# s-esposito/MonoGS

Measured on AMD Instinct MI355X. Metric: rasteriser fwd+bwd Mpix/s @1080p, higher is better.
Workload: dtype f32; 1 GPU; C5: 2000000 Gaussians, 1920x1080, fwd+bwd, seeded synthetic map (SURVEY.md 8d), one keyframe per GPU; gaussians=2000000, width=1920, height=1080, settle_steps=60, instance_count=device-side (capacity mode, overflow checked), parallelism=keyframe-per-gpu x1

## Files before the change

### include/monogs_raster.h

```cpp
#ifndef MONOGS_RASTER_H
#define MONOGS_RASTER_H

#include <stddef.h>
#include <stdint.h>

#ifdef __cplusplus
extern "C" {
#endif

#define MGS_ABI_VERSION 9
#define MGS_TILE 16

typedef struct mgs_camera {
    int32_t image_height;
    int32_t image_width;
    float tanfovx;
    float tanfovy;
    float scale_modifier;
    int32_t sh_degree;
    int32_t sh_coeffs;
    int32_t scale_dim;
    int32_t flags;
    const float* bg;
    const float* viewmatrix;
    const float* projmatrix;
    const float* projmatrix_raw;
    const float* campos;
} mgs_camera;

#define MGS_FLAG_EXCLUSIVE_DEVICE 1

typedef struct mgs_timing {
    float preprocess_ms;
    float depth_sort_ms;
    float scan_ms;
    float duplicate_ms;
    float sort_ms;
    float ranges_ms;
    float blend_fwd_ms;
    float blend_bwd_ms;
    float geom_bwd_ms;
} mgs_timing;

int mgs_abi_version(void);
const char* mgs_last_error(void);

#define MGS_MAX_GAUSSIANS ((1 << 26) - 1)

size_t mgs_geometry_bytes(int32_t P);
size_t mgs_image_bytes(int32_t width, int32_t height);
size_t mgs_binning_bytes(uint64_t num_rendered, int32_t width, int32_t height);
size_t mgs_backward_bytes(int32_t P);
float* mgs_backward_tau(void* backward_scratch, int32_t P);

int mgs_forward_preprocess(const mgs_camera* cam, int32_t P,
                           const float* means3D,
                           const float* shs,
                           const float* colors_precomp,
                           const float* opacities,
                           const float* scales,
                           const float* rotations,
                           const float* cov3D_precomp,
                           void* geometry, int32_t* radii ,
                           void* prepare_backward ,
                           uint64_t* num_rendered ,
                           const uint32_t* prev_status ,
                           uint32_t* prev_status_out ,
                           mgs_timing* timing , void* stream);

int mgs_forward_render(const mgs_camera* cam, int32_t P, uint64_t num_rendered,
                       void* geometry, void* binning, void* image,
                       float* out_color, float* out_depth, float* out_opacity, int32_t* n_touched,
                       uint32_t* status ,
                       mgs_timing* timing, void* stream);

#define MGS_STATUS_CAPACITY_OVERFLOW 1u
#define MGS_STATUS_DEPTH_SORT_TIMEOUT 2u
#define MGS_STATUS_TILE_SORT_TIMEOUT 4u

int mgs_debug_set_radix_spin_limit(uint32_t limit);
int mgs_debug_set_option(const char* name, int64_t value);

size_t mgs_debug_sort_temp_bytes(uint64_t n, int32_t bits);
int mgs_debug_sort_pairs(uint32_t* keys, uint32_t* vals, uint32_t* keys_alt, uint32_t* vals_alt, uint64_t n, int32_t bits,
                         void* temp, void* stream);

int mgs_forward_render_capacity(const mgs_camera* cam, int32_t P, uint64_t capacity,
                                void* geometry, void* binning, void* image,
                                float* out_color, float* out_depth, float* out_opacity, int32_t* n_touched,
                                uint32_t* overflow, mgs_timing* timing, void* stream);
int mgs_forward_capacity(const mgs_camera* cam, int32_t P, const float* means3D, const float* shs,
                         const float* colors_precomp, const float* opacities, const float* scales, const float* rotations,
                         const float* cov3D_precomp, void* geometry, int32_t* radii, void* prepare_backward,
                         uint64_t capacity, void* binning, void* image, float* out_color, float* out_depth,
                         float* out_opacity, int32_t* n_touched, uint32_t* overflow, mgs_timing* timing, void* stream);

int mgs_backward(const mgs_camera* cam, int32_t P, uint64_t num_rendered,
                 const float* means3D, const float* shs, const float* colors_precomp,
                 const float* opacities, const float* scales, const float* rotations,
                 const float* cov3D_precomp, const int32_t* radii,
                 const void* geometry, const void* binning, const void* image,
                 const float* dL_dcolor, const float* dL_ddepth,
                 float* dL_dmeans2D,
                 float* dL_dcolors,
                 float* dL_dopacity,
                 float* dL_dmeans3D,
                 float* dL_dcov3D,
                 float* dL_dsh,
                 float* dL_dscales,
                 float* dL_drotations,
                 float* dL_dtau,
                 void* backward_scratch, int32_t scratch_prepared, mgs_timing* timing, void* stream);

#define MGS_VALU_CEILING_BLOCKS 2048
int mgs_debug_valu_ceiling(float* out, int32_t iters, void* stream);

int mgs_debug_set_blend_events(void* fwd_start, void* fwd_end, void* bwd_start, void* bwd_end);

#define MGS_BLEND_STATS_WORDS 24
int mgs_debug_blend_stats(const mgs_camera* cam, int32_t P, uint64_t num_rendered, const void* geometry,
                          const void* binning, const void* image, uint64_t* stats_dev, void* stream);

int mgs_mark_visible(int32_t P, const float* means3D, const float* viewmatrix, const float* projmatrix,
                     uint8_t* visible, void* stream);

size_t mgs_knn_scratch_bytes(int32_t P);
int mgs_dist2_knn(int32_t P, const float* points , float* out ,
                  void* scratch, void* stream);

#define MGS_LOSS_TRACKING 1
#define MGS_LOSS_INVERT_DEPTH 2
#define MGS_LOSS_SCRATCH_DAB 10
#define MGS_LOSS_SCRATCH_LOSS 12
size_t mgs_loss_scratch_bytes(void);
int mgs_loss_forward(int32_t width, int32_t height, int32_t mode, int32_t init, float lambda_rgb,
                     const float* render, const float* depth, const float* opacity, const float* gt_rgb,
                     const float* gt_depth, const uint8_t* mask, const uint8_t* grad_mask,
                     const float* exposure_a, const float* exposure_b, float* scratch, float* loss_out,
                     void* stream);
int mgs_loss_backward(int32_t width, int32_t height, int32_t mode, int32_t init, float lambda_rgb,
                      const float* render, const float* depth, const float* opacity, const float* gt_rgb,
                      const float* gt_depth, const uint8_t* mask, const uint8_t* grad_mask,
                      const float* exposure_a, const float* exposure_b, const float* scratch,
                      const float* grad_out, float* d_render, float* d_depth, float* d_exposure, void* stream);
int mgs_loss_grads(int32_t width, int32_t height, int32_t mode, int32_t init, float lambda_rgb,
                   const float* render, const float* depth, const float* opacity, const float* gt_rgb,
                   const float* gt_depth, const uint8_t* mask, const uint8_t* grad_mask,
                   const float* exposure_a, const float* exposure_b, float* scratch, float* d_render, float* d_depth,
                   void* stream);

#define MGS_POSE_STICKY 1
int mgs_pose_step(float* R, float* T, float* rot_delta, float* trans_delta, float* exposure_a, float* exposure_b,
                  const float* grad_rot, const float* grad_trans, const float* grad_a, const float* grad_b,
                  float* adam_m, float* adam_v, int32_t step, float lr_rot, float lr_trans, float lr_exposure,
                  float beta1, float beta2, float eps, float converged_threshold, int32_t* step_counter, float* out,
                  int32_t flags, float* host_flag ,
                  const float* projmatrix_raw, float* viewmatrix, float* projmatrix, float* campos ,
                  void* stream);
int mgs_pose_step_batch(int32_t n, void* const* ptrs, float lr_rot, float lr_trans, float lr_exposure, float beta1,
                        float beta2, float eps, float converged_threshold, int32_t flags, void* stream);

int mgs_backproject(int32_t N, int32_t W, int32_t H, const int64_t* selected, const float* rgb ,
                    const float* depth , const int32_t* segmentation ,
                    const float* exposure_a, const float* exposure_b, float fx, float fy, float cx, float cy,
                    const float* R, const float* T, float* points , float* features ,
                    int32_t* ids , void* stream);

int mgs_camera_setup(const float* R, const float* T, const float* projmatrix_raw, float* viewmatrix ,
                     float* projmatrix , float* campos , void* stream);

int mgs_adam_step(int32_t n_tensors, float* const* params, const float* const* grads, float* const* exp_avg,
                  float* const* exp_avg_sq, const uint64_t* numel, const float* lr, double beta1, double beta2,
                  double eps, int32_t step, int32_t* step_counter,
                  const float* lr_device ,
                  void* stream);
int mgs_densify_stats(int32_t P, const float* viewspace_grad , const int32_t* radii,
                      float* xyz_gradient_accum , float* denom , float* max_radii_2d ,
                      void* stream);
int mgs_window_stats(int32_t P, int32_t n_keyframes, const float* const* grad_means2D, const int32_t* const* radii,
                     const int32_t* const* n_touched, float* grad_norm , float* visible ,
                     float* max_radii , int32_t accumulate, uint64_t* visibility_bits, void* stream);
int mgs_window_apply(int32_t P, const float* grad_norm, const float* visible, const float* max_radii,
                     float* xyz_gradient_accum, float* denom, float* max_radii_2d, void* stream);
int mgs_lr_schedule_step(int32_t* iteration, float* lr_out, double lr_init, double lr_final, int32_t lr_delay_steps,
                         double lr_delay_mult, int32_t max_steps, void* stream);

int mgs_activate_forward(int32_t P, int32_t scale_dim , const float* rot_raw ,
                         const float* scale_raw , const float* opacity_raw ,
                         float* rotations , float* scales3 , float* opacities ,
                         void* stream);
int mgs_activate_backward(int32_t P, int32_t scale_dim, const float* rot_raw, const float* scales3,
                          const float* opacities, const float* grad_rotations, const float* grad_scales3,
                          const float* grad_opacities, float* d_rot_raw, float* d_scale_raw, float* d_opacity_raw,
                          void* stream);

int mgs_sum_buffers(int32_t n_src, const float* const* src, float* dst, uint64_t count, void* stream);

#ifdef __cplusplus
}
#endif
#endif
```

### monogs_amd/_lib.py

```python
from __future__ import annotations

import ctypes as C
import os

_HERE = os.path.dirname(os.path.abspath(__file__))
LIB_PATH = os.environ.get("MGS_LIB_PATH") or os.path.join(_HERE, "lib", "libmonogs_raster.so")
ABI_VERSION = 9

c_float_p = C.c_void_p


class MgsCamera(C.Structure):
    _fields_ = [
        ("image_height", C.c_int32), ("image_width", C.c_int32),
        ("tanfovx", C.c_float), ("tanfovy", C.c_float), ("scale_modifier", C.c_float),
        ("sh_degree", C.c_int32), ("sh_coeffs", C.c_int32), ("scale_dim", C.c_int32), ("flags", C.c_int32),
        ("bg", C.c_void_p), ("viewmatrix", C.c_void_p), ("projmatrix", C.c_void_p),
        ("projmatrix_raw", C.c_void_p), ("campos", C.c_void_p),
    ]


class MgsTiming(C.Structure):
    _fields_ = [(n, C.c_float) for n in (
        "preprocess_ms", "depth_sort_ms", "scan_ms", "duplicate_ms", "sort_ms", "ranges_ms", "blend_fwd_ms",
        "blend_bwd_ms", "geom_bwd_ms")]

    def as_dict(self):
        return {n: float(getattr(self, n)) for n, _ in self._fields_}


SIGNATURES = {
    "mgs_abi_version": (C.c_int, []),
    "mgs_last_error": (C.c_char_p, []),
    "mgs_geometry_bytes": (C.c_size_t, [C.c_int32]),
    "mgs_image_bytes": (C.c_size_t, [C.c_int32, C.c_int32]),
    "mgs_binning_bytes": (C.c_size_t, [C.c_uint64, C.c_int32, C.c_int32]),
    "mgs_backward_bytes": (C.c_size_t, [C.c_int32]),
    "mgs_forward_preprocess": (C.c_int, [C.POINTER(MgsCamera), C.c_int32] + [C.c_void_p] * 7
                               + [C.c_void_p, C.c_void_p, C.c_void_p, C.POINTER(C.c_uint64), C.c_void_p, C.POINTER(C.c_uint32),
                                  C.POINTER(MgsTiming), C.c_void_p]),
    "mgs_forward_capacity": (C.c_int, [C.POINTER(MgsCamera), C.c_int32] + [C.c_void_p] * 7 + [C.c_void_p] * 3 + [C.c_uint64]
                             + [C.c_void_p] * 7 + [C.POINTER(MgsTiming), C.c_void_p]),
    "mgs_forward_render": (C.c_int, [C.POINTER(MgsCamera), C.c_int32, C.c_uint64] + [C.c_void_p] * 8
                           + [C.POINTER(MgsTiming), C.c_void_p]),
    "mgs_debug_set_radix_spin_limit": (C.c_int, [C.c_uint32]),
    "mgs_debug_set_option": (C.c_int, [C.c_char_p, C.c_int64]),
    "mgs_debug_sort_temp_bytes": (C.c_size_t, [C.c_uint64, C.c_int32]),
    "mgs_debug_sort_pairs": (C.c_int, [C.c_void_p] * 4 + [C.c_uint64, C.c_int32, C.c_void_p, C.c_void_p]),
    "mgs_forward_render_capacity": (C.c_int, [C.POINTER(MgsCamera), C.c_int32, C.c_uint64] + [C.c_void_p] * 8
                                    + [C.POINTER(MgsTiming), C.c_void_p]),
    "mgs_backward": (C.c_int, [C.POINTER(MgsCamera), C.c_int32, C.c_uint64] + [C.c_void_p] * 7
                     + [C.c_void_p] * 4 + [C.c_void_p] * 2 + [C.c_void_p] * 9
                     + [C.c_void_p, C.c_int32, C.POINTER(MgsTiming), C.c_void_p]),
    "mgs_backward_tau": (C.c_void_p, [C.c_void_p, C.c_int32]),
    "mgs_debug_blend_stats": (C.c_int, [C.POINTER(MgsCamera), C.c_int32, C.c_uint64] + [C.c_void_p] * 5),
    "mgs_debug_valu_ceiling": (C.c_int, [C.c_void_p, C.c_int32, C.c_void_p]),
    "mgs_debug_set_blend_events": (C.c_int, [C.c_void_p] * 4),
    "mgs_mark_visible": (C.c_int, [C.c_int32, C.c_void_p, C.c_void_p, C.c_void_p, C.c_void_p, C.c_void_p]),
    "mgs_loss_scratch_bytes": (C.c_size_t, []),
    "mgs_loss_forward": (C.c_int, [C.c_int32] * 4 + [C.c_float] + [C.c_void_p] * 9 + [C.c_void_p, C.c_void_p, C.c_void_p]),
    "mgs_loss_backward": (C.c_int, [C.c_int32] * 4 + [C.c_float] + [C.c_void_p] * 9
                          + [C.c_void_p, C.c_void_p, C.c_void_p, C.c_void_p, C.c_void_p, C.c_void_p]),
    "mgs_loss_grads": (C.c_int, [C.c_int32] * 4 + [C.c_float] + [C.c_void_p] * 9 + [C.c_void_p] * 4),
    "mgs_backproject": (C.c_int, [C.c_int32] * 3 + [C.c_void_p] * 6 + [C.c_float] * 4 + [C.c_void_p] * 6),
    "mgs_camera_setup": (C.c_int, [C.c_void_p] * 7),
    "mgs_pose_step": (C.c_int, [C.c_void_p] * 12 + [C.c_int32] + [C.c_float] * 7
                      + [C.c_void_p, C.c_void_p, C.c_int32, C.c_void_p] + [C.c_void_p] * 4 + [C.c_void_p]),
    "mgs_pose_step_batch": (C.c_int, [C.c_int32, C.POINTER(C.c_void_p)] + [C.c_float] * 7 + [C.c_int32, C.c_void_p]),
    "mgs_adam_step": (C.c_int, [C.c_int32] + [C.c_void_p] * 6 + [C.c_double] * 3 + [C.c_int32, C.c_void_p, C.c_void_p, C.c_void_p]),
    "mgs_window_stats": (C.c_int, [C.c_int32, C.c_int32] + [C.c_void_p] * 6 + [C.c_int32, C.c_void_p, C.c_void_p]),
    "mgs_window_apply": (C.c_int, [C.c_int32] + [C.c_void_p] * 7),
    "mgs_lr_schedule_step": (C.c_int, [C.c_void_p, C.c_void_p, C.c_double, C.c_double, C.c_int32, C.c_double, C.c_int32, C.c_void_p]),
    "mgs_densify_stats": (C.c_int, [C.c_int32] + [C.c_void_p] * 6),
    "mgs_sum_buffers": (C.c_int, [C.c_int32, C.POINTER(C.c_void_p), C.c_void_p, C.c_uint64, C.c_void_p]),
    "mgs_activate_forward": (C.c_int, [C.c_int32, C.c_int32] + [C.c_void_p] * 7),
    "mgs_activate_backward": (C.c_int, [C.c_int32, C.c_int32] + [C.c_void_p] * 10),
    "mgs_knn_scratch_bytes": (C.c_size_t, [C.c_int32]),
    "mgs_dist2_knn": (C.c_int, [C.c_int32, C.c_void_p, C.c_void_p, C.c_void_p, C.c_void_p]),
}

_lib = None


class MonoGSNativeError(RuntimeError):
    pass


def load():
    global _lib
    if _lib is not None:
        return _lib
    if not os.path.exists(LIB_PATH):
        raise MonoGSNativeError(
            f"{LIB_PATH} not found: build it with `python -c 'import __graft_entry__ as g; g.build()'` "
            "or `make -C monogs_amd/csrc`.  There is no CPU fallback.")
    lib = C.CDLL(LIB_PATH)
    for name, (res, args) in SIGNATURES.items():
        fn = getattr(lib, name)
        fn.restype = res
        fn.argtypes = args
    if lib.mgs_abi_version() != ABI_VERSION:
        raise MonoGSNativeError(f"ABI mismatch: library {lib.mgs_abi_version()} vs binding {ABI_VERSION}; rebuild")
    for kv in filter(None, os.environ.get("MGS_DEBUG_OPTIONS", "").split(",")):
        k, _, v = kv.partition("=")
        if lib.mgs_debug_set_option(k.strip().encode(), int(v)) != 0:
            raise MonoGSNativeError(f"MGS_DEBUG_OPTIONS: {lib.mgs_last_error().decode()}")
    _lib = lib
    return lib


def check(rc: int, what: str):
    if rc != 0:
        msg = load().mgs_last_error().decode("utf-8", "replace")
        raise Exception(msg) if rc == 1 else MonoGSNativeError(f"{what}: {msg}")
```

### monogs_amd/csrc/api.hip

```cpp
#include "common.h"

#include <stdarg.h>
#include <stdio.h>
#include <string.h>

namespace mgs {

static thread_local char g_err[512] = "";

void set_error(const char* fmt, ...) {
    va_list ap;
    va_start(ap, fmt);
    vsnprintf(g_err, sizeof(g_err), fmt, ap);
    va_end(ap);
}

static inline char* take(char*& p, size_t bytes) {
    char* r = p;
    p += align_up(bytes, 256);
    return r;
}

GeometryState GeometryState::carve(void* base, int P) {
    char* p = (char*)align_up((size_t)base, 256);
    GeometryState g;
    g.rec = (float*)take(p, (size_t)P * REC_FLOATS * sizeof(float));
    g.depth_key = (uint32_t*)take(p, (size_t)P * sizeof(uint32_t));
    g.depth_alt = (uint32_t*)take(p, (size_t)P * sizeof(uint32_t));
    g.iota = (uint32_t*)take(p, (size_t)P * sizeof(uint32_t));
    g.iota_alt = (uint32_t*)take(p, (size_t)P * sizeof(uint32_t));
    g.perm = (uint32_t*)take(p, (size_t)P * sizeof(uint32_t));
    g.point_offsets = (uint32_t*)take(p, (size_t)P * sizeof(uint32_t));
    g.scan_blocks = (uint32_t*)take(p, ((size_t)scan_nblocks(P) + 64) * sizeof(uint32_t));
    g.clamped = (uint8_t*)take(p, (size_t)P * 4);
    g.rect = (uint2*)take(p, (size_t)P * sizeof(uint2));
    g.rect_sorted = (uint2*)take(p, (size_t)P * sizeof(uint2));
    g.scan_status = (uint64_t*)take(p, (SCAN_SMALL_MAX_BLOCKS + 1) * sizeof(uint64_t));
    g.tile_hist = (uint32_t*)take(p, 4 * 256 * sizeof(uint32_t));
    g.sort_temp_bytes = radix_depth_temp_bytes((uint64_t)P);
    g.sort_temp = take(p, g.sort_temp_bytes);
    g.end = p;
    return g;
}
size_t GeometryState::bytes(int P) {
    const GeometryState g = carve(nullptr, P);
    return (size_t)g.end + 256;
}

size_t ImageState::bytes(int W, int H) {
    const size_t HW = (size_t)W * H, nt = (size_t)tiles_x(W) * tiles_y(H);
    return align_up(HW * 4, 256) * 2 + align_up(nt * sizeof(uint2), 256) + 256;
}
ImageState ImageState::carve(void* base, int W, int H) {
    const size_t HW = (size_t)W * H, nt = (size_t)tiles_x(W) * tiles_y(H);
    char* p = (char*)align_up((size_t)base, 256);
    ImageState s;
    s.final_T = (float*)take(p, HW * 4);
    s.n_contrib = (uint32_t*)take(p, HW * 4);
    s.ranges = (uint2*)take(p, nt * sizeof(uint2));
    return s;
}

size_t BinningState::bytes(uint64_t R, int W, int H) {
    const size_t r = (size_t)(R ? R : 1);
    return align_up(r * 4, 256) * 4 + align_up(mgs::sort_temp_bytes(R, tile_bits(W, H)), 256) + 256 + 256;
}
BinningState BinningState::carve(void* base, uint64_t R, int W, int H) {
    const size_t r = (size_t)(R ? R : 1);
    char* p = (char*)align_up((size_t)base, 256);
    BinningState b;
    b.keys_a = (uint32_t*)take(p, r * 4);
    b.keys_b = (uint32_t*)take(p, r * 4);
    b.vals_a = (uint32_t*)take(p, r * 4);
    b.vals_b = (uint32_t*)take(p, r * 4);
    const bool in_b = radix_result_in_b(tile_bits(W, H));
    b.keys_sorted = in_b ? b.keys_b : b.keys_a;
    b.vals_sorted = in_b ? b.vals_b : b.vals_a;
    b.sort_temp_bytes = mgs::sort_temp_bytes(R, tile_bits(W, H));
    b.sort_temp = take(p, b.sort_temp_bytes);
    b.count = (uint32_t*)take(p, 2 * sizeof(uint32_t));
    return b;
}

struct StageTimer {
    hipStream_t s;
    bool on;
    hipEvent_t ev[10];
    int n = 0;
    StageTimer(hipStream_t s_, bool on_) : s(s_), on(on_) {
        if (on) for (auto& e : ev) (void)hipEventCreate(&e);
    }
    ~StageTimer() {
        if (on) for (auto& e : ev) (void)hipEventDestroy(e);
    }
    void mark() {
        if (on && n < 10) (void)hipEventRecord(ev[n++], s);
    }
    float ms(int i) {
        float t = 0.f;
        if (on && i + 1 < n) (void)hipEventElapsedTime(&t, ev[i], ev[i + 1]);
        return t;
    }
    void sync() {
        if (on && n) (void)hipEventSynchronize(ev[n - 1]);
    }
};

static int check_cam(const mgs_camera* cam) {
    if (!cam) { set_error("camera is NULL"); return 1; }
    if (cam->image_width <= 0 || cam->image_height <= 0) { set_error("image size must be positive"); return 1; }
    if (!cam->bg || !cam->viewmatrix || !cam->projmatrix || !cam->projmatrix_raw || !cam->campos) {
        set_error("camera tensors (bg, viewmatrix, projmatrix, projmatrix_raw, campos) must be non-NULL");
        return 1;
    }
    return 0;
}

static hipEvent_t g_dbg_fwd_events[2] = {nullptr, nullptr}, g_dbg_bwd_events[2] = {nullptr, nullptr};

static int check_map_size(int32_t P) {
    if (P > MGS_MAX_GAUSSIANS) {
        set_error("P exceeds MGS_MAX_GAUSSIANS (2^26 - 1): the gradient-line offset of the blend backward is 32-bit");
        return 1;
    }
    return 0;
}

}

using namespace mgs;

extern "C" {

int mgs_abi_version(void) { return MGS_ABI_VERSION; }
const char* mgs_last_error(void) { return g_err; }

size_t mgs_geometry_bytes(int32_t P) { return GeometryState::bytes(P < 0 ? 0 : P); }
size_t mgs_image_bytes(int32_t W, int32_t H) { return ImageState::bytes(W, H); }
size_t mgs_binning_bytes(uint64_t R, int32_t W, int32_t H) { return BinningState::bytes(R, W, H); }
size_t mgs_backward_bytes(int32_t P) {
    return (size_t)(P < 0 ? 0 : P) * GRAD_FLOATS * sizeof(float) + (size_t)(TAU_SLOTS + 1) * 16 * sizeof(float) + 256;
}
float* mgs_backward_tau(void* backward_scratch, int32_t P) { return backward_tau_out(backward_scratch, P < 0 ? 0 : P); }

int mgs_forward_preprocess(const mgs_camera* cam, int32_t P, const float* means3D, const float* shs,
                           const float* colors_precomp, const float* opacities, const float* scales,
                           const float* rotations, const float* cov3D_precomp, void* geometry, int32_t* radii,
                           void* prepare_backward, uint64_t* num_rendered, const uint32_t* prev_status,
                           uint32_t* prev_status_out, mgs_timing* timing, void* stream) {
    if (check_cam(cam)) return 1;
    if (P < 0) { set_error("P must be >= 0"); return 1; }
    if (check_map_size(P)) return 1;
    if (num_rendered) *num_rendered = 0;
    if (prev_status_out) *prev_status_out = 0;
    if (P == 0) {
        if (prev_status && prev_status_out) {
            MGS_HIP(hipMemcpyAsync(prev_status_out, prev_status, sizeof(uint32_t), hipMemcpyDeviceToHost, (hipStream_t)stream));
            MGS_HIP(hipStreamSynchronize((hipStream_t)stream));
        }
        return 0;
    }
    if (!means3D || !opacities || !geometry || !radii) { set_error("means3D, opacities, geometry, radii must be non-NULL"); return 1; }
    if ((shs == nullptr) == (colors_precomp == nullptr)) {
        set_error("Please provide excatly one of either SHs or precomputed colors!");
        return 1;
    }
    const bool have_sr = scales != nullptr || rotations != nullptr;
    if ((have_sr && (!scales || !rotations || cov3D_precomp)) || (!have_sr && !cov3D_precomp)) {
        set_error("Please provide exactly one of either scale/rotation pair or precomputed 3D covariance!");
        return 1;
    }
    if (shs && (cam->sh_degree < 0 || cam->sh_degree > 3 || cam->sh_coeffs < (cam->sh_degree + 1) * (cam->sh_degree + 1))) {
        set_error("sh_degree must be 0..3 and shs must hold at least (degree+1)^2 coefficients");
        return 1;
    }
    hipStream_t s = (hipStream_t)stream;
    GeometryState g = GeometryState::carve(geometry, P);
    StageTimer tm(s, timing != nullptr);
    tm.mark();
    if (int rc = launch_preprocess_forward(*cam, P, means3D, shs, colors_precomp, opacities, scales, rotations,
                                           cov3D_precomp, g, radii,
                                           prepare_backward ? backward_grad_acc(prepare_backward) : nullptr, s)) return rc;
    tm.mark();
    const bool exclusive = (cam->flags & MGS_FLAG_EXCLUSIVE_DEVICE) != 0;
    if (depth_chain_is_small(P)) {
        if (int rc = launch_depth_chain_small(g, P, s)) return rc;
        tm.mark();
    } else {
        if (int rc = launch_depth_sort(g, P, depth_sort_payload(P, cam->image_width, cam->image_height), s, exclusive)) return rc;
        tm.mark();
        if (int rc = launch_scan(g, P, s, exclusive)) return rc;
    }
    tm.mark();
    if (num_rendered) {
        uint32_t total = 0, sort_errors[RADIX_ERROR_WORDS] = {0, 0, 0, 0};
        MGS_HIP(hipMemcpyAsync(&total, g.scan_blocks + scan_nblocks(P), sizeof(uint32_t), hipMemcpyDeviceToHost, s));
        MGS_HIP(hipMemcpyAsync(sort_errors, radix_depth_error_flag(g.sort_temp, (uint64_t)P), sizeof(sort_errors),
                               hipMemcpyDeviceToHost, s));
        if (prev_status && prev_status_out)
            MGS_HIP(hipMemcpyAsync(prev_status_out, prev_status, sizeof(uint32_t), hipMemcpyDeviceToHost, s));
        MGS_HIP(hipStreamSynchronize(s));
        if (sort_errors[0] | sort_errors[1] | sort_errors[2] | sort_errors[3]) { set_error("depth sort: a look-back spin timed out (results invalid)"); return 3; }
        *num_rendered = total;
    }
    if (timing) {
        if (!num_rendered) MGS_HIP(hipStreamSynchronize(s));
        timing->preprocess_ms = tm.ms(0);
        timing->depth_sort_ms = tm.ms(1);
        timing->scan_ms = tm.ms(2);
    }
    return 0;
}

static int forward_render_impl(const mgs_camera* cam, int32_t P, uint64_t R, bool capacity, void* geometry,
                               void* binning, void* image, float* out_color, float* out_depth, float* out_opacity,
                               int32_t* n_touched, uint32_t* overflow, mgs_timing* timing, void* stream) {
    if (check_cam(cam)) return 1;
    if (P < 0) { set_error("P must be >= 0"); return 1; }
    if (check_map_size(P)) return 1;
    if (!image || !out_color || !out_depth || !out_opacity) { set_error("image scratch and outputs must be non-NULL"); return 1; }
    if (P > 0 && (!geometry || !n_touched)) { set_error("geometry and n_touched must be non-NULL"); return 1; }
    if (R > 0 && !binning) { set_error("binning scratch is NULL"); return 1; }
    if (R >= (1ull << 32)) { set_error("num_rendered exceeds 2^32-1"); return 1; }
    if (P == 0) R = 0;
    hipStream_t s = (hipStream_t)stream;
    const int W = cam->image_width, H = cam->image_height;
    GeometryState g = GeometryState::carve(geometry, P);
    ImageState img = ImageState::carve(image, W, H);
    BinningState b = BinningState::carve(binning, R, W, H);
    const uint32_t* n_dev = nullptr;
    StageTimer tm(s, timing != nullptr);
    const bool cap = capacity && binning;
    if (cap) n_dev = b.count;
    tm.mark();
    if (int rc = launch_duplicate(*cam, P, g, b, capacity ? R : (R > 0 ? 0xFFFFFFFFull : 0ull), n_touched, img, R,
                                  tile_bits(W, H), cap ? b.count : nullptr, overflow, s)) return rc;
    tm.mark();
    if (int rc = launch_sort(g, b, R, tile_bits(W, H), s, n_dev, (cam->flags & MGS_FLAG_EXCLUSIVE_DEVICE) != 0, img.ranges)) return rc;
    tm.mark();
    if (g_dbg_fwd_events[0]) MGS_HIP(hipEventRecord(g_dbg_fwd_events[0], s));
    if (int rc = launch_blend_forward(*cam, g, b, img, out_color, out_depth, out_opacity, n_touched,
                                      R > 0 ? radix_error_flag(b.sort_temp, R, tile_bits(W, H)) : nullptr, overflow, s)) return rc;
    if (g_dbg_fwd_events[1]) MGS_HIP(hipEventRecord(g_dbg_fwd_events[1], s));
    tm.mark();
    if (timing) {
        tm.sync();
        timing->duplicate_ms = tm.ms(0);
        timing->sort_ms = tm.ms(1);
        timing->ranges_ms = 0.f;
        timing->blend_fwd_ms = tm.ms(2);
    }
    return 0;
}

int mgs_forward_render(const mgs_camera* cam, int32_t P, uint64_t R, void* geometry, void* binning, void* image,
                       float* out_color, float* out_depth, float* out_opacity, int32_t* n_touched,
                       uint32_t* status, mgs_timing* timing, void* stream) {
    return forward_render_impl(cam, P, R, false, geometry, binning, image, out_color, out_depth, out_opacity, n_touched,
                               status, timing, stream);
}

int mgs_forward_render_capacity(const mgs_camera* cam, int32_t P, uint64_t capacity, void* geometry, void* binning,
                                void* image, float* out_color, float* out_depth, float* out_opacity,
                                int32_t* n_touched, uint32_t* overflow, mgs_timing* timing, void* stream) {
    if (capacity == 0) { set_error("capacity must be > 0"); return 1; }
    return forward_render_impl(cam, P, capacity, true, geometry, binning, image, out_color, out_depth, out_opacity,
                               n_touched, overflow, timing, stream);
}

int mgs_forward_capacity(const mgs_camera* cam, int32_t P, const float* means3D, const float* shs,
                         const float* colors_precomp, const float* opacities, const float* scales, const float* rotations,
                         const float* cov3D_precomp, void* geometry, int32_t* radii, void* prepare_backward,
                         uint64_t capacity, void* binning, void* image, float* out_color, float* out_depth,
                         float* out_opacity, int32_t* n_touched, uint32_t* overflow, mgs_timing* timing, void* stream) {
    if (int rc = mgs_forward_preprocess(cam, P, means3D, shs, colors_precomp, opacities, scales, rotations, cov3D_precomp,
                                        geometry, radii, prepare_backward, nullptr, nullptr, nullptr, timing, stream)) return rc;
    return mgs_forward_render_capacity(cam, P, capacity, geometry, binning, image, out_color, out_depth, out_opacity,
                                       n_touched, overflow, timing, stream);
}

int mgs_backward(const mgs_camera* cam, int32_t P, uint64_t R, const float* means3D, const float* shs,
                 const float* colors_precomp, const float* opacities, const float* scales, const float* rotations,
                 const float* cov3D_precomp, const int32_t* radii, const void* geometry, const void* binning,
                 const void* image, const float* dL_dcolor, const float* dL_ddepth, float* dL_dmeans2D,
                 float* dL_dcolors, float* dL_dopacity, float* dL_dmeans3D, float* dL_dcov3D, float* dL_dsh,
                 float* dL_dscales, float* dL_drotations, float* dL_dtau, void* backward_scratch,
                 int32_t scratch_prepared, mgs_timing* timing, void* stream) {
    if (check_cam(cam)) return 1;
    if (P < 0) { set_error("P must be >= 0"); return 1; }
    if (check_map_size(P)) return 1;
    hipStream_t s = (hipStream_t)stream;
    if (P == 0) {
        if (dL_dtau) MGS_HIP(zero_fill(dL_dtau, 6 * sizeof(float), s));
        return 0;
    }
    if (!means3D || !opacities || !radii || !geometry || !image || !dL_dcolor || !dL_ddepth || !backward_scratch) {
        set_error("means3D, opacities, radii, geometry, image, dL_dcolor, dL_ddepth, backward_scratch must be non-NULL");
        return 1;
    }
    if (R > 0 && !binning) { set_error("binning scratch is NULL"); return 1; }
    const int W = cam->image_width, H = cam->image_height;
    GeometryState g = GeometryState::carve(const_cast<void*>(geometry), P);
    ImageState img = ImageState::carve(const_cast<void*>(image), W, H);
    BinningState b = BinningState::carve(const_cast<void*>(binning), R, W, H);
    float* grad_acc = backward_grad_acc(backward_scratch);
    StageTimer tm(s, timing != nullptr);
    float* tau_part = (dL_dtau && (P + 255) / 256 > TAU_DIRECT_MAX_BLOCKS) ? backward_tau_part(backward_scratch, P) : nullptr;
    if (scratch_prepared) {
        if (dL_dtau && dL_dtau != backward_tau_out(backward_scratch, P)) {
            set_error("scratch_prepared: dL_dtau must be mgs_backward_tau(backward_scratch, P)");
            return 1;
        }
    } else {
        MGS_HIP(zero_fill2(grad_acc, (size_t)P * GRAD_FLOATS * sizeof(float) + (tau_part ? (size_t)TAU_SLOTS * 16 * sizeof(float) : 0),
                           dL_dtau, 6 * sizeof(float), s));
    }
    tm.mark();
    if (R > 0) {
        const bool pose_only = !dL_dcolors && !dL_dopacity && !dL_dsh && !shs;
        if (g_dbg_bwd_events[0]) MGS_HIP(hipEventRecord(g_dbg_bwd_events[0], s));
        if (int rc = launch_blend_backward(*cam, g, b, img, dL_dcolor, dL_ddepth, grad_acc, pose_only, s)) return rc;
        if (g_dbg_bwd_events[1]) MGS_HIP(hipEventRecord(g_dbg_bwd_events[1], s));
    }
    tm.mark();
    GeomBackwardArgs a;
    a.means3D = means3D; a.shs = shs; a.colors_precomp = colors_precomp; a.opacities = opacities;
    a.scales = scales; a.rotations = rotations; a.cov3D_precomp = cov3D_precomp; a.radii = radii;
    a.grad_acc = grad_acc;
    a.dL_dmeans2D = dL_dmeans2D; a.dL_dcolors = dL_dcolors; a.dL_dopacity = dL_dopacity;
    a.dL_dmeans3D = dL_dmeans3D; a.dL_dcov3D = dL_dcov3D; a.dL_dsh = dL_dsh; a.dL_dscales = dL_dscales;
    a.dL_drotations = dL_drotations; a.dL_dtau = dL_dtau; a.tau_part = tau_part;
    if (int rc = launch_geom_backward(*cam, P, g, a, s)) return rc;
    tm.mark();
    if (timing) {
        tm.sync();
        timing->blend_bwd_ms = tm.ms(0);
        timing->geom_bwd_ms = tm.ms(1);
    }
    return 0;
}

int mgs_debug_blend_stats(const mgs_camera* cam, int32_t P, uint64_t R, const void* geometry, const void* binning,
                           const void* image, uint64_t* stats_dev, void* stream) {
    if (check_cam(cam)) return 1;
    if (!geometry || !image || !stats_dev || (R > 0 && !binning)) { set_error("bad arguments"); return 1; }
    hipStream_t s = (hipStream_t)stream;
    MGS_HIP(zero_fill(stats_dev, MGS_BLEND_STATS_WORDS * sizeof(uint64_t), s));
    if (P == 0 || R == 0) return 0;
    const int W = cam->image_width, H = cam->image_height;
    GeometryState g = GeometryState::carve(const_cast<void*>(geometry), P);
    ImageState img = ImageState::carve(const_cast<void*>(image), W, H);
    BinningState b = BinningState::carve(const_cast<void*>(binning), R, W, H);
    return launch_blend_backward_stats(*cam, g, b, img, (unsigned long long*)stats_dev, s);
}

int mgs_debug_valu_ceiling(float* out, int32_t iters, void* stream) {
    if (!out || iters < 1) { set_error("mgs_debug_valu_ceiling: bad arguments"); return 1; }
    return launch_valu_ceiling(out, iters, (hipStream_t)stream);
}

int mgs_debug_set_radix_spin_limit(uint32_t limit) { return set_radix_spin_limit(limit); }

int mgs_debug_set_blend_events(void* fwd_start, void* fwd_end, void* bwd_start, void* bwd_end) {
    if ((fwd_start == nullptr) != (fwd_end == nullptr) || (bwd_start == nullptr) != (bwd_end == nullptr)) {
        set_error("mgs_debug_set_blend_events: a pair is both events or neither");
        return 1;
    }
    g_dbg_fwd_events[0] = (hipEvent_t)fwd_start; g_dbg_fwd_events[1] = (hipEvent_t)fwd_end;
    g_dbg_bwd_events[0] = (hipEvent_t)bwd_start; g_dbg_bwd_events[1] = (hipEvent_t)bwd_end;
    return 0;
}

static int g_opt_debug_sort_exclusive = 0;
size_t mgs_debug_sort_temp_bytes(uint64_t n, int32_t bits) { return radix_temp_bytes(n, bits); }
int mgs_debug_sort_pairs(uint32_t* keys, uint32_t* vals, uint32_t* keys_alt, uint32_t* vals_alt, uint64_t n, int32_t bits,
                         void* temp, void* stream) {
    if (bits < 1 || bits > 32 || (n && (!keys || !vals || !keys_alt || !vals_alt || !temp))) {
        set_error("mgs_debug_sort_pairs: bad arguments");
        return 1;
    }
    if (n == 0) return 0;
    hipStream_t s = (hipStream_t)stream;
    if (int rc = radix_sort_pairs(keys, vals, keys_alt, vals_alt, n, bits, temp, s, nullptr, false, nullptr, nullptr, nullptr, false,
                                  g_opt_debug_sort_exclusive != 0))
        return rc;
    if (radix_result_in_b(bits)) {
        MGS_HIP(hipMemcpyAsync(keys, keys_alt, n * 4, hipMemcpyDeviceToDevice, s));
        MGS_HIP(hipMemcpyAsync(vals, vals_alt, n * 4, hipMemcpyDeviceToDevice, s));
    }
    uint32_t err[RADIX_ERROR_WORDS];
    MGS_HIP(hipMemcpyAsync(err, radix_error_flag(temp, n, bits), sizeof(err), hipMemcpyDeviceToHost, s));
    MGS_HIP(hipStreamSynchronize(s));
    if (err[0] | err[1] | err[2] | err[3]) { set_error("mgs_debug_sort_pairs: a look-back spin timed out"); return 2; }
    return 0;
}

int mgs_debug_set_option(const char* name, int64_t value) {
    if (name && !strcmp(name, "radix_scanned")) { g_opt_radix_scanned = (int)value; return 0; }
    if (name && !strcmp(name, "radix_ballot_rank")) { g_opt_radix_ballot_rank = (int)value; return 0; }
    if (name && !strcmp(name, "radix_tile_items")) { g_opt_radix_tile_items = (int)value; return 0; }
    if (name && !strcmp(name, "radix_xcd_band")) { g_opt_radix_xcd_band = (int)value; return 0; }
    if (name && !strcmp(name, "debug_sort_exclusive")) { g_opt_debug_sort_exclusive = (int)value; return 0; }
    if (name && !strcmp(name, "dup_slot_major")) { g_opt_dup_slot_major = (int)value; return 0; }
    if (name && !strcmp(name, "blend_bwd_transposed")) { g_opt_blend_bwd_transposed = (int)value; return 0; }
    if (name && !strcmp(name, "scan_small")) { g_opt_scan_small = (int)value; return 0; }
    if (name && !strcmp(name, "depth_small")) { g_opt_depth_small = (int)value; return 0; }
    if (name && !strcmp(name, "blend_lds_pad_fwd")) { g_opt_blend_lds_pad_fwd = (int)value; return 0; }
    if (name && !strcmp(name, "blend_lds_pad_bwd")) { g_opt_blend_lds_pad_bwd = (int)value; return 0; }
    if (name && !strcmp(name, "knn_grid_min")) { g_opt_knn_grid_min = value > 0x7FFFFFFF ? 0x7FFFFFFF : (int)value; return 0; }
    set_error("mgs_debug_set_option: unknown option");
    return 1;
}

int mgs_mark_visible(int32_t P, const float* means3D, const float* viewmatrix, const float* projmatrix,
                     uint8_t* visible, void* stream) {
    (void)projmatrix;
    if (P < 0 || (P > 0 && (!means3D || !viewmatrix || !visible))) { set_error("bad arguments"); return 1; }
    return launch_mark_visible(P, means3D, viewmatrix, visible, (hipStream_t)stream);
}

size_t mgs_knn_scratch_bytes(int32_t P) { return knn_scratch_bytes(P); }

int mgs_dist2_knn(int32_t P, const float* points, float* out, void* scratch, void* stream) {
    if (P < 0 || (P > 0 && (!points || !out))) { set_error("bad arguments"); return 1; }
    return launch_knn(P, points, out, scratch, (hipStream_t)stream);
}

}
```

### monogs_amd/csrc/binning.hip

```cpp
#include "common.h"


namespace mgs {

constexpr int SCAN_THREADS = 256;
__device__ __forceinline__ int scan_nblocks_dev(int P) { return (P + SCAN_ITEMS - 1) / SCAN_ITEMS; }
constexpr int SCAN_PER_THREAD = SCAN_ITEMS / SCAN_THREADS;

__device__ __forceinline__ uint32_t wave_incl_scan(uint32_t v, int) { return wave_incl_scan_dpp(v); }

__device__ __forceinline__ uint32_t block_excl_scan(uint32_t v, uint32_t& total, uint32_t* smem ) {
    const int lane = threadIdx.x & 63, wv = threadIdx.x >> 6;
    const uint32_t incl = wave_incl_scan(v, lane);
    if (lane == 63) smem[wv] = incl;
    __syncthreads();
    uint32_t base = 0;
    for (int w = 0; w < wv; ++w) base += smem[w];
    total = smem[0] + smem[1] + smem[2] + smem[3];
    __syncthreads();
    return base + incl - v;
}

__device__ __forceinline__ uint32_t scan_block_rows(const uint2* __restrict__ rects, int n, int cbase, int lane, int wv,
                                                    uint32_t (&incl)[SCAN_PER_THREAD], uint32_t* smem ) {
    uint32_t v[SCAN_PER_THREAD];
#pragma unroll
    for (int i = 0; i < SCAN_PER_THREAD; ++i) {
        const int idx = cbase + i * WAVE + lane;
        const uint32_t wh = idx < n ? rects[idx].y : 0u;
        v[i] = (wh & 0xFFFFu) * (wh >> 16);
    }
    uint32_t run = 0;
#pragma unroll
    for (int i = 0; i < SCAN_PER_THREAD; ++i) {
        const uint32_t sc = wave_incl_scan_dpp(v[i]);
        incl[i] = run + sc;
        run += (uint32_t)__builtin_amdgcn_readlane((int)sc, 63);
    }
    if (lane == 0) smem[wv] = run;
    __syncthreads();
    uint32_t wbase = 0;
    for (int w = 0; w < wv; ++w) wbase += smem[w];
    const uint32_t total = (smem[0] + smem[1]) + (smem[2] + smem[3]);
#pragma unroll
    for (int i = 0; i < SCAN_PER_THREAD; ++i) incl[i] += wbase;
    return total;
}

__global__ void __launch_bounds__(SCAN_THREADS) scan_local_kernel(const uint2* __restrict__ rects, uint32_t* out,
                                                                  uint32_t* block_sums, int n) {
    __shared__ uint32_t smem[8];
    const int lane = threadIdx.x & 63, wv = threadIdx.x >> 6;
    const int cbase = blockIdx.x * SCAN_ITEMS + wv * (SCAN_PER_THREAD * WAVE);
    uint32_t incl[SCAN_PER_THREAD];
    const uint32_t total = scan_block_rows(rects, n, cbase, lane, wv, incl, smem);
#pragma unroll
    for (int i = 0; i < SCAN_PER_THREAD; ++i) {
        const int idx = cbase + i * WAVE + lane;
        if (idx < n) out[idx] = incl[i];
    }
    if (threadIdx.x == 0) block_sums[blockIdx.x] = total;
}

__global__ void __launch_bounds__(SCAN_THREADS) scan_blocks_kernel(uint32_t* block_sums, int nblocks) {
    __shared__ uint32_t smem[8];
    uint32_t carry = 0;
    for (int start = 0; start < nblocks; start += SCAN_THREADS) {
        const int i = start + threadIdx.x;
        const uint32_t v = i < nblocks ? block_sums[i] : 0u;
        uint32_t total;
        const uint32_t ex = block_excl_scan(v, total, smem);
        if (i < nblocks) block_sums[i] = carry + ex;
        carry += total;
    }
    if (threadIdx.x == 0) block_sums[nblocks] = carry;
}

constexpr uint32_t SCAN_SPIN_LIMIT = 1u << 22;
__global__ void __launch_bounds__(SCAN_THREADS) scan_small_kernel(const uint2* __restrict__ rects, uint32_t* out,
                                                                  uint32_t* block_sums, uint64_t* status, int n, int nb,
                                                                  uint32_t* err, int ticketed) {
    __shared__ uint32_t smem[8];
    __shared__ uint32_t s_prefix, s_bid;
    const int lane = threadIdx.x & 63, wv = threadIdx.x >> 6;
    int bid = (int)blockIdx.x;
    if (ticketed) {
        if (threadIdx.x == 0) s_bid = atomicAdd((uint32_t*)(status + SCAN_SMALL_MAX_BLOCKS), 1u);
        __syncthreads();
        bid = (int)s_bid;
    }
    const int cbase = bid * SCAN_ITEMS + wv * (SCAN_PER_THREAD * WAVE);
    uint32_t incl[SCAN_PER_THREAD];
    const uint32_t total = scan_block_rows(rects, n, cbase, lane, wv, incl, smem);
    if (threadIdx.x == 0)
        __hip_atomic_store(status + bid, (1ull << 63) | (uint64_t)total, __ATOMIC_RELAXED, __HIP_MEMORY_SCOPE_AGENT);
    if (threadIdx.x < WAVE) {
        uint32_t before = 0;
        if ((int)threadIdx.x < bid) {
            uint64_t w = 0;
            uint32_t spins = 0;
            while (true) {
                w = __hip_atomic_load(status + threadIdx.x, __ATOMIC_RELAXED, __HIP_MEMORY_SCOPE_AGENT);
                if (w >> 63) break;
                if (++spins > SCAN_SPIN_LIMIT) { atomicExch(err, 1u); break; }
                __builtin_amdgcn_s_sleep(1);
            }
            before = (uint32_t)w;
        }
#pragma unroll
        for (int o = 32; o > 0; o >>= 1) before += __shfl_xor(before, o, 64);
        if (threadIdx.x == 0) s_prefix = before;
    }
    __syncthreads();
#pragma unroll
    for (int i = 0; i < SCAN_PER_THREAD; ++i) {
        const int idx = cbase + i * WAVE + lane;
        if (idx < n) out[idx] = incl[i] + s_prefix;
    }
    if (threadIdx.x == 0 && bid == nb - 1) block_sums[nb] = s_prefix + total;
}
int g_opt_scan_small = -1;
bool scan_is_small(int P) { return g_opt_scan_small != 0 && scan_nblocks(P) <= SCAN_SMALL_MAX_BLOCKS; }


int launch_scan(const GeometryState& g, int P, hipStream_t s, bool exclusive) {
    if (P == 0) return 0;
    const int nb = scan_nblocks(P);
    if (scan_is_small(P)) {
        hipLaunchKernelGGL(scan_small_kernel, dim3(nb), dim3(SCAN_THREADS), 0, s, g.rect_sorted, g.point_offsets, g.scan_blocks,
                           g.scan_status, P, nb, const_cast<uint32_t*>(radix_depth_error_flag(g.sort_temp, (uint64_t)P)),
                           exclusive ? 0 : 1);
        MGS_HIP(hipGetLastError());
        return 0;
    }
    hipLaunchKernelGGL(scan_local_kernel, dim3(nb), dim3(SCAN_THREADS), 0, s, g.rect_sorted, g.point_offsets,
                       g.scan_blocks, P);
    hipLaunchKernelGGL(scan_blocks_kernel, dim3(1), dim3(SCAN_THREADS), 0, s, g.scan_blocks, nb);
    MGS_HIP(hipGetLastError());
    return 0;
}

constexpr int DS_THREADS = 1024, DS_WAVES = DS_THREADS / WAVE, DS_ROWS = 24;
constexpr int DS_SMALL_MAX = DS_THREADS * DS_ROWS;
__global__ void __launch_bounds__(DS_THREADS) depth_chain_small_kernel(const uint32_t* __restrict__ depth_key,
                                                                       const uint2* __restrict__ rect,
                                                                       uint32_t* __restrict__ perm, uint2* __restrict__ rect_sorted,
                                                                       uint32_t* __restrict__ offsets,
                                                                       uint32_t* __restrict__ grand_total, int n
#ifdef DS_TRACE
                                                                       , unsigned long long* trace
#define DS_STAMP(i) do { __syncthreads(); if (threadIdx.x == 0) { unsigned long long t_; asm volatile("s_memrealtime %0\n\ts_waitcnt lgkmcnt(0)" : "=s"(t_) :: "memory"); trace[i] = t_; } } while (0)
#else
#define DS_STAMP(i) do { } while (0)
#endif
                                                                       ) {
    __shared__ uint32_t s_key[DS_SMALL_MAX];
    __shared__ uint16_t s_idx[DS_SMALL_MAX];
    __shared__ uint32_t s_tab[DS_WAVES][128];
    __shared__ uint32_t s_part[DS_WAVES];
    const int lane = threadIdx.x & 63, wv = __builtin_amdgcn_readfirstlane((int)(threadIdx.x >> 6));
    const int rows = (n + DS_THREADS - 1) / DS_THREADS;
    const int chunk = rows * WAVE;
    const int e0 = wv * chunk + lane;
#pragma unroll
    for (int i = 0; i < DS_ROWS; ++i) {
        const int e = e0 + i * WAVE;
        if (i < rows && e < n) {
            s_key[e] = depth_key[e];
            s_idx[e] = (uint16_t)e;
        }
    }
    uint16_t* const tab16 = reinterpret_cast<uint16_t*>(&s_tab[0][0]);
    DS_STAMP(0);
    for (int pass = 0; pass < 4; ++pass) {
        const int shift = 8 * pass;
        for (int t = threadIdx.x; t < DS_WAVES * 128; t += DS_THREADS) (&s_tab[0][0])[t] = 0u;
        __syncthreads();
        uint32_t k[DS_ROWS], vr[DS_ROWS];
#pragma unroll
        for (int i = 0; i < DS_ROWS; ++i) {
            const int e = e0 + i * WAVE;
            k[i] = 0u; vr[i] = 0u;
            if (i < rows && e < n) {
                k[i] = s_key[e];
                const uint32_t d = (k[i] >> shift) & 255u, sh = 16u * (d & 1u);
                const uint32_t old = atomicAdd(&s_tab[wv][d >> 1], 1u << sh);
                vr[i] = ((uint32_t)s_idx[e] << 16) | ((old >> sh) & 0xFFFFu);
            }
        }
        __syncthreads();
        DS_STAMP(1 + 4 * pass);
        uint32_t tot = 0;
        if (threadIdx.x < 256) {
#pragma unroll
            for (int w = 0; w < DS_WAVES; ++w) {
                const uint32_t c = tab16[w * 256 + threadIdx.x];
                tab16[w * 256 + threadIdx.x] = (uint16_t)tot;
                tot += c;
            }
        }
        if (threadIdx.x < 256) {
            const uint32_t incl = wave_incl_scan_dpp(tot);
            if (lane == 63) s_part[wv] = incl;
            tot = incl - tot;
        }
        __syncthreads();
        if (threadIdx.x < 256) {
            uint32_t base = tot;
            for (int w = 0; w < wv; ++w) base += s_part[w];
#pragma unroll
            for (int w = 0; w < DS_WAVES; ++w) tab16[w * 256 + threadIdx.x] = (uint16_t)(tab16[w * 256 + threadIdx.x] + base);
        }
        __syncthreads();
        DS_STAMP(2 + 4 * pass);
#pragma unroll
        for (int i = 0; i < DS_ROWS; ++i) {
            const int e = e0 + i * WAVE;
            if (i < rows && e < n) {
                const uint32_t d = (k[i] >> shift) & 255u;
                const uint32_t dst = (uint32_t)tab16[wv * 256 + d] + (vr[i] & 0xFFFFu);
                s_key[dst] = k[i];
                s_idx[dst] = (uint16_t)(vr[i] >> 16);
            }
        }
        __syncthreads();
        DS_STAMP(3 + 4 * pass);
    }
    uint2 rc[DS_ROWS];
#pragma unroll
    for (int i = 0; i < DS_ROWS; ++i) {
        const int e = e0 + i * WAVE;
        rc[i] = make_uint2(0u, 0u);
        if (i < rows && e < n) {
            const uint32_t g = s_idx[e];
            perm[e] = g;
            if (s_key[e] != 0xFFFFFFFFu) rc[i] = rect[g];
        }
    }
    DS_STAMP(17);
    uint32_t incl[DS_ROWS], run = 0;
#pragma unroll
    for (int i = 0; i < DS_ROWS; ++i) {
        const uint32_t tt = (rc[i].y & 0xFFFFu) * (rc[i].y >> 16);
        const uint32_t sc = wave_incl_scan_dpp(tt);
        incl[i] = run + sc;
        run += (uint32_t)__builtin_amdgcn_readlane((int)sc, 63);
    }
    if (lane == 0) s_part[wv] = run;
    __syncthreads();
    uint32_t wbase = 0, total = 0;
    for (int w = 0; w < DS_WAVES; ++w) {
        const uint32_t p = s_part[w];
        wbase += w < wv ? p : 0u;
        total += p;
    }
#pragma unroll
    for (int i = 0; i < DS_ROWS; ++i) {
        const int e = e0 + i * WAVE;
        if (i < rows && e < n) {
            rect_sorted[e] = rc[i];
            offsets[e] = incl[i] + wbase;
        }
    }
    if (threadIdx.x == 0) *grand_total = total;
    DS_STAMP(18);
}
int g_opt_depth_small = 0;
bool depth_chain_is_small(int P) { return g_opt_depth_small > 0 && P > 0 && P <= DS_SMALL_MAX; }
int launch_depth_chain_small(const GeometryState& g, int P, hipStream_t s) {
    hipLaunchKernelGGL(depth_chain_small_kernel, dim3(1), dim3(DS_THREADS), 0, s, g.depth_key, g.rect, g.perm, g.rect_sorted,
                       g.point_offsets, g.scan_blocks + scan_nblocks(P), P
#ifdef DS_TRACE
                       , (unsigned long long*)nullptr
#endif
                       );
    MGS_HIP(hipGetLastError());
    return 0;
}

__global__ void __launch_bounds__(256) duplicate_kernel(int P, const uint2* __restrict__ rects,
                                                        const uint32_t* __restrict__ perm,
                                                        const uint32_t* __restrict__ offsets ,
                                                        const uint32_t* __restrict__ block_sums ,
                                                        uint32_t* keys,
                                                        uint32_t* vals, int gx, int gy, uint32_t r_cap,
                                                        int32_t* __restrict__ n_touched, uint2* __restrict__ ranges,
                                                        int ntiles, uint32_t* __restrict__ zero_ptr, size_t zero_words,
                                                        uint32_t* __restrict__ count, uint32_t* __restrict__ overflow,
                                                        const uint32_t* __restrict__ depth_err, int offsets_global,
                                                        uint32_t* __restrict__ hist , int hist_passes,
                                                        int n_threads , int slot_major) {
    const int i = blockIdx.x * 256 + threadIdx.x;
    const int lane = threadIdx.x & 63;
    grid_zero(zero_ptr, zero_words, (size_t)n_threads, 256);
    const bool depth_bad = depth_err && radix_failed(depth_err) != 0u;
    if (i == 0 && count) {
        const uint32_t R = (P > 0 && !depth_bad) ? block_sums[scan_nblocks_dev(P)] : 0u;
        count[0] = min(R, r_cap);
        count[1] = R > r_cap ? 1u : 0u;
    }
    if (i == 0 && overflow)
        overflow[0] = (count ? count[1] : 0u) | (depth_bad ? (uint32_t)MGS_STATUS_DEPTH_SORT_TIMEOUT : 0u);
    if (i < ntiles) ranges[i] = make_uint2(0xFFFFFFFFu, 0u);
    if (i < P) n_touched[i] = 0;
    uint32_t idx = 0, nt = 0, off = 0;
    int x0 = 0, y0 = 0, x1 = 0;
    if (i < P) {
        idx = perm[i];
        const uint2 r = rects[i];
        const int w = (int)(r.y & 0xFFFFu), h = (int)(r.y >> 16);
        nt = (uint32_t)(w * h);
        x0 = (int)(r.x & 0xFFFFu); y0 = (int)(r.x >> 16); x1 = x0 + w;
    }
    if (depth_bad) nt = 0;
    if (nt) off = i == 0 ? 0u : offsets[i - 1] + (offsets_global ? 0u : block_sums[(i - 1) / SCAN_ITEMS]);
    __shared__ uint32_t s_own[4][WAVE];
    __shared__ uint32_t s_idx[4][WAVE], s_off[4][WAVE];
    __shared__ int s_x0[4][WAVE], s_y0[4][WAVE], s_w[4][WAVE];
    __shared__ uint32_t s_hist[2][256];
    if (hist) {
        s_hist[0][threadIdx.x] = 0u; s_hist[1][threadIdx.x] = 0u;
        __syncthreads();
    }
    const int wv = threadIdx.x >> 6;
    if (slot_major) {
        const uint32_t R_all = (P > 0 && !depth_bad) ? block_sums[scan_nblocks_dev(P)] : 0u;
        const uint32_t R_emit = min(R_all, r_cap);
        const uint32_t n_waves = (uint32_t)n_threads / WAVE;
        const uint32_t CH = (((R_emit + n_waves - 1u) / n_waves) + 63u) & ~63u;
        const uint32_t wave_id = (uint32_t)blockIdx.x * 4u + (uint32_t)wv;
        const uint64_t s0w = (uint64_t)wave_id * CH;
        const uint32_t s0 = s0w < (uint64_t)R_emit ? (uint32_t)s0w : R_emit, s1 = (uint64_t)s0 + CH < (uint64_t)R_emit ? s0 + CH : R_emit;
        auto incl = [&](uint32_t k) { return offsets[k] + (offsets_global ? 0u : block_sums[k / SCAN_ITEMS]); };
        uint32_t g = 0;
        if (s0 < s1) {
            uint32_t lo = 0, hi = (uint32_t)P;
            while (hi - lo > 1u) {
                const uint32_t span = hi - lo, step = (span + 63u) / 64u;
                const uint32_t probe = lo + min(((uint32_t)lane + 1u) * step, span) - 1u;
                const unsigned long long above = __builtin_amdgcn_ballot_w64(incl(probe) > s0);
                const int k = __builtin_ctzll(above);
                const uint32_t pk = lo + min(((uint32_t)k + 1u) * step, span) - 1u;
                const uint32_t pk1 = k == 0 ? lo : lo + min((uint32_t)k * step, span);
                lo = pk1; hi = pk + 1u;
            }
            g = lo;
        }
        uint32_t sl = s0;
        while (sl < s1 && g < (uint32_t)P) {
            const uint32_t gi = g + (uint32_t)lane;
            const bool valid = gi < (uint32_t)P;
            uint32_t inc = 0, ntg = 0, idg = 0;
            int gx0 = 0, gy0 = 0, gw = 1;
            if (valid) {
                inc = incl(gi);
                const uint2 r = rects[gi];
                gw = (int)(r.y & 0xFFFFu);
                ntg = (uint32_t)(gw * (int)(r.y >> 16));
                gx0 = (int)(r.x & 0xFFFFu); gy0 = (int)(r.x >> 16);
                idg = perm[gi];
            }
            const uint32_t exc = inc - ntg;
            uint32_t Eg = valid ? inc : 0u;
#pragma unroll
            for (int o2 = 32; o2 > 0; o2 >>= 1) Eg = max(Eg, (uint32_t)__shfl_xor((int)Eg, o2, 64));
            __builtin_amdgcn_wave_barrier();
            s_idx[wv][lane] = idg; s_off[wv][lane] = exc; s_x0[wv][lane] = gx0; s_y0[wv][lane] = gy0; s_w[wv][lane] = max(gw, 1);
            const uint32_t e = min(s1, Eg);
            const uint32_t cb0 = sl & ~63u;
            const unsigned long long before = __builtin_amdgcn_ballot_w64(ntg != 0u && exc < cb0);
            uint32_t carry = before ? 64u - (uint32_t)__builtin_clzll(before) : 0u;
            for (uint32_t cb = cb0; cb < e; cb += WAVE) {
                __builtin_amdgcn_wave_barrier();
                s_own[wv][lane] = 0u;
                __builtin_amdgcn_wave_barrier();
                if (ntg != 0u && exc >= cb && exc < cb + WAVE) s_own[wv][exc - cb] = (uint32_t)lane + 1u;
                __builtin_amdgcn_wave_barrier();
                uint32_t m = s_own[wv][lane];
#define MGS_DPP_MAX(ctrl, row_mask) m = max(m, (uint32_t)__builtin_amdgcn_update_dpp(0, (int)m, ctrl, row_mask, 0xf, false))
                MGS_DPP_MAX(0x111, 0xf); MGS_DPP_MAX(0x112, 0xf); MGS_DPP_MAX(0x114, 0xf); MGS_DPP_MAX(0x118, 0xf);
                MGS_DPP_MAX(0x142, 0xa); MGS_DPP_MAX(0x143, 0xc);
#undef MGS_DPP_MAX
                const uint32_t owner = max(m, carry);
                carry = (uint32_t)__builtin_amdgcn_readlane((int)owner, 63);
                const uint32_t o = cb + lane;
                if (owner != 0u && o >= sl && o < e) {
                    const uint32_t L = owner - 1u;
                    const uint32_t t = o - s_off[wv][L];
                    const uint32_t w = (uint32_t)s_w[wv][L];
                    const uint32_t yy = t / w, xx = t - yy * w;
                    const uint32_t key = (uint32_t)((s_y0[wv][L] + (int)yy) * gx + s_x0[wv][L] + (int)xx);
                    keys[o] = key;
                    vals[o] = s_idx[wv][L];
                    if (hist) {
                        atomicAdd(&s_hist[0][key & 0xFFu], 1u);
                        if (hist_passes > 1) {
                            const uint32_t d1 = (key >> 8) & 0xFFu;
                            const uint32_t lead = (uint32_t)__builtin_amdgcn_readfirstlane((int)d1);
                            const unsigned long long same = __builtin_amdgcn_ballot_w64(d1 == lead);
                            if (d1 != lead) atomicAdd(&s_hist[1][d1], 1u);
                            else if (lane == (int)__builtin_ctzll(same)) atomicAdd(&s_hist[1][lead], (uint32_t)__popcll(same));
                        }
                    }
                }
            }
            sl = max(sl, e);
            if (Eg <= sl) g += WAVE;
        }
        if (hist) {
            __syncthreads();
            const uint32_t c0 = s_hist[0][threadIdx.x], c1 = s_hist[1][threadIdx.x];
            if (c0) atomicAdd(hist + threadIdx.x, c0);
            if (c1) atomicAdd(hist + 256 + threadIdx.x, c1);
        }
        return;
    }
    s_idx[wv][lane] = idx; s_off[wv][lane] = off; s_x0[wv][lane] = x0; s_y0[wv][lane] = y0; s_w[wv][lane] = max(x1 - x0, 1);
    const unsigned long long live = __builtin_amdgcn_ballot_w64(nt != 0);
    if (live == 0ull && !hist) return;
    const int first = live ? __builtin_ctzll(live) : 0, lastl = live ? 63 - __builtin_clzll(live) : 0;
    const uint32_t S = live ? (uint32_t)__builtin_amdgcn_readlane((int)off, first) : 0u;
    const uint32_t E = live ? (uint32_t)__builtin_amdgcn_readlane((int)(off + nt), lastl) : 0u;
    uint32_t carry = 0;
    for (uint32_t cb = S & ~63u; cb < E; cb += WAVE) {
        __builtin_amdgcn_wave_barrier();
        s_own[wv][lane] = 0u;
        __builtin_amdgcn_wave_barrier();
        if (nt != 0 && off >= cb && off < cb + WAVE) s_own[wv][off - cb] = (uint32_t)lane + 1u;
        __builtin_amdgcn_wave_barrier();
        uint32_t m = s_own[wv][lane];
#define MGS_DPP_MAX(ctrl, row_mask) m = max(m, (uint32_t)__builtin_amdgcn_update_dpp(0, (int)m, ctrl, row_mask, 0xf, false))
        MGS_DPP_MAX(0x111, 0xf); MGS_DPP_MAX(0x112, 0xf); MGS_DPP_MAX(0x114, 0xf); MGS_DPP_MAX(0x118, 0xf);
        MGS_DPP_MAX(0x142, 0xa); MGS_DPP_MAX(0x143, 0xc);
#undef MGS_DPP_MAX
        const uint32_t owner = max(m, carry);
        carry = (uint32_t)__builtin_amdgcn_readlane((int)owner, 63);
        const uint32_t o = cb + lane;
        if (owner != 0u && o < E && o < r_cap) {
            const uint32_t L = owner - 1u;
            const uint32_t t = o - s_off[wv][L];
            const uint32_t w = (uint32_t)s_w[wv][L];
            const uint32_t yy = t / w, xx = t - yy * w;
            const uint32_t key = (uint32_t)((s_y0[wv][L] + (int)yy) * gx + s_x0[wv][L] + (int)xx);
            keys[o] = key;
            vals[o] = s_idx[wv][L];
            if (hist) {
                atomicAdd(&s_hist[0][key & 0xFFu], 1u);
                if (hist_passes > 1) {
                    const uint32_t d1 = (key >> 8) & 0xFFu;
                    const uint32_t lead = (uint32_t)__builtin_amdgcn_readfirstlane((int)d1);
                    const unsigned long long same = __builtin_amdgcn_ballot_w64(d1 == lead);
                    if (d1 != lead) atomicAdd(&s_hist[1][d1], 1u);
                    else if (lane == (int)__builtin_ctzll(same)) atomicAdd(&s_hist[1][lead], (uint32_t)__popcll(same));
                }
            }
        }
    }
    if (hist) {
        __syncthreads();
        const uint32_t c0 = s_hist[0][threadIdx.x], c1 = s_hist[1][threadIdx.x];
        if (c0) atomicAdd(hist + threadIdx.x, c0);
        if (c1) atomicAdd(hist + 256 + threadIdx.x, c1);
    }
}

constexpr uint64_t DUP_SLOT_MAJOR_MIN = 768ull * 1024;
int g_opt_dup_slot_major = -1;

int launch_duplicate(const mgs_camera& cam, int P, const GeometryState& g, const BinningState& b, uint64_t r_cap,
                     int32_t* n_touched, const ImageState& img, uint64_t sort_n, int sort_bits, uint32_t* count,
                     uint32_t* overflow, hipStream_t s) {
    const uint32_t* depth_err = P > 0 ? radix_depth_error_flag(g.sort_temp, (uint64_t)P) : nullptr;
    const int ntiles = tiles_x(cam.image_width) * tiles_y(cam.image_height);
    int n = P > ntiles ? P : ntiles;
    if (n == 0) return 0;
    const bool slot_major = P > 0 && g_opt_dup_slot_major != 0 &&
                            (g_opt_dup_slot_major > 0 || (sort_n >= DUP_SLOT_MAJOR_MIN && sort_n >= 6ull * (uint64_t)P));
    if (slot_major) {
        const uint64_t want = sort_n / 8;
        if (want > (uint64_t)n) n = (int)(want > 0x3FFFFFFFull ? 0x3FFFFFFFull : want);
    }
    const int n_threads = (n + 255) / 256 * 256;
    uint32_t* zero_ptr = nullptr;
    size_t zero_words = 0;
    if (sort_n > 0) radix_zero_region(b.sort_temp, sort_n, sort_bits, &zero_ptr, &zero_words);
    const bool count_digits = P > 0 && sort_bits <= 16 && radix_wants_hist(sort_n);
    hipLaunchKernelGGL(duplicate_kernel, dim3(n_threads / 256), dim3(256), 0, s, P, g.rect_sorted, g.perm, g.point_offsets,
                       g.scan_blocks, b.keys_a, b.vals_a, tiles_x(cam.image_width), tiles_y(cam.image_height),
                       (uint32_t)(r_cap > 0xFFFFFFFFull ? 0xFFFFFFFFull : r_cap), n_touched, img.ranges, ntiles, zero_ptr,
                       zero_words, count, overflow, depth_err, (P > 0 && (scan_is_small(P) || depth_chain_is_small(P))) ? 1 : 0,
                       count_digits ? g.tile_hist : nullptr, (sort_bits + 7) / 8, n_threads, slot_major ? 1 : 0);
    MGS_HIP(hipGetLastError());
    return 0;
}

size_t sort_temp_bytes(uint64_t n, int bits) { return radix_temp_bytes(n, bits); }

int launch_depth_sort(const GeometryState& g, int P, bool payload, hipStream_t s, bool exclusive) {
    return radix_sort_depth(g.depth_key, g.depth_alt, g.iota, g.iota_alt, g.rect, payload, g.perm, g.rect_sorted, (uint64_t)P,
                            g.sort_temp, s, true, exclusive);
}

int launch_sort(const GeometryState& g, const BinningState& b, uint64_t R, int bits, hipStream_t s, const uint32_t* n_dev,
                bool exclusive, uint2* ranges) {
    if (R == 0) return 0;
    const bool counted = bits <= 16 && radix_wants_hist(R) && g.tile_hist != nullptr;
    return radix_sort_pairs(b.keys_a, b.vals_a, b.keys_b, b.vals_b, R, bits, b.sort_temp, s, n_dev, true, nullptr, nullptr,
                            counted ? g.tile_hist : nullptr, false, exclusive, ranges);
}


}
```

### monogs_amd/csrc/common.h

```cpp
#pragma once

#include <hip/hip_runtime.h>
#include <stdint.h>
#include <stddef.h>

#include "../../include/monogs_raster.h"

namespace mgs {

constexpr int TILE = MGS_TILE;
constexpr int WAVE = 64;
constexpr int SUB = 8;
constexpr int REC_FLOATS = 16;
constexpr int GRAD_FLOATS = 16;

enum : int {
    R_X = 0, R_Y = 1, R_EX = 2, R_EY = 3,
    R_CA = 4, R_CB = 5, R_CC = 6, R_OPAC = 7,
    R_R = 8, R_G = 9, R_B = 10, R_DEPTH = 11,
    R_NA = 12, R_NB = 13, R_NC = 14, R_RADIUS = 15
};
enum : int {
    G_SX = 0, G_SY = 1, G_SXX = 2, G_SXY = 3, G_SYY = 4, G_SH = 5,
    G_DR = 6, G_DG = 7, G_DB = 8, G_DDEPTH = 9
};

inline size_t align_up(size_t v, size_t a) { return (v + a - 1) / a * a; }

#if defined(__HIP_DEVICE_COMPILE__)
typedef const float __attribute__((address_space(4))) * const_float_p;
#define MGS_CONST(p) ((mgs::const_float_p)(p))
#else
typedef const float* const_float_p;
#define MGS_CONST(p) (p)
#endif

__device__ __forceinline__ uint32_t wave_incl_scan_dpp(uint32_t v) {
#define MGS_DPP_ADD(ctrl, row_mask) v += (uint32_t)__builtin_amdgcn_update_dpp(0, (int)v, ctrl, row_mask, 0xf, false)
    MGS_DPP_ADD(0x111, 0xf);
    MGS_DPP_ADD(0x112, 0xf);
    MGS_DPP_ADD(0x114, 0xf);
    MGS_DPP_ADD(0x118, 0xf);
    MGS_DPP_ADD(0x142, 0xa);
    MGS_DPP_ADD(0x143, 0xc);
#undef MGS_DPP_ADD
    return v;
}

__global__ static void zero_fill_kernel(uint32_t* __restrict__ p, size_t n_words, int vec) {
    const size_t i0 = (size_t)blockIdx.x * blockDim.x + threadIdx.x, stride = (size_t)gridDim.x * blockDim.x;
    if (vec) {
        uint4* q = reinterpret_cast<uint4*>(p);
        const size_t nv = n_words / 4;
        for (size_t i = i0; i < nv; i += stride) q[i] = make_uint4(0u, 0u, 0u, 0u);
        for (size_t i = nv * 4 + i0; i < n_words; i += stride) p[i] = 0u;
    } else {
        for (size_t i = i0; i < n_words; i += stride) p[i] = 0u;
    }
}
__device__ __forceinline__ void grid_zero(uint32_t* __restrict__ p, size_t n_words, size_t threads, int block) {
    const size_t i0 = (size_t)blockIdx.x * block + threadIdx.x, stride = threads;
    uint4* q = reinterpret_cast<uint4*>(p);
    const size_t nv = n_words / 4;
    for (size_t i = i0; i < nv; i += stride) q[i] = make_uint4(0u, 0u, 0u, 0u);
    for (size_t i = nv * 4 + i0; i < n_words; i += stride) p[i] = 0u;
}
__global__ static void zero_fill2_kernel(uint32_t* __restrict__ p, size_t n_words, uint32_t* __restrict__ p2, int n2) {
    grid_zero(p, n_words, (size_t)gridDim.x * 256, 256);
    if (blockIdx.x == 0 && (int)threadIdx.x < n2) p2[threadIdx.x] = 0u;
}
static inline hipError_t zero_fill2(void* ptr, size_t bytes, void* ptr2, size_t bytes2, hipStream_t s) {
    const size_t n_words = bytes / 4;
    size_t blocks = (n_words / 4 + 255) / 256;
    blocks = blocks < 1 ? 1 : (blocks > 4096 ? 4096 : blocks);
    hipLaunchKernelGGL(zero_fill2_kernel, dim3((unsigned)blocks), dim3(256), 0, s, (uint32_t*)ptr, n_words,
                       (uint32_t*)ptr2, ptr2 ? (int)(bytes2 / 4) : 0);
    return hipGetLastError();
}
static inline hipError_t zero_fill(void* ptr, size_t bytes, hipStream_t s) {
    if (bytes == 0) return hipSuccess;
    const size_t n_words = bytes / 4;
    const int vec = ((size_t)ptr % 16 == 0) ? 1 : 0;
    const size_t items = vec ? (n_words + 3) / 4 : n_words;
    size_t blocks = (items + 255) / 256;
    if (blocks > 4096) blocks = 4096;
    hipLaunchKernelGGL(zero_fill_kernel, dim3((unsigned)blocks), dim3(256), 0, s, (uint32_t*)ptr, n_words, vec);
    return hipGetLastError();
}

struct GeometryState {
    float* rec;
    uint32_t* depth_key;
    uint32_t* depth_alt;
    uint32_t* iota;
    uint32_t* iota_alt;
    uint32_t* perm;
    uint32_t* point_offsets;
    uint32_t* scan_blocks;
    uint8_t* clamped;
    uint2* rect;
    uint2* rect_sorted;
    uint64_t* scan_status;
    uint32_t* tile_hist;
    void* sort_temp;
    size_t sort_temp_bytes;
    char* end;
    static size_t bytes(int P);
    static GeometryState carve(void* base, int P);
};
constexpr int SCAN_SMALL_MAX_BLOCKS = 64;

struct ImageState {
    float* final_T;
    uint32_t* n_contrib;
    uint2* ranges;
    static size_t bytes(int W, int H);
    static ImageState carve(void* base, int W, int H);
};

struct BinningState {
    uint32_t* keys_a;
    uint32_t* vals_a;
    uint32_t* keys_b;
    uint32_t* vals_b;
    uint32_t* keys_sorted;
    uint32_t* vals_sorted;
    void* sort_temp;
    size_t sort_temp_bytes;
    uint32_t* count;
    static size_t bytes(uint64_t R, int W, int H);
    static BinningState carve(void* base, uint64_t R, int W, int H);
};

constexpr int SCAN_ITEMS = 2048;
inline int scan_nblocks(int P) { return (P + SCAN_ITEMS - 1) / SCAN_ITEMS; }

inline int tiles_x(int W) { return (W + TILE - 1) / TILE; }
inline int tiles_y(int H) { return (H + TILE - 1) / TILE; }
inline int tile_bits(int W, int H) {
    uint32_t n = (uint32_t)(tiles_x(W) * tiles_y(H));
    int b = 0;
    while ((1u << b) < n && b < 31) ++b;
    return b == 0 ? 1 : b;
}

void set_error(const char* fmt, ...);
#define MGS_HIP(expr)                                                                     \
    do {                                                                                  \
        hipError_t _e = (expr);                                                           \
        if (_e != hipSuccess) {                                                           \
            mgs::set_error("%s failed: %s (%s:%d)", #expr, hipGetErrorString(_e), __FILE__, __LINE__); \
            return 2;                                                                     \
        }                                                                                 \
    } while (0)

struct StageTimer;

int launch_preprocess_forward(const mgs_camera& cam, int P, const float* means3D, const float* shs,
                              const float* colors_precomp, const float* opacities, const float* scales,
                              const float* rotations, const float* cov3D_precomp,
                              const GeometryState& g, int32_t* radii, float* prepare_grad_acc, hipStream_t s);
constexpr int TAU_SLOTS = 256;
inline float* backward_grad_acc(void* scratch) { return (float*)align_up((size_t)scratch, 256); }
inline float* backward_tau_part(void* scratch, int P) { return backward_grad_acc(scratch) + (size_t)P * GRAD_FLOATS; }
inline float* backward_tau_out(void* scratch, int P) { return backward_tau_part(scratch, P) + (size_t)TAU_SLOTS * 16; }
int launch_scan(const GeometryState& g, int P, hipStream_t s, bool exclusive = false);
bool depth_chain_is_small(int P);
int launch_depth_chain_small(const GeometryState& g, int P, hipStream_t s);
int launch_duplicate(const mgs_camera& cam, int P, const GeometryState& g, const BinningState& b, uint64_t r_cap,
                     int32_t* n_touched, const ImageState& img, uint64_t sort_n, int sort_bits, uint32_t* count,
                     uint32_t* overflow, hipStream_t s);
size_t sort_temp_bytes(uint64_t n, int bits);
size_t radix_temp_bytes(uint64_t n, int bits);
size_t radix_depth_temp_bytes(uint64_t n);
bool radix_result_in_b(int bits);
constexpr int RADIX_ERROR_WORDS = 4;
const uint32_t* radix_error_flag(void* temp, uint64_t n, int bits);
const uint32_t* radix_depth_error_flag(void* temp, uint64_t n);
__device__ __forceinline__ uint32_t radix_failed(const uint32_t* __restrict__ e) { return (e[0] | e[1]) | (e[2] | e[3]); }
void radix_zero_region(void* temp, uint64_t n, int bits, uint32_t** ptr, size_t* words);
void radix_depth_zero_region(void* temp, uint64_t n, uint32_t** ptr, size_t* words);
int radix_sort_pairs(uint32_t* ka, uint32_t* va, uint32_t* kb, uint32_t* vb, uint64_t n, int bits, void* temp,
                     hipStream_t s, const uint32_t* n_dev = nullptr, bool temp_zeroed = false,
                     const uint2* aux_in = nullptr, uint2* aux_out = nullptr,
                     const uint32_t* ext_hist = nullptr,
                     bool aux_empty_for_ones = false,
                     bool exclusive = false,
                     uint2* ranges = nullptr);
bool radix_wants_hist(uint64_t n);
bool radix_depth_payload(uint64_t n);
int radix_sort_depth(uint32_t* keys, uint32_t* key_b, uint32_t* val_a, uint32_t* val_b, void* rect, bool payload,
                     uint32_t* perm, uint2* rect_sorted, uint64_t n, void* temp, hipStream_t s, bool temp_zeroed,
                     bool exclusive = false);
inline bool depth_sort_payload(int P, int W, int H) { return radix_depth_payload((uint64_t)P) && tiles_x(W) <= 255 && tiles_y(H) <= 255; }
int launch_depth_sort(const GeometryState& g, int P, bool payload, hipStream_t s, bool exclusive = false);
int launch_sort(const GeometryState& g, const BinningState& b, uint64_t R, int bits, hipStream_t s,
                const uint32_t* n_dev = nullptr, bool exclusive = false, uint2* ranges = nullptr);
int set_radix_spin_limit(uint32_t limit);
extern int g_opt_radix_ballot_rank, g_opt_radix_scanned, g_opt_radix_xcd_band, g_opt_radix_tile_items, g_opt_knn_grid_min, g_opt_scan_small, g_opt_dup_slot_major, g_opt_blend_bwd_transposed, g_opt_blend_lds_pad_fwd, g_opt_blend_lds_pad_bwd, g_opt_depth_small;
int launch_blend_forward(const mgs_camera& cam, const GeometryState& g, const BinningState& b,
                         const ImageState& img, float* out_color, float* out_depth, float* out_opacity,
                         int32_t* n_touched, const uint32_t* sort_err, uint32_t* status, hipStream_t s);
int launch_blend_backward(const mgs_camera& cam, const GeometryState& g, const BinningState& b,
                          const ImageState& img, const float* dL_dcolor, const float* dL_ddepth,
                          float* grad_acc, bool pose_only, hipStream_t s);
int launch_blend_backward_stats(const mgs_camera& cam, const GeometryState& g, const BinningState& b,
                                const ImageState& img, unsigned long long* stats, hipStream_t s);
int launch_valu_ceiling(float* out, int iters, hipStream_t s);
struct GeomBackwardArgs {
    const float *means3D, *shs, *colors_precomp, *opacities, *scales, *rotations, *cov3D_precomp;
    const int32_t* radii;
    const float* grad_acc;
    float *dL_dmeans2D, *dL_dcolors, *dL_dopacity, *dL_dmeans3D, *dL_dcov3D, *dL_dsh, *dL_dscales,
        *dL_drotations, *dL_dtau;
    float* tau_part;
};
constexpr int TAU_DIRECT_MAX_BLOCKS = 256;
int launch_geom_backward(const mgs_camera& cam, int P, const GeometryState& g, const GeomBackwardArgs& a,
                         hipStream_t s);
int launch_mark_visible(int P, const float* means3D, const float* viewmatrix, uint8_t* visible, hipStream_t s);
size_t knn_scratch_bytes(int P);
int launch_knn(int P, const float* points, float* out, void* scratch, hipStream_t s);

}
```

### monogs_amd/csrc/preprocess.hip

```cpp
#include "common.h"

#pragma clang fp contract(off)

namespace mgs {

__device__ __forceinline__ float dot3p(float m0, float m1, float m2, float m3, float x, float y, float z) {
    return ((m0 * x + m1 * y) + m2 * z) + m3;
}

__device__ constexpr float SH_C0 = 0.28209479177387814f;
__device__ constexpr float SH_C1 = 0.4886025119029199f;
__device__ constexpr float SH_C2[5] = {1.0925484305920792f, -1.0925484305920792f, 0.31539156525252005f,
                                       -1.0925484305920792f, 0.5462742152960396f};
__device__ constexpr float SH_C3[7] = {-0.5900435899266435f, 2.890611442640554f, -0.4570457994644658f,
                                       0.3731763325901154f, -0.4570457994644658f, 1.445305721320277f,
                                       -0.5900435899266435f};

struct Cam {
    float V[16], PM[16], PR[16];
    float campos[3];
    float tanfovx, tanfovy, focal_x, focal_y, mod;
    int W, H, gx, gy, deg, M;
};

__device__ __forceinline__ void load_cam(Cam& c, const float* V_, const float* PM_, const float* PR_,
                                         const float* campos_) {
    const const_float_p V = MGS_CONST(V_), PM = MGS_CONST(PM_), PR = MGS_CONST(PR_), campos = MGS_CONST(campos_);
#pragma unroll
    for (int i = 0; i < 16; ++i) { c.V[i] = V[i]; c.PM[i] = PM[i]; }
    if (PR_) {
#pragma unroll
        for (int i = 0; i < 16; ++i) c.PR[i] = PR[i];
    } else {
#pragma unroll
        for (int i = 0; i < 16; ++i) c.PR[i] = 0.f;
    }
    c.campos[0] = campos[0]; c.campos[1] = campos[1]; c.campos[2] = campos[2];
}

__device__ __forceinline__ void pin_cam(const Cam& c, bool with_pr) {
    asm volatile("" ::"s"(c.V[0]), "s"(c.V[1]), "s"(c.V[2]), "s"(c.V[3]), "s"(c.V[4]), "s"(c.V[5]), "s"(c.V[6]), "s"(c.V[7]),
                 "s"(c.V[8]), "s"(c.V[9]), "s"(c.V[10]), "s"(c.V[11]), "s"(c.V[12]), "s"(c.V[13]), "s"(c.V[14]), "s"(c.V[15]));
    asm volatile("" ::"s"(c.PM[0]), "s"(c.PM[1]), "s"(c.PM[2]), "s"(c.PM[3]), "s"(c.PM[4]), "s"(c.PM[5]), "s"(c.PM[6]),
                 "s"(c.PM[7]), "s"(c.PM[8]), "s"(c.PM[9]), "s"(c.PM[10]), "s"(c.PM[11]), "s"(c.PM[12]), "s"(c.PM[13]),
                 "s"(c.PM[14]), "s"(c.PM[15]), "s"(c.campos[0]), "s"(c.campos[1]), "s"(c.campos[2]));
    if (with_pr)
        asm volatile("" ::"s"(c.PR[0]), "s"(c.PR[1]), "s"(c.PR[2]), "s"(c.PR[3]), "s"(c.PR[4]), "s"(c.PR[5]), "s"(c.PR[6]),
                     "s"(c.PR[7]), "s"(c.PR[8]), "s"(c.PR[9]), "s"(c.PR[10]), "s"(c.PR[11]), "s"(c.PR[12]), "s"(c.PR[13]),
                     "s"(c.PR[14]), "s"(c.PR[15]));
}

__device__ __forceinline__ void cov3d_from_scale_rot(const float s[3], const float q[4], float mod, float cov[6],
                                                     float Mm[9]) {
    const float r = q[0], x = q[1], y = q[2], z = q[3];
    float Rm[9] = {1.f - 2.f * (y * y + z * z), 2.f * (x * y - r * z), 2.f * (x * z + r * y),
                   2.f * (x * y + r * z), 1.f - 2.f * (x * x + z * z), 2.f * (y * z - r * x),
                   2.f * (x * z - r * y), 2.f * (y * z + r * x), 1.f - 2.f * (x * x + y * y)};
    const float sx = s[0] * mod, sy = s[1] * mod, sz = s[2] * mod;
#pragma unroll
    for (int i = 0; i < 3; ++i) {
        Mm[3 * i + 0] = Rm[3 * i + 0] * sx;
        Mm[3 * i + 1] = Rm[3 * i + 1] * sy;
        Mm[3 * i + 2] = Rm[3 * i + 2] * sz;
    }
    auto e = [&](int i, int j) {
        return (Mm[3 * i] * Mm[3 * j] + Mm[3 * i + 1] * Mm[3 * j + 1]) + Mm[3 * i + 2] * Mm[3 * j + 2];
    };
    cov[0] = e(0, 0); cov[1] = e(0, 1); cov[2] = e(0, 2);
    cov[3] = e(1, 1); cov[4] = e(1, 2); cov[5] = e(2, 2);
}

struct Proj {
    float tx, ty, tz;
    bool clamp_x, clamp_y;
    float J00, J02, J11, J12;
    float T0[3], T1[3];
    float cxx, cxy, cyy;
};

__device__ __forceinline__ void project_cov(const Cam& c, const float pv[3], const float cov[6], Proj& p) {
    const float limx = 1.3f * c.tanfovx, limy = 1.3f * c.tanfovy;
    const float tz = pv[2];
    const float txtz = pv[0] / tz, tytz = pv[1] / tz;
    p.clamp_x = (txtz < -limx) || (txtz > limx);
    p.clamp_y = (tytz < -limy) || (tytz > limy);
    p.tx = fminf(limx, fmaxf(-limx, txtz)) * tz;
    p.ty = fminf(limy, fmaxf(-limy, tytz)) * tz;
    p.tz = tz;
    const float tz2 = tz * tz;
    p.J00 = c.focal_x / tz;
    p.J02 = -(c.focal_x * p.tx) / tz2;
    p.J11 = c.focal_y / tz;
    p.J12 = -(c.focal_y * p.ty) / tz2;
#pragma unroll
    for (int j = 0; j < 3; ++j) {
        p.T0[j] = p.J00 * c.V[4 * j + 0] + p.J02 * c.V[4 * j + 2];
        p.T1[j] = p.J11 * c.V[4 * j + 1] + p.J12 * c.V[4 * j + 2];
    }
    const float S[3][3] = {{cov[0], cov[1], cov[2]}, {cov[1], cov[3], cov[4]}, {cov[2], cov[4], cov[5]}};
    float U0[3], U1[3];
#pragma unroll
    for (int j = 0; j < 3; ++j) {
        U0[j] = (p.T0[0] * S[0][j] + p.T0[1] * S[1][j]) + p.T0[2] * S[2][j];
        U1[j] = (p.T1[0] * S[0][j] + p.T1[1] * S[1][j]) + p.T1[2] * S[2][j];
    }
    p.cxx = ((U0[0] * p.T0[0] + U0[1] * p.T0[1]) + U0[2] * p.T0[2]) + 0.3f;
    p.cxy = (U0[0] * p.T1[0] + U0[1] * p.T1[1]) + U0[2] * p.T1[2];
    p.cyy = ((U1[0] * p.T1[0] + U1[1] * p.T1[1]) + U1[2] * p.T1[2]) + 0.3f;
}

__device__ __forceinline__ void tile_rect(float px, float py, float radius, int gx, int gy, int& x0, int& y0,
                                          int& x1, int& y1) {
    x0 = min(gx, max(0, (int)((px - radius) / (float)TILE)));
    y0 = min(gy, max(0, (int)((py - radius) / (float)TILE)));
    x1 = min(gx, max(0, (int)(((px + radius) + (float)(TILE - 1)) / (float)TILE)));
    y1 = min(gy, max(0, (int)(((py + radius) + (float)(TILE - 1)) / (float)TILE)));
}

__device__ __forceinline__ void eval_sh(int deg, const float* sh, const float d[3], float out[3]) {
    const float x = d[0], y = d[1], z = d[2];
#pragma unroll
    for (int ch = 0; ch < 3; ++ch) {
        float res = SH_C0 * sh[ch];
        if (deg > 0) {
            res = res - SH_C1 * y * sh[3 + ch] + SH_C1 * z * sh[6 + ch] - SH_C1 * x * sh[9 + ch];
            if (deg > 1) {
                const float xx = x * x, yy = y * y, zz = z * z, xy = x * y, yz = y * z, xz = x * z;
                res = res + SH_C2[0] * xy * sh[12 + ch] + SH_C2[1] * yz * sh[15 + ch] +
                      SH_C2[2] * (2.f * zz - xx - yy) * sh[18 + ch] + SH_C2[3] * xz * sh[21 + ch] +
                      SH_C2[4] * (xx - yy) * sh[24 + ch];
                if (deg > 2) {
                    res = res + SH_C3[0] * y * (3.f * xx - yy) * sh[27 + ch] + SH_C3[1] * xy * z * sh[30 + ch] +
                          SH_C3[2] * y * (4.f * zz - xx - yy) * sh[33 + ch] +
                          SH_C3[3] * z * (2.f * zz - 3.f * xx - 3.f * yy) * sh[36 + ch] +
                          SH_C3[4] * x * (4.f * zz - xx - yy) * sh[39 + ch] + SH_C3[5] * z * (xx - yy) * sh[42 + ch] +
                          SH_C3[6] * x * (xx - 3.f * yy) * sh[45 + ch];
                }
            }
        }
        out[ch] = res + 0.5f;
    }
}

struct PreArgs {
    const float *means3D, *shs, *colors, *opacities, *scales, *rotations, *cov3D;
    const float *V, *PM, *campos;
    float* rec;
    uint32_t* depth_key;
    int rect_packed;
    uint8_t* clamped;
    uint2* rect;
    int32_t* radii;
    float tanfovx, tanfovy, focal_x, focal_y, mod;
    int P, W, H, gx, gy, deg, M;
    int iso;
    int rot_aligned16;
    uint32_t* zero_ptr;
    size_t zero_words;
    float* grad_acc;
};

__device__ __forceinline__ void load4(const float* __restrict__ p, bool aligned16, float o[4]) {
    if (aligned16) {
        const float4 v = *reinterpret_cast<const float4*>(p);
        o[0] = v.x; o[1] = v.y; o[2] = v.z; o[3] = v.w;
    } else {
        o[0] = p[0]; o[1] = p[1]; o[2] = p[2]; o[3] = p[3];
    }
}

struct PreOut {
    float4 r0, r1, r2, r3;
    int radius;
    uint2 rect;
    uint32_t key;
};

template <bool COV, bool PRECOMP>
__device__ __forceinline__ bool preprocess_one(const PreArgs& a, const Cam& c, int idx, float x, float y, float z,
                                               const float cov_in[6], const float s[3], const float q[4],
                                               const float col_in[3], float opac, PreOut& o) {
    float pv[3];
#pragma unroll
    for (int k = 0; k < 3; ++k) pv[k] = dot3p(c.V[k], c.V[4 + k], c.V[8 + k], c.V[12 + k], x, y, z);
    if (!(pv[2] > 0.2f)) return false;
    float ph[4];
#pragma unroll
    for (int k = 0; k < 4; ++k) ph[k] = dot3p(c.PM[k], c.PM[4 + k], c.PM[8 + k], c.PM[12 + k], x, y, z);
    const float p_w = 1.0f / (ph[3] + 0.0000001f);
    const float projx = ph[0] * p_w, projy = ph[1] * p_w;

    float cov[6];
    if (COV) {
#pragma unroll
        for (int k = 0; k < 6; ++k) cov[k] = cov_in[k];
    } else {
        float Mm[9];
        cov3d_from_scale_rot(s, q, a.mod, cov, Mm);
    }
    Proj p;
    project_cov(c, pv, cov, p);
    const float det = p.cxx * p.cyy - p.cxy * p.cxy;
    if (det == 0.0f) return false;
    const float det_inv = 1.f / det;
    const float ca = p.cyy * det_inv, cb = -p.cxy * det_inv, cc = p.cxx * det_inv;
    const float mid = 0.5f * (p.cxx + p.cyy);
    const float disc = sqrtf(fmaxf(0.1f, mid * mid - det));
    const float lam = fmaxf(mid + disc, mid - disc);
    const float radius = ceilf(3.f * sqrtf(lam));
    const float px = ((projx + 1.0f) * (float)a.W - 1.0f) * 0.5f;
    const float py = ((projy + 1.0f) * (float)a.H - 1.0f) * 0.5f;
    if (!(isfinite(px) && isfinite(py) && isfinite(radius))) return false;
    int x0, y0, x1, y1;
    tile_rect(px, py, radius, a.gx, a.gy, x0, y0, x1, y1);
    const int ntile = (x1 - x0) * (y1 - y0);
    if (ntile == 0) return false;

    float rgb[3];
    if (PRECOMP) {
        rgb[0] = col_in[0]; rgb[1] = col_in[1]; rgb[2] = col_in[2];
    } else {
        float d[3] = {x - c.campos[0], y - c.campos[1], z - c.campos[2]};
        const float len = sqrtf((d[0] * d[0] + d[1] * d[1]) + d[2] * d[2]);
        d[0] = d[0] / len; d[1] = d[1] / len; d[2] = d[2] / len;
        eval_sh(a.deg, a.shs + (size_t)idx * a.M * 3, d, rgb);
#pragma unroll
        for (int ch = 0; ch < 3; ++ch) {
            a.clamped[4 * idx + ch] = rgb[ch] < 0.f;
            rgb[ch] = fmaxf(rgb[ch], 0.f);
        }
    }

    float ex = -1.f, ey = -1.f;
    float na = 0.f, nb = 0.f, nc = 0.f;
    const float tau = logf(255.0f * opac);
    if (tau > 0.f) {
        ex = sqrtf(2.f * tau * p.cxx) * 1.001f + 0.05f;
        ey = sqrtf(2.f * tau * p.cyy) * 1.001f + 0.05f;
        const float it = 1.f / (2.f * tau);
        na = ca * it; nb = cb * it; nc = cc * it;
    } else if (!(tau <= 0.f)) {
        ex = ey = 3.0e38f;
    }

    o.r0 = make_float4(px, py, ex, ey);
    constexpr float LOG2E = 1.4426950408889634f;
    o.r1 = make_float4(-0.5f * LOG2E * ca, -LOG2E * cb, -0.5f * LOG2E * cc, opac);
    o.r2 = make_float4(rgb[0], rgb[1], rgb[2], pv[2]);
    o.r3 = make_float4(na, nb, nc, radius);
    o.radius = (int)radius;
    o.rect = make_uint2((uint32_t)x0 | ((uint32_t)y0 << 16), (uint32_t)(x1 - x0) | ((uint32_t)(y1 - y0) << 16));
    o.key = __float_as_uint(pv[2]);
    return true;
}

template <bool COV, bool PRECOMP>
__global__ void __launch_bounds__(256) preprocess_forward_kernel(PreArgs a) {
    const int idx = blockIdx.x * 256 + threadIdx.x;
    grid_zero(a.zero_ptr, a.zero_words, (size_t)((a.P + 255) / 256) * 256, 256);
    if (a.grad_acc && blockIdx.x == 0) {
        float4* t4 = reinterpret_cast<float4*>(a.grad_acc + (size_t)a.P * GRAD_FLOATS);
        for (int i = threadIdx.x; i < (TAU_SLOTS + 1) * 4; i += 256) t4[i] = make_float4(0.f, 0.f, 0.f, 0.f);
    }
    if (idx >= a.P) return;
    Cam c;
    load_cam(c, a.V, a.PM, nullptr, a.campos);
    c.tanfovx = a.tanfovx; c.tanfovy = a.tanfovy; c.focal_x = a.focal_x; c.focal_y = a.focal_y;
    const float x = a.means3D[3 * idx], y = a.means3D[3 * idx + 1], z = a.means3D[3 * idx + 2];
    const float opac = a.opacities[idx];
    float cov_in[6] = {0.f, 0.f, 0.f, 0.f, 0.f, 0.f}, s[3] = {0.f, 0.f, 0.f}, q[4] = {1.f, 0.f, 0.f, 0.f};
    float col_in[3] = {0.f, 0.f, 0.f};
    if (COV) {
#pragma unroll
        for (int k = 0; k < 6; ++k) cov_in[k] = a.cov3D[6 * idx + k];
    } else {
        const float* sp = a.scales + (a.iso ? (size_t)idx : 3 * (size_t)idx);
        const int o1 = a.iso ? 0 : 1, o2 = a.iso ? 0 : 2;
        s[0] = sp[0]; s[1] = sp[o1]; s[2] = sp[o2];
        load4(a.rotations + 4 * (size_t)idx, a.rot_aligned16 != 0, q);
    }
    if (PRECOMP) { col_in[0] = a.colors[3 * idx]; col_in[1] = a.colors[3 * idx + 1]; col_in[2] = a.colors[3 * idx + 2]; }
    asm volatile("" ::"v"(x), "v"(y), "v"(z), "v"(opac), "v"(s[0]), "v"(s[1]), "v"(s[2]), "v"(q[0]), "v"(q[1]), "v"(q[2]),
                 "v"(q[3]), "v"(col_in[0]), "v"(col_in[1]), "v"(col_in[2]));
    if (COV) asm volatile("" ::"v"(cov_in[0]), "v"(cov_in[1]), "v"(cov_in[2]), "v"(cov_in[3]), "v"(cov_in[4]), "v"(cov_in[5]));
    pin_cam(c, false);

    PreOut o;
    const bool vis = preprocess_one<COV, PRECOMP>(a, c, idx, x, y, z, cov_in, s, q, col_in, opac, o);
    a.radii[idx] = vis ? o.radius : 0;
    if (a.rect_packed) {
        const uint32_t r4 = (o.rect.x & 0xFFu) | ((o.rect.x >> 16) << 8) | ((o.rect.y & 0xFFu) << 16) | ((o.rect.y >> 16) << 24);
        reinterpret_cast<uint32_t*>(a.rect)[idx] = vis ? r4 : 0u;
    } else {
        a.rect[idx] = vis ? o.rect : make_uint2(0u, 0u);
    }
    a.depth_key[idx] = vis ? o.key : 0xFFFFFFFFu;
    {
        __shared__ float4 s_rec[4][WAVE * 5];
        const int lane = threadIdx.x & 63, wv = threadIdx.x >> 6, wave_first = idx - lane;
        if (wave_first + WAVE <= a.P) {
            const unsigned long long vm = __builtin_amdgcn_ballot_w64(vis);
            float4* mine = s_rec[wv] + lane * 5;
            mine[0] = o.r0; mine[1] = o.r1; mine[2] = o.r2; mine[3] = o.r3;
            float4* base = reinterpret_cast<float4*>(a.rec + (size_t)wave_first * REC_FLOATS);
#pragma unroll
            for (int k = 0; k < 4; ++k) {
                const int src = (lane >> 2) + 16 * k;
                const float4 v = s_rec[wv][src * 5 + (lane & 3)];
                if ((vm >> src) & 1ull) base[k * WAVE + lane] = v;
            }
        } else if (vis) {
            float4* rec = reinterpret_cast<float4*>(a.rec + (size_t)idx * REC_FLOATS);
            rec[0] = o.r0; rec[1] = o.r1; rec[2] = o.r2; rec[3] = o.r3;
        }
    }
    if (a.grad_acc) {
        const float4 z4 = make_float4(0.f, 0.f, 0.f, 0.f);
        const int lane = threadIdx.x & 63, wave_first = idx - lane;
        if (wave_first + WAVE <= a.P) {
            const unsigned long long vm = __builtin_amdgcn_ballot_w64(vis);
            float4* base = reinterpret_cast<float4*>(a.grad_acc + (size_t)wave_first * GRAD_FLOATS);
#pragma unroll
            for (int k = 0; k < 4; ++k)
                if ((vm >> ((lane >> 2) + 16 * k)) & 1ull) base[k * WAVE + lane] = z4;
        } else if (vis) {
            float4* ga = reinterpret_cast<float4*>(a.grad_acc + (size_t)idx * GRAD_FLOATS);
            ga[0] = z4; ga[1] = z4; ga[2] = z4; ga[3] = z4;
        }
    }
}

int launch_preprocess_forward(const mgs_camera& cam, int P, const float* means3D, const float* shs,
                              const float* colors_precomp, const float* opacities, const float* scales,
                              const float* rotations, const float* cov3D_precomp, const GeometryState& g,
                              int32_t* radii, float* prepare_grad_acc, hipStream_t s) {
    PreArgs a;
    a.means3D = means3D; a.shs = shs; a.colors = colors_precomp; a.opacities = opacities;
    a.scales = scales; a.rotations = rotations; a.cov3D = cov3D_precomp;
    a.V = cam.viewmatrix; a.PM = cam.projmatrix; a.campos = cam.campos;
    a.rec = g.rec; a.depth_key = g.depth_key;
    a.grad_acc = prepare_grad_acc;
    a.rot_aligned16 = rotations && ((size_t)rotations % 16 == 0);
    a.clamped = g.clamped; a.rect = g.rect; a.radii = radii;
    a.tanfovx = cam.tanfovx; a.tanfovy = cam.tanfovy;
    a.focal_x = (float)cam.image_width / (2.0f * cam.tanfovx);
    a.focal_y = (float)cam.image_height / (2.0f * cam.tanfovy);
    a.mod = cam.scale_modifier;
    a.iso = cam.scale_dim == 1;
    a.P = P; a.W = cam.image_width; a.H = cam.image_height;
    a.gx = tiles_x(a.W); a.gy = tiles_y(a.H); a.deg = cam.sh_degree; a.M = cam.sh_coeffs;
    if (P == 0) return 0;
    a.rect_packed = depth_sort_payload(P, cam.image_width, cam.image_height) ? 1 : 0;
    radix_depth_zero_region(g.sort_temp, (uint64_t)P, &a.zero_ptr, &a.zero_words);
    a.zero_words += (size_t)((char*)a.zero_ptr - (char*)g.scan_status) / 4;
    a.zero_ptr = (uint32_t*)g.scan_status;
    const dim3 grid((P + 255) / 256), block(256);
    if (cov3D_precomp && colors_precomp) hipLaunchKernelGGL((preprocess_forward_kernel<true, true>), grid, block, 0, s, a);
    else if (cov3D_precomp) hipLaunchKernelGGL((preprocess_forward_kernel<true, false>), grid, block, 0, s, a);
    else if (colors_precomp) hipLaunchKernelGGL((preprocess_forward_kernel<false, true>), grid, block, 0, s, a);
    else hipLaunchKernelGGL((preprocess_forward_kernel<false, false>), grid, block, 0, s, a);
    MGS_HIP(hipGetLastError());
    return 0;
}

struct BwdArgs {
    GeomBackwardArgs g;
    const float *V, *PM, *PR, *campos;
    const float* rec;
    const uint8_t* clamped;
    float tanfovx, tanfovy, focal_x, focal_y, mod;
    int P, W, H, deg, M;
    int iso;
    int rot_aligned16, drot_aligned16;
};

__device__ __forceinline__ float wave_sum(float v) {
#pragma unroll
    for (int o = 32; o > 0; o >>= 1) v += __shfl_xor(v, o, 64);
    return v;
}

template <bool SH, bool COV>
__global__ void __launch_bounds__(256) geom_backward_kernel(BwdArgs a) {
    const int idx = blockIdx.x * 256 + threadIdx.x;
    float tau[6] = {0.f, 0.f, 0.f, 0.f, 0.f, 0.f};
    const bool in = idx < a.P;
    const size_t ci = in ? (size_t)idx : 0;
    Cam c;
    load_cam(c, a.V, a.PM, a.PR, a.campos);
    c.tanfovx = a.tanfovx; c.tanfovy = a.tanfovy; c.focal_x = a.focal_x; c.focal_y = a.focal_y;
    const int rad = a.g.radii[ci];
    const float x = a.g.means3D[3 * ci], y = a.g.means3D[3 * ci + 1], z = a.g.means3D[3 * ci + 2];
    const float opq = a.g.opacities[ci];
    __shared__ float4 s_ga[4][WAVE * 5];
    const int lane_ = threadIdx.x & 63, wv_ = threadIdx.x >> 6, wave_first = idx - lane_;
    const bool full_wave = wave_first + WAVE <= a.P;
    const float4* gsrc = full_wave ? reinterpret_cast<const float4*>(a.g.grad_acc + (size_t)wave_first * GRAD_FLOATS) + lane_
                                   : reinterpret_cast<const float4*>(a.g.grad_acc + ci * GRAD_FLOATS);
    const int gstep = full_wave ? WAVE : 1;
    const float4 t0 = gsrc[0], t1 = gsrc[gstep], t2 = gsrc[2 * gstep], t3 = gsrc[3 * gstep];
    float cov[6] = {0.f, 0.f, 0.f, 0.f, 0.f, 0.f}, Mm[9];
    float s[3] = {0.f, 0.f, 0.f}, q[4] = {1.f, 0.f, 0.f, 0.f};
    if (COV) {
#pragma unroll
        for (int k = 0; k < 6; ++k) cov[k] = a.g.cov3D_precomp[6 * ci + k];
        asm volatile("" ::"v"(cov[0]), "v"(cov[1]), "v"(cov[2]), "v"(cov[3]), "v"(cov[4]), "v"(cov[5]));
    } else {
        const float* sp = a.g.scales + (a.iso ? ci : 3 * ci);
        const int o1 = a.iso ? 0 : 1, o2 = a.iso ? 0 : 2;
        s[0] = sp[0]; s[1] = sp[o1]; s[2] = sp[o2];
        load4(a.g.rotations + 4 * ci, a.rot_aligned16 != 0, q);
        asm volatile("" ::"v"(s[0]), "v"(s[1]), "v"(s[2]), "v"(q[0]), "v"(q[1]), "v"(q[2]), "v"(q[3]));
    }
    asm volatile("" ::"v"(rad), "v"(x), "v"(y), "v"(z), "v"(opq));
    float4 ga0 = t0, ga1 = t1, ga2 = t2;
    if (full_wave) {
        float4* row = s_ga[wv_] + (lane_ >> 2) * 5 + (lane_ & 3);
        row[0] = t0; row[16 * 5] = t1; row[32 * 5] = t2; row[48 * 5] = t3;
        ga0 = s_ga[wv_][lane_ * 5 + 0]; ga1 = s_ga[wv_][lane_ * 5 + 1]; ga2 = s_ga[wv_][lane_ * 5 + 2];
    }
    pin_cam(c, true);
    const float ga[GRAD_FLOATS] = {ga0.x, ga0.y, ga0.z, ga0.w, ga1.x, ga1.y, ga1.z, ga1.w, ga2.x, ga2.y, 0.f, 0.f, 0.f, 0.f, 0.f, 0.f};
    const bool live = in && rad > 0;
    float o_m2[2] = {0.f, 0.f}, o_m3[3] = {0.f, 0.f, 0.f}, o_col[3] = {0.f, 0.f, 0.f}, o_sc[3] = {0.f, 0.f, 0.f};
    float o_rot[4] = {0.f, 0.f, 0.f, 0.f}, o_cov[6] = {0.f, 0.f, 0.f, 0.f, 0.f, 0.f}, o_opac = 0.f, o_siso = 0.f;
    if (in && !live && a.g.dL_dsh) for (int k = 0; k < a.M * 3; ++k) a.g.dL_dsh[(size_t)idx * a.M * 3 + k] = 0.f;
    if (live) {
        float pv[3];
#pragma unroll
        for (int k = 0; k < 3; ++k) pv[k] = dot3p(c.V[k], c.V[4 + k], c.V[8 + k], c.V[12 + k], x, y, z);
        if (!COV) cov3d_from_scale_rot(s, q, a.mod, cov, Mm);
        Proj p;
        project_cov(c, pv, cov, p);

        const float det_q = p.cxx * p.cyy - p.cxy * p.cxy;
        const float det_inv_q = 1.f / det_q;
        const float qa = p.cyy * det_inv_q, qb = -p.cxy * det_inv_q, qc = p.cxx * det_inv_q;
        const float gA = -0.5f * opq * ga[G_SXX], gBh = 0.5f * (-opq * ga[G_SXY]), gC = -0.5f * opq * ga[G_SYY];
        const float n00 = gA * qa + gBh * qb, n01 = gA * qb + gBh * qc;
        const float n10 = gBh * qa + gC * qb, n11 = gBh * qb + gC * qc;
        const float m00 = -(qa * n00 + qb * n10);
        const float m01 = -(qa * n01 + qb * n11);
        const float m11 = -(qb * n01 + qc * n11);

        float A0[3], A1[3];
#pragma unroll
        for (int j = 0; j < 3; ++j) {
            A0[j] = m00 * p.T0[j] + m01 * p.T1[j];
            A1[j] = m01 * p.T0[j] + m11 * p.T1[j];
        }
        float Gs[3][3];
#pragma unroll
        for (int i = 0; i < 3; ++i)
#pragma unroll
            for (int j = 0; j < 3; ++j) Gs[i][j] = p.T0[i] * A0[j] + p.T1[i] * A1[j];
        const float S[3][3] = {{cov[0], cov[1], cov[2]}, {cov[1], cov[3], cov[4]}, {cov[2], cov[4], cov[5]}};
        float dT0[3], dT1[3];
#pragma unroll
        for (int j = 0; j < 3; ++j) {
            dT0[j] = 2.f * ((A0[0] * S[0][j] + A0[1] * S[1][j]) + A0[2] * S[2][j]);
            dT1[j] = 2.f * ((A1[0] * S[0][j] + A1[1] * S[1][j]) + A1[2] * S[2][j]);
        }
        const float dJ00 = (dT0[0] * c.V[0] + dT0[1] * c.V[4]) + dT0[2] * c.V[8];
        const float dJ02 = (dT0[0] * c.V[2] + dT0[1] * c.V[6]) + dT0[2] * c.V[10];
        const float dJ11 = (dT1[0] * c.V[1] + dT1[1] * c.V[5]) + dT1[2] * c.V[9];
        const float dJ12 = (dT1[0] * c.V[2] + dT1[1] * c.V[6]) + dT1[2] * c.V[10];
        float dRv[3][3];
#pragma unroll
        for (int j = 0; j < 3; ++j) {
            dRv[0][j] = p.J00 * dT0[j];
            dRv[1][j] = p.J11 * dT1[j];
            dRv[2][j] = p.J02 * dT0[j] + p.J12 * dT1[j];
        }
        const float tz = p.tz, itz = 1.f / tz, itz2 = itz * itz, itz3 = itz2 * itz;
        float gpc[3];
        gpc[0] = p.clamp_x ? 0.f : -c.focal_x * itz2 * dJ02;
        gpc[1] = p.clamp_y ? 0.f : -c.focal_y * itz2 * dJ12;
        gpc[2] = -c.focal_x * itz2 * dJ00 - c.focal_y * itz2 * dJ11 + 2.f * c.focal_x * p.tx * itz3 * dJ02 +
                 2.f * c.focal_y * p.ty * itz3 * dJ12;

        const float gpx = -opq * (qa * ga[G_SX] + qb * ga[G_SY]);
        const float gpy = -opq * (qc * ga[G_SY] + qb * ga[G_SX]);
        const float gnx = gpx * 0.5f * (float)a.W, gny = gpy * 0.5f * (float)a.H;
        o_m2[0] = gnx; o_m2[1] = gny;
        float ph[4];
#pragma unroll
        for (int k = 0; k < 4; ++k) ph[k] = dot3p(c.PM[k], c.PM[4 + k], c.PM[8 + k], c.PM[12 + k], x, y, z);
        const float p_w = 1.0f / (ph[3] + 0.0000001f);
        const float dph[4] = {gnx * p_w, gny * p_w, 0.f, -(gnx * ph[0] + gny * ph[1]) * p_w * p_w};
#pragma unroll
        for (int j = 0; j < 3; ++j)
            gpc[j] += ((dph[0] * c.PR[4 * j] + dph[1] * c.PR[4 * j + 1]) + dph[2] * c.PR[4 * j + 2]) +
                      dph[3] * c.PR[4 * j + 3];
        gpc[2] += ga[G_DDEPTH];

        float gmean_w[3] = {0.f, 0.f, 0.f};
        if (!SH) {
            if (a.g.dL_dcolors) { o_col[0] = ga[G_DR]; o_col[1] = ga[G_DG]; o_col[2] = ga[G_DB]; }
        } else {
            float gc[3] = {ga[G_DR], ga[G_DG], ga[G_DB]};
#pragma unroll
            for (int ch = 0; ch < 3; ++ch) if (a.clamped[4 * idx + ch]) gc[ch] = 0.f;
            float dv[3] = {x - c.campos[0], y - c.campos[1], z - c.campos[2]};
            const float len2 = (dv[0] * dv[0] + dv[1] * dv[1]) + dv[2] * dv[2];
            const float len = sqrtf(len2), ilen = 1.f / len;
            const float dx = dv[0] * ilen, dy = dv[1] * ilen, dz = dv[2] * ilen;
            const float* sh = a.g.shs + (size_t)idx * a.M * 3;
            float* dsh = a.g.dL_dsh ? a.g.dL_dsh + (size_t)idx * a.M * 3 : nullptr;
            float gdir[3] = {0.f, 0.f, 0.f};
            const int deg = a.deg;
            if (dsh) for (int k = (deg + 1) * (deg + 1) * 3; k < a.M * 3; ++k) dsh[k] = 0.f;
#pragma unroll
            for (int ch = 0; ch < 3; ++ch) {
                const float g = gc[ch];
                if (dsh) dsh[ch] = SH_C0 * g;
                if (deg > 0) {
                    if (dsh) { dsh[3 + ch] = -SH_C1 * dy * g; dsh[6 + ch] = SH_C1 * dz * g; dsh[9 + ch] = -SH_C1 * dx * g; }
                    float gx_ = -SH_C1 * sh[9 + ch], gy_ = -SH_C1 * sh[3 + ch], gz_ = SH_C1 * sh[6 + ch];
                    if (deg > 1) {
                        const float xx = dx * dx, yy = dy * dy, zz = dz * dz, xy = dx * dy, yz = dy * dz, xz = dx * dz;
                        if (dsh) {
                            dsh[12 + ch] = SH_C2[0] * xy * g; dsh[15 + ch] = SH_C2[1] * yz * g;
                            dsh[18 + ch] = SH_C2[2] * (2.f * zz - xx - yy) * g;
                            dsh[21 + ch] = SH_C2[3] * xz * g; dsh[24 + ch] = SH_C2[4] * (xx - yy) * g;
                        }
                        gx_ += SH_C2[0] * dy * sh[12 + ch] + SH_C2[2] * 2.f * -dx * sh[18 + ch] + SH_C2[3] * dz * sh[21 + ch] + SH_C2[4] * 2.f * dx * sh[24 + ch];
                        gy_ += SH_C2[0] * dx * sh[12 + ch] + SH_C2[1] * dz * sh[15 + ch] + SH_C2[2] * 2.f * -dy * sh[18 + ch] + SH_C2[4] * 2.f * -dy * sh[24 + ch];
                        gz_ += SH_C2[1] * dy * sh[15 + ch] + SH_C2[2] * 2.f * 2.f * dz * sh[18 + ch] + SH_C2[3] * dx * sh[21 + ch];
                        if (deg > 2) {
                            if (dsh) {
                                dsh[27 + ch] = SH_C3[0] * dy * (3.f * xx - yy) * g; dsh[30 + ch] = SH_C3[1] * xy * dz * g;
                                dsh[33 + ch] = SH_C3[2] * dy * (4.f * zz - xx - yy) * g;
                                dsh[36 + ch] = SH_C3[3] * dz * (2.f * zz - 3.f * xx - 3.f * yy) * g;
                                dsh[39 + ch] = SH_C3[4] * dx * (4.f * zz - xx - yy) * g;
                                dsh[42 + ch] = SH_C3[5] * dz * (xx - yy) * g; dsh[45 + ch] = SH_C3[6] * dx * (xx - 3.f * yy) * g;
                            }
                            gx_ += SH_C3[0] * sh[27 + ch] * 3.f * 2.f * xy + SH_C3[1] * sh[30 + ch] * yz +
                                   SH_C3[2] * sh[33 + ch] * -2.f * xy + SH_C3[3] * sh[36 + ch] * -3.f * 2.f * xz +
                                   SH_C3[4] * sh[39 + ch] * (-3.f * xx + 4.f * zz - yy) + SH_C3[5] * sh[42 + ch] * 2.f * xz +
                                   SH_C3[6] * sh[45 + ch] * 3.f * (xx - yy);
                            gy_ += SH_C3[0] * sh[27 + ch] * 3.f * (xx - yy) + SH_C3[1] * sh[30 + ch] * xz +
                                   SH_C3[2] * sh[33 + ch] * (-3.f * yy + 4.f * zz - xx) + SH_C3[3] * sh[36 + ch] * -3.f * 2.f * yz +
                                   SH_C3[4] * sh[39 + ch] * -2.f * xy + SH_C3[5] * sh[42 + ch] * -2.f * yz +
                                   SH_C3[6] * sh[45 + ch] * -3.f * 2.f * xy;
                            gz_ += SH_C3[1] * sh[30 + ch] * xy + SH_C3[2] * sh[33 + ch] * 4.f * 2.f * yz +
                                   SH_C3[3] * sh[36 + ch] * 3.f * (2.f * zz - xx - yy) + SH_C3[4] * sh[39 + ch] * 4.f * 2.f * xz +
                                   SH_C3[5] * sh[42 + ch] * (xx - yy);
                        }
                    }
                    gdir[0] += gx_ * g; gdir[1] += gy_ * g; gdir[2] += gz_ * g;
                }
            }
            const float dg = (dx * gdir[0] + dy * gdir[1]) + dz * gdir[2];
            gmean_w[0] = (gdir[0] - dx * dg) * ilen;
            gmean_w[1] = (gdir[1] - dy * dg) * ilen;
            gmean_w[2] = (gdir[2] - dz * dg) * ilen;
#pragma unroll
            for (int i = 0; i < 3; ++i)
                tau[i] += (c.V[i] * gmean_w[0] + c.V[4 + i] * gmean_w[1]) + c.V[8 + i] * gmean_w[2];
        }
        o_opac = ga[G_SH];

        if (a.g.dL_dmeans3D) {
#pragma unroll
            for (int j = 0; j < 3; ++j)
                o_m3[j] = ((c.V[4 * j] * gpc[0] + c.V[4 * j + 1] * gpc[1]) + c.V[4 * j + 2] * gpc[2]) + gmean_w[j];
        }
        tau[0] += gpc[0]; tau[1] += gpc[1]; tau[2] += gpc[2];
        tau[3] += pv[1] * gpc[2] - pv[2] * gpc[1];
        tau[4] += pv[2] * gpc[0] - pv[0] * gpc[2];
        tau[5] += pv[0] * gpc[1] - pv[1] * gpc[0];
#pragma unroll
        for (int j = 0; j < 3; ++j) {
            const float r0 = c.V[4 * j], r1_ = c.V[4 * j + 1], r2 = c.V[4 * j + 2];
            tau[3] += r1_ * dRv[2][j] - r2 * dRv[1][j];
            tau[4] += r2 * dRv[0][j] - r0 * dRv[2][j];
            tau[5] += r0 * dRv[1][j] - r1_ * dRv[0][j];
        }

        if (COV) {
            o_cov[0] = Gs[0][0]; o_cov[1] = 2.f * Gs[0][1]; o_cov[2] = 2.f * Gs[0][2];
            o_cov[3] = Gs[1][1]; o_cov[4] = 2.f * Gs[1][2]; o_cov[5] = Gs[2][2];
        } else {
            float dM[9];
#pragma unroll
            for (int i = 0; i < 3; ++i)
#pragma unroll
                for (int j = 0; j < 3; ++j)
                    dM[3 * i + j] = 2.f * ((Gs[i][0] * Mm[j] + Gs[i][1] * Mm[3 + j]) + Gs[i][2] * Mm[6 + j]);
            const float r = q[0], qx = q[1], qy = q[2], qz = q[3];
            const float Rm[9] = {1.f - 2.f * (qy * qy + qz * qz), 2.f * (qx * qy - r * qz), 2.f * (qx * qz + r * qy),
                                 2.f * (qx * qy + r * qz), 1.f - 2.f * (qx * qx + qz * qz), 2.f * (qy * qz - r * qx),
                                 2.f * (qx * qz - r * qy), 2.f * (qy * qz + r * qx), 1.f - 2.f * (qx * qx + qy * qy)};
            const float sm[3] = {s[0] * a.mod, s[1] * a.mod, s[2] * a.mod};
            if (a.g.dL_dscales) {
                float ds[3];
#pragma unroll
                for (int j = 0; j < 3; ++j)
                    ds[j] = a.mod * ((dM[j] * Rm[j] + dM[3 + j] * Rm[3 + j]) + dM[6 + j] * Rm[6 + j]);
                if (a.iso) o_siso = (ds[0] + ds[1]) + ds[2];
                else { o_sc[0] = ds[0]; o_sc[1] = ds[1]; o_sc[2] = ds[2]; }
            }
            if (a.g.dL_drotations) {
                float dR[9];
#pragma unroll
                for (int i = 0; i < 3; ++i)
#pragma unroll
                    for (int j = 0; j < 3; ++j) dR[3 * i + j] = dM[3 * i + j] * sm[j];
                const float dr = 2.f * (qz * (dR[3] - dR[1]) + qy * (dR[2] - dR[6]) + qx * (dR[7] - dR[5]));
                const float dqx = 2.f * (qy * (dR[1] + dR[3]) + qz * (dR[2] + dR[6]) + r * (dR[7] - dR[5])) -
                                  4.f * qx * (dR[4] + dR[8]);
                const float dqy = 2.f * (qx * (dR[1] + dR[3]) + r * (dR[2] - dR[6]) + qz * (dR[5] + dR[7])) -
                                  4.f * qy * (dR[0] + dR[8]);
                const float dqz = 2.f * (r * (dR[3] - dR[1]) + qx * (dR[2] + dR[6]) + qy * (dR[5] + dR[7])) -
                                  4.f * qz * (dR[0] + dR[4]);
                o_rot[0] = dr; o_rot[1] = dqx; o_rot[2] = dqy; o_rot[3] = dqz;
            }
        }
    }
    if (in) {
        if (a.g.dL_dopacity) a.g.dL_dopacity[idx] = o_opac;
        if (a.g.dL_dscales && a.iso) a.g.dL_dscales[idx] = o_siso;
        if (a.g.dL_drotations) {
            float* o = a.g.dL_drotations + 4 * (size_t)idx;
            if (a.drot_aligned16) *reinterpret_cast<float4*>(o) = make_float4(o_rot[0], o_rot[1], o_rot[2], o_rot[3]);
            else { o[0] = o_rot[0]; o[1] = o_rot[1]; o[2] = o_rot[2]; o[3] = o_rot[3]; }
        }
        if (COV && a.g.dL_dcov3D) {
            float* o = a.g.dL_dcov3D + 6 * (size_t)idx;
#pragma unroll
            for (int k = 0; k < 6; ++k) o[k] = o_cov[k];
        }
    }
    if (in) {
        struct F3 { float x, y, z; };
        auto store3 = [&](float* __restrict__ out, float v0, float v1, float v2) {
            if (out) *reinterpret_cast<F3*>(out + 3 * (size_t)idx) = F3{v0, v1, v2};
        };
        store3(a.g.dL_dmeans2D, o_m2[0], o_m2[1], 0.f);
        store3(a.g.dL_dmeans3D, o_m3[0], o_m3[1], o_m3[2]);
        store3(a.g.dL_dcolors, o_col[0], o_col[1], o_col[2]);
        if (!a.iso) store3(a.g.dL_dscales, o_sc[0], o_sc[1], o_sc[2]);
    }
    if (a.g.dL_dtau) {
        __shared__ float part[4][6];
        const int lane = threadIdx.x & 63, wv = threadIdx.x >> 6;
#pragma unroll
        for (int k = 0; k < 6; ++k) {
            const float v = wave_sum(tau[k]);
            if (lane == 0) part[wv][k] = v;
        }
        __syncthreads();
        if (threadIdx.x < 6) {
            const float v = (part[0][threadIdx.x] + part[1][threadIdx.x]) + (part[2][threadIdx.x] + part[3][threadIdx.x]);
            if (v != 0.f) {
                if (a.g.tau_part) atomicAdd(a.g.tau_part + (size_t)(blockIdx.x % TAU_SLOTS) * 16 + threadIdx.x, v);
                else atomicAdd(a.g.dL_dtau + threadIdx.x, v);
            }
        }
    }
}

__global__ void __launch_bounds__(256) tau_finalize_kernel(const float* __restrict__ tau_part, float* __restrict__ dL_dtau) {
    __shared__ float part[4][6];
    const int t = threadIdx.x, lane = t & 63, wv = t >> 6;
    float v[6];
#pragma unroll
    for (int k = 0; k < 6; ++k) v[k] = t < TAU_SLOTS ? tau_part[(size_t)t * 16 + k] : 0.f;
#pragma unroll
    for (int k = 0; k < 6; ++k) {
        const float r = wave_sum(v[k]);
        if (lane == 0) part[wv][k] = r;
    }
    __syncthreads();
    if (t < 6) dL_dtau[t] = (part[0][t] + part[1][t]) + (part[2][t] + part[3][t]);
}

int launch_geom_backward(const mgs_camera& cam, int P, const GeometryState& g, const GeomBackwardArgs& ga,
                         hipStream_t s) {
    BwdArgs a;
    a.g = ga;
    a.V = cam.viewmatrix; a.PM = cam.projmatrix; a.PR = cam.projmatrix_raw; a.campos = cam.campos;
    a.rec = g.rec; a.clamped = g.clamped;
    a.tanfovx = cam.tanfovx; a.tanfovy = cam.tanfovy;
    a.focal_x = (float)cam.image_width / (2.0f * cam.tanfovx);
    a.focal_y = (float)cam.image_height / (2.0f * cam.tanfovy);
    a.mod = cam.scale_modifier;
    a.iso = cam.scale_dim == 1;
    a.P = P; a.W = cam.image_width; a.H = cam.image_height; a.deg = cam.sh_degree; a.M = cam.sh_coeffs;
    if (P == 0) return 0;
    a.rot_aligned16 = ga.rotations && ((size_t)ga.rotations % 16 == 0);
    a.drot_aligned16 = ga.dL_drotations && ((size_t)ga.dL_drotations % 16 == 0);
    const dim3 grid((P + 255) / 256), block(256);
    const bool cov = ga.cov3D_precomp != nullptr;
    if (ga.colors_precomp && cov) hipLaunchKernelGGL((geom_backward_kernel<false, true>), grid, block, 0, s, a);
    else if (ga.colors_precomp) hipLaunchKernelGGL((geom_backward_kernel<false, false>), grid, block, 0, s, a);
    else if (cov) hipLaunchKernelGGL((geom_backward_kernel<true, true>), grid, block, 0, s, a);
    else hipLaunchKernelGGL((geom_backward_kernel<true, false>), grid, block, 0, s, a);
    if (ga.tau_part && ga.dL_dtau) hipLaunchKernelGGL(tau_finalize_kernel, dim3(1), dim3(256), 0, s, ga.tau_part, ga.dL_dtau);
    MGS_HIP(hipGetLastError());
    return 0;
}

__global__ void mark_visible_kernel(int P, const float* means3D, const float* V, uint8_t* visible) {
    const int idx = blockIdx.x * 256 + threadIdx.x;
    if (idx >= P) return;
    const float x = means3D[3 * idx], y = means3D[3 * idx + 1], z = means3D[3 * idx + 2];
    const float vz = dot3p(V[2], V[6], V[10], V[14], x, y, z);
    visible[idx] = vz > 0.2f;
}

int launch_mark_visible(int P, const float* means3D, const float* viewmatrix, uint8_t* visible, hipStream_t s) {
    if (P == 0) return 0;
    hipLaunchKernelGGL(mark_visible_kernel, dim3((P + 255) / 256), dim3(256), 0, s, P, means3D, viewmatrix, visible);
    MGS_HIP(hipGetLastError());
    return 0;
}

}
```

### monogs_amd/csrc/radix_sort.hip

```cpp
#include "common.h"

namespace mgs {

#ifdef RS_TRACE
__device__ uint64_t* g_rs_trace = nullptr;
#define RS_STAMP(k) do { if (g_rs_trace && threadIdx.x == 0) g_rs_trace[(size_t)blockIdx.x * 8 + (k)] = wall_clock64(); } while (0)
#define RS_DRAIN() asm volatile("s_waitcnt vmcnt(0) lgkmcnt(0)" ::: "memory")
__device__ uint64_t* g_rs_htrace = nullptr;
#define RS_HSTAMP(k) do { if (g_rs_htrace && threadIdx.x == 0) g_rs_htrace[(size_t)blockIdx.x * 4 + (k)] = wall_clock64(); } while (0)
#else
#define RS_HSTAMP(k)
#define RS_STAMP(k)
#define RS_DRAIN()
#endif

constexpr int RS_THREADS = 256;
constexpr int RS_WAVES = RS_THREADS / WAVE;
constexpr int RS_ITEMS = 16;
constexpr int RS_ITEMS_WIDE = 12;
constexpr int RS_ITEMS_MID = 8;
constexpr int RS_ITEMS_SMALL = 4;
constexpr uint64_t RS_ONE_SWEEP_MAX = 512ull * 1024;
static inline int rs_items(uint64_t n) {
    return n <= 192ull * 1024 ? RS_ITEMS_SMALL : (n <= RS_ONE_SWEEP_MAX ? RS_ITEMS_MID : RS_ITEMS);
}
constexpr int RS_MAX_RADIX = 512;
constexpr int RS_MAX_PASSES = 4;
constexpr uint64_t RS_FLAG_LOCAL = 1ull << 62;
constexpr uint64_t RS_FLAG_GLOBAL = 2ull << 62;
constexpr uint64_t RS_COUNT_MASK = (1ull << 62) - 1;
constexpr uint32_t RS_SPIN_LIMIT = 1u << 22;
__device__ uint32_t g_rs_spin_limit = RS_SPIN_LIMIT;
constexpr uint32_t RS_GROUP = 16;

constexpr uint32_t RS_DEPTH_SUB = 0x3E4CCCCDu;
constexpr uint32_t RS_DEPTH_NARROW = (1u << 27) - 1u;
__device__ __forceinline__ uint32_t rs_xf(uint32_t k, uint32_t sub) { return k == 0xFFFFFFFFu ? k : k - sub; }

int g_opt_radix_scanned = -1;
int g_opt_radix_ballot_rank = 0;
int g_opt_radix_xcd_band = 1;
constexpr uint64_t RS_SCANNED_MIN = 64ull * 1024;
static inline bool rs_scanned(uint64_t n) {
    if (g_opt_radix_scanned >= 0) return g_opt_radix_scanned == 1 && n > RS_SCANNED_MIN;
    return n > RS_ONE_SWEEP_MAX;
}
int g_opt_radix_tile_items = 0;
static inline int rs_tile_items(uint64_t n, bool scanned) {
    if (!scanned) return rs_items(n);
    if (g_opt_radix_tile_items == RS_ITEMS_MID || g_opt_radix_tile_items == RS_ITEMS_WIDE || g_opt_radix_tile_items == RS_ITEMS)
        return g_opt_radix_tile_items;
    return n > 1024ull * RS_THREADS * RS_ITEMS ? RS_ITEMS_WIDE : RS_ITEMS;
}
static inline uint32_t rs_tiles(uint64_t n, bool scanned) {
    const uint64_t tile = (uint64_t)RS_THREADS * rs_tile_items(n, scanned);
    return (uint32_t)((n + tile - 1) / tile);
}
static inline uint32_t rs_tiles(uint64_t n) { return rs_tiles(n, rs_scanned(n)); }

struct RsPlan {
    int npasses;
    int shift[RS_MAX_PASSES];
    int db[RS_MAX_PASSES];
    int radix;
    uint32_t sub;
    bool depth;
};
static inline RsPlan rs_plan_plain(int bits) {
    RsPlan pl;
    pl.npasses = (bits + 7) / 8;
    for (int p = 0; p < RS_MAX_PASSES; ++p) { pl.shift[p] = 8 * p; pl.db[p] = 8; }
    pl.radix = 256; pl.sub = 0u; pl.depth = false;
    return pl;
}
static inline RsPlan rs_plan_depth() {
    RsPlan pl;
    pl.npasses = 4;
    for (int p = 0; p < 3; ++p) { pl.shift[p] = 9 * p; pl.db[p] = 9; }
    pl.shift[3] = 27; pl.db[3] = 8;
    pl.radix = 512; pl.sub = RS_DEPTH_SUB; pl.depth = true;
    return pl;
}

static inline RsPlan rs_plan_for_depth(uint64_t n) { return rs_scanned(n) ? rs_plan_depth() : rs_plan_plain(32); }

constexpr int RS_FAN_LOG = 2;
constexpr int RS_TOP_BATCH = 8;
constexpr int RS_MAX_LEVELS = 6;
struct RsTree {
    int levels;
    uint32_t rows[RS_MAX_LEVELS];
    uint32_t off[RS_MAX_LEVELS];
    uint32_t sum_rows;
};
static inline RsTree rs_tree(uint32_t tiles) {
    RsTree tr;
    tr.levels = 1; tr.rows[0] = tiles; tr.off[0] = 0; tr.sum_rows = 0;
    while (tr.rows[tr.levels - 1] > (uint32_t)RS_TOP_BATCH && tr.levels < RS_MAX_LEVELS) {
        tr.rows[tr.levels] = (tr.rows[tr.levels - 1] + (1u << RS_FAN_LOG) - 1u) >> RS_FAN_LOG;
        tr.off[tr.levels] = tr.sum_rows;
        tr.sum_rows += tr.rows[tr.levels];
        ++tr.levels;
    }
    return tr;
}

static inline size_t rs_status_rows(uint32_t tiles) { return (size_t)tiles + (tiles + RS_GROUP - 1) / RS_GROUP; }
struct RsTemp {
    uint32_t* hist;
    uint32_t* tickets;
    uint32_t* error;
    uint32_t* wide;
    uint64_t* status;
    uint32_t* sums;
    uint32_t* counts;
    size_t zero_bytes;
    size_t bytes;
};
static RsTemp rs_carve(void* temp, uint64_t n, const RsPlan& pl, bool scanned) {
    char* p = (char*)align_up((size_t)temp, 256);
    RsTemp t;
    t.hist = (uint32_t*)p;
    t.tickets = t.hist + RS_MAX_PASSES * pl.radix;
    t.error = t.tickets + RS_MAX_PASSES;
    t.wide = t.error + RS_MAX_PASSES;
    char* q = (char*)align_up((size_t)(t.wide + 1), 256);
    t.status = (uint64_t*)q;
    t.sums = (uint32_t*)q;
    const uint32_t tiles = rs_tiles(n, scanned);
    if (scanned) {
        const size_t sums_bytes = (size_t)pl.npasses * rs_tree(tiles).sum_rows * pl.radix * sizeof(uint32_t);
        t.counts = (uint32_t*)(q + sums_bytes);
        t.zero_bytes = (size_t)(q - p) + sums_bytes;
        t.bytes = t.zero_bytes + (size_t)tiles * pl.radix * sizeof(uint32_t);
    } else {
        t.counts = nullptr;
        t.zero_bytes = (size_t)(q - p) + (size_t)pl.npasses * rs_status_rows(tiles) * pl.radix * sizeof(uint64_t);
        t.bytes = t.zero_bytes;
    }
    return t;
}
static size_t rs_temp_bytes(uint64_t n, const RsPlan& pl) {
    if (n == 0) return 256;
    const size_t a = rs_carve(nullptr, n, pl, false).bytes;
    const size_t b = n > RS_SCANNED_MIN ? rs_carve(nullptr, n, pl, true).bytes : 0;
    return (a > b ? a : b) + 512;
}
size_t radix_temp_bytes(uint64_t n, int bits) { return rs_temp_bytes(n, rs_plan_plain(bits)); }
size_t radix_depth_temp_bytes(uint64_t n) {
    const size_t a = rs_temp_bytes(n, rs_plan_depth()), b = rs_temp_bytes(n, rs_plan_plain(32));
    return a > b ? a : b;
}


struct RsHistArgs {
    int npasses, radix;
    int shift[RS_MAX_PASSES], mask[RS_MAX_PASSES];
    uint32_t sub;
    uint32_t* wide;
};
__global__ void __launch_bounds__(RS_THREADS) rs_hist_kernel(const uint32_t* __restrict__ keys, uint32_t n,
                                                             const uint32_t* __restrict__ n_dev, RsHistArgs h,
                                                             uint32_t* __restrict__ hist) {
    __shared__ uint32_t lh[RS_WAVES][RS_MAX_PASSES * RS_MAX_RADIX];
    if (n_dev) n = min(n, n_dev[0]);
    const int words = h.npasses * h.radix;
    for (int w = 0; w < RS_WAVES; ++w)
        for (int i = threadIdx.x; i < words; i += RS_THREADS) lh[w][i] = 0;
    __syncthreads();
    const int wv = threadIdx.x >> 6;
    bool far = false;
    for (uint32_t i = blockIdx.x * RS_THREADS + threadIdx.x; i < n; i += gridDim.x * RS_THREADS) {
        const uint32_t k = keys[i], x = rs_xf(k, h.sub);
        far |= k != 0xFFFFFFFFu && x >= RS_DEPTH_NARROW;
        for (int p = 0; p < h.npasses; ++p) atomicAdd(&lh[wv][p * h.radix + ((x >> h.shift[p]) & h.mask[p])], 1u);
    }
    if (h.wide && far) atomicOr(h.wide, 1u);
    __syncthreads();
    for (int i = threadIdx.x; i < words; i += RS_THREADS) {
        uint32_t c = 0;
#pragma unroll
        for (int w = 0; w < RS_WAVES; ++w) c += lh[w][i];
        if (c) atomicAdd(hist + i, c);
    }
}

struct RsTreeArgs {
    int levels;
    uint32_t off[RS_MAX_LEVELS];
    uint32_t top_rows;
};
struct RsTileHistArgs {
    const uint32_t* keys;
    uint32_t n;
    const uint32_t* n_dev;
    int shift;
    uint32_t sub;
    uint32_t tiles;
    RsTreeArgs tr;
    uint32_t* counts;
    uint32_t* sums;
    uint32_t* wide;
    int detect;
    int only_if_wide;
};
template <int ITEMS, int TPW, int DB>
__global__ void __launch_bounds__(RS_THREADS * TPW) rs_tile_hist_kernel(RsTileHistArgs a) {
    static_assert(TPW == 1 || TPW == (1 << RS_FAN_LOG), "a workgroup counts one tile or one level-1 node");
    constexpr int RADIX = 1 << DB, DPT = RADIX / RS_THREADS, COPIES = 16 / DPT;
    constexpr uint32_t TILE_PAIRS = RS_THREADS * ITEMS;
    __shared__ uint32_t wh[TPW][COPIES][RADIX];
    const int t = threadIdx.x & (RS_THREADS - 1), q = threadIdx.x >> 8, wv = t >> 6, lane = t & 63;
    if (a.only_if_wide && a.wide[0] == 0u) return;
    RS_HSTAMP(0);
    const uint32_t n_live = a.n_dev ? min(a.n, a.n_dev[0]) : a.n;
    if (a.tr.levels > 1 && (uint64_t)blockIdx.x * TPW * TILE_PAIRS >= n_live) return;
    const uint32_t tile = blockIdx.x * TPW + q, tile_start = tile * TILE_PAIRS;
    const uint32_t tile_n = tile_start < n_live ? min(TILE_PAIRS, n_live - tile_start) : 0u;
    uint32_t k[ITEMS];
#pragma unroll
    for (int i = 0; i < ITEMS; ++i) {
        const uint32_t e = (uint32_t)i * RS_THREADS + t;
        k[i] = e < tile_n ? a.keys[tile_start + e] : 0xFFFFFFFFu;
    }
#pragma unroll
    for (int i = 0; i < COPIES; ++i)
#pragma unroll
        for (int j = 0; j < DPT; ++j) wh[q][i][t * DPT + j] = 0;
    __syncthreads();
    RS_DRAIN();
    RS_HSTAMP(1);
    uint32_t* mine = wh[q][wv * (COPIES / RS_WAVES) + (lane & (COPIES / RS_WAVES - 1))];
    bool far = false;
#pragma unroll
    for (int i = 0; i < ITEMS; ++i) {
        const uint32_t x = rs_xf(k[i], a.sub);
        far |= k[i] != 0xFFFFFFFFu && x >= RS_DEPTH_NARROW;
        if ((uint32_t)i * RS_THREADS + t < tile_n) atomicAdd(&mine[(x >> a.shift) & (RADIX - 1)], 1u);
    }
    if (a.detect && far) atomicOr(a.wide, 1u);
    __syncthreads();
    RS_HSTAMP(2);
    uint32_t c[DPT];
#pragma unroll
    for (int j = 0; j < DPT; ++j) {
        c[j] = 0;
#pragma unroll
        for (int i = 0; i < COPIES; ++i) c[j] += wh[q][i][t * DPT + j];
        if (tile < a.tiles) a.counts[(size_t)tile * RADIX + t * DPT + j] = c[j];
    }
    if (TPW == 1) {
#pragma unroll
        for (int j = 0; j < DPT; ++j)
            if (c[j])
                for (int l = 1; l < a.tr.levels; ++l)
                    atomicAdd(a.sums + ((size_t)a.tr.off[l] + (tile >> (RS_FAN_LOG * l))) * RADIX + t * DPT + j, c[j]);
    } else if (a.tr.levels > 1) {
        __syncthreads();
#pragma unroll
        for (int j = 0; j < DPT; ++j) wh[q][0][t * DPT + j] = c[j];
        __syncthreads();
        if (q == 0) {
#pragma unroll
            for (int j = 0; j < DPT; ++j) {
                uint32_t s1 = 0;
#pragma unroll
                for (int m = 0; m < TPW; ++m) s1 += wh[m][0][t * DPT + j];
                a.sums[((size_t)a.tr.off[1] + blockIdx.x) * RADIX + t * DPT + j] = s1;
                if (s1)
                    for (int l = 2; l < a.tr.levels; ++l)
                        atomicAdd(a.sums + ((size_t)a.tr.off[l] + (blockIdx.x >> (RS_FAN_LOG * (l - 1)))) * RADIX + t * DPT + j, s1);
            }
        }
    }
    RS_DRAIN();
    RS_HSTAMP(3);
}
template <int ITEMS, int DB>
static void rs_launch_tile_hist(const RsTileHistArgs& a, hipStream_t s) {
    if (a.tiles >= 1024u)
        hipLaunchKernelGGL((rs_tile_hist_kernel<ITEMS, 4, DB>), dim3((a.tiles + 3) / 4), dim3(RS_THREADS * 4), 0, s, a);
    else
        hipLaunchKernelGGL((rs_tile_hist_kernel<ITEMS, 1, DB>), dim3(a.tiles), dim3(RS_THREADS), 0, s, a);
}

struct RsPassArgs {
    const uint32_t* kin;
    const uint32_t* vin;
    const uint32_t* pin;
    uint32_t* kout;
    uint32_t* vout;
    uint32_t* pout;
    uint32_t* vfinal;
    uint32_t* kfinal;
    const uint2* aux_in;
    uint2* aux_out;
    int aux_skip_ones;
    uint32_t n;
    const uint32_t* n_dev;
    int shift;
    uint32_t sub;
    const uint32_t* hist;
    uint64_t* status;
    uint32_t tiles;
    uint32_t* ticket;
    uint32_t* error;
    int pass;
    int xcd_band;
    int last;
    int cond;
    const uint32_t* wide;
    uint2* ranges;
    const uint32_t* counts;
    const uint32_t* sums;
    RsTreeArgs tree;
};

template <int ITEMS>
__device__ __forceinline__ void rs_exchange(uint32_t* __restrict__ sbuf, const uint32_t (&slot)[ITEMS], uint32_t (&x)[ITEMS], int t) {
#pragma unroll
    for (int i = 0; i < ITEMS; ++i)
        if (slot[i] != 0xFFFFFFFFu) sbuf[slot[i]] = x[i];
    __syncthreads();
#pragma unroll
    for (int i = 0; i < ITEMS; ++i) x[i] = sbuf[min((uint32_t)i * RS_THREADS + (uint32_t)t, (uint32_t)(RS_THREADS * ITEMS - 1))];
}

template <int DPT>
__device__ __forceinline__ void rs_digit_bases(const uint32_t (&hcount)[DPT], uint32_t (&gdigit_base)[DPT], uint32_t* wsum, int lane, int wv) {
    uint32_t hsum = 0;
#pragma unroll
    for (int j = 0; j < DPT; ++j) hsum += hcount[j];
    const uint32_t hincl = wave_incl_scan_dpp(hsum);
    __syncthreads();
    if (lane == 63) wsum[wv] = hincl;
    __syncthreads();
    uint32_t hadd = 0;
    for (int w = 0; w < wv; ++w) hadd += wsum[w];
    uint32_t run = hadd + hincl - hsum;
#pragma unroll
    for (int j = 0; j < DPT; ++j) { gdigit_base[j] = run; run += hcount[j]; }
}

__device__ __forceinline__ bool rs_gather(const uint64_t* row, size_t stride, uint32_t cnt, uint32_t& pre, uint32_t& spins,
                                          uint32_t* err) {
    constexpr uint32_t G = RS_GROUP;
    for (uint32_t r0 = 0; r0 < cnt; r0 += G) {
        uint64_t w[G];
        bool ready;
        do {
#pragma unroll
            for (uint32_t q = 0; q < G; ++q) {
                const uint32_t r = r0 + q;
                w[q] = r < cnt ? __hip_atomic_load(row + (size_t)r * stride, __ATOMIC_RELAXED, __HIP_MEMORY_SCOPE_AGENT)
                                              : RS_FLAG_GLOBAL;
            }
            ready = true;
#pragma unroll
            for (uint32_t q = 0; q < G; ++q) ready &= (w[q] >> 62) != 0ull;
            if (!ready) {
                if (++spins > g_rs_spin_limit) { atomicExch(err, 1u); return false; }
                __builtin_amdgcn_s_sleep(1);
            }
        } while (!ready);
#pragma unroll
        for (uint32_t q = 0; q < G; ++q) pre += (uint32_t)(w[q] & RS_COUNT_MASK);
    }
    return true;
}

template <int ITEMS, int DB, bool SCANNED, bool PAYLOAD, bool BALLOT, bool VIDX>
__global__ void __launch_bounds__(RS_THREADS, (SCANNED && ITEMS == RS_ITEMS_WIDE && DB == 8 && !PAYLOAD) ? 7 : 1) rs_pass_kernel(RsPassArgs a) {
    constexpr int TILE_PAIRS = RS_THREADS * ITEMS;
    constexpr int RADIX = 1 << DB, DPT = RADIX / RS_THREADS;
    constexpr int SBUF = (SCANNED && 2 * RS_WAVES * RADIX > TILE_PAIRS) ? 2 * RS_WAVES * RADIX : TILE_PAIRS;
    __shared__ uint32_t wave_hist[RS_WAVES][RADIX];
    __shared__ uint32_t digit_base[RADIX];
    __shared__ uint32_t gbase[RADIX];
    __shared__ uint32_t sbuf[SBUF];
    __shared__ uint32_t wsum[RS_WAVES];
    __shared__ uint32_t s_tile;

    const int t = threadIdx.x, lane = t & 63, wv = t >> 6;
    const bool wide = a.wide ? a.wide[0] != 0u : false;
    if (a.cond == 2 && !wide) return;
    RS_STAMP(0);
    const bool final_pass = a.cond == 0 ? a.last != 0 : (a.cond == 1 ? !wide : true);
    if (!SCANNED) {
        uint32_t failed = 0;
        for (int q = 0; q < a.pass; ++q) failed |= a.error[q];
        if (failed) return;
    }
    const uint32_t n_live = a.n_dev ? min(a.n, a.n_dev[0]) : a.n;
    if (t == 0) {
        uint32_t id = blockIdx.x;
        if (a.xcd_band) {
            const uint32_t live = (n_live + (uint32_t)TILE_PAIRS - 1) / (uint32_t)TILE_PAIRS;
            const uint32_t q = live >> 3, r = live & 7u, x = id & 7u, j = id >> 3;
            id = j < q + (x < r ? 1u : 0u) ? x * q + min(x, r) + j : 0xFFFFFFFFu;
        }
        s_tile = (!SCANNED && a.ticket) ? atomicAdd(a.ticket, 1u) : id;
    }
#pragma unroll
    for (int w = 0; w < RS_WAVES; ++w)
#pragma unroll
        for (int j = 0; j < DPT; ++j) wave_hist[w][t * DPT + j] = 0;
    __syncthreads();
    const uint32_t tile = s_tile;
    if (tile == 0xFFFFFFFFu) return;
    const uint32_t tile_start = tile * (uint32_t)TILE_PAIRS;
    if (tile_start >= n_live) return;
    const uint32_t tile_n = min((uint32_t)TILE_PAIRS, n_live - tile_start);

    uint32_t hcount[DPT], before[DPT];
#pragma unroll
    for (int j = 0; j < DPT; ++j) hcount[j] = before[j] = 0;
    constexpr int R4 = RADIX / 4;
    uint4 lv[RS_MAX_LEVELS - 1][DPT], tv[RS_TOP_BATCH / RS_WAVES][DPT];
    uint32_t lw[RS_MAX_LEVELS - 1], tw[RS_TOP_BATCH / RS_WAVES], tb[RS_TOP_BATCH / RS_WAVES];
    const int levels = a.tree.levels;
    const uint32_t top_node = tile >> (RS_FAN_LOG * (levels - 1));
    const uint4* __restrict__ c4 = reinterpret_cast<const uint4*>(a.counts);
    const uint4* __restrict__ top4 = levels == 1 ? c4 : reinterpret_cast<const uint4*>(a.sums) + (size_t)a.tree.off[levels - 1] * R4;
    if (SCANNED) {
#pragma unroll
        for (int l = 0; l < RS_MAX_LEVELS - 1; ++l) {
            const bool have = l < levels - 1;
            const uint32_t node = tile >> (RS_FAN_LOG * l), first = node & ~3u, nb = node & 3u;
            const uint4* base = (l == 0 || !have) ? c4 : reinterpret_cast<const uint4*>(a.sums) + (size_t)a.tree.off[l] * R4;
            lw[l] = (have && (uint32_t)wv < nb) ? 1u : 0u;
#pragma unroll
            for (int j = 0; j < DPT; ++j) lv[l][j] = base[(size_t)(lw[l] ? first + (uint32_t)wv : 0u) * R4 + j * WAVE + lane];
        }
#pragma unroll
        for (int q = 0; q < RS_TOP_BATCH / RS_WAVES; ++q) {
            const uint32_t r = (uint32_t)wv + 4u * q;
            tw[q] = r < a.tree.top_rows ? 1u : 0u;
            tb[q] = r < top_node ? 1u : 0u;
#pragma unroll
            for (int j = 0; j < DPT; ++j) tv[q][j] = top4[(size_t)(tw[q] ? r : 0u) * R4 + j * WAVE + lane];
        }
    } else {
#pragma unroll
        for (int j = 0; j < DPT; ++j) hcount[j] = a.hist[t * DPT + j];
    }

    uint32_t key[ITEMS], val[ITEMS], rank[ITEMS], pay[PAYLOAD ? ITEMS : 1];
#pragma unroll
    for (int i = 0; i < ITEMS; ++i) {
        const uint32_t e = (uint32_t)wv * (ITEMS * WAVE) + (uint32_t)i * WAVE + lane;
        const bool valid = e < tile_n;
        key[i] = valid ? a.kin[tile_start + e] : 0xFFFFFFFFu;
        if constexpr (VIDX) val[i] = tile_start + e;
        else val[i] = valid ? a.vin[tile_start + e] : 0u;
        if constexpr (PAYLOAD) pay[i] = valid ? a.pin[tile_start + e] : 0u;
    }
    if (SCANNED) {
        uint4* part = reinterpret_cast<uint4*>(sbuf);
#pragma unroll
        for (int j = 0; j < DPT; ++j) {
            uint4 ab = make_uint4(0u, 0u, 0u, 0u), at = make_uint4(0u, 0u, 0u, 0u);
#pragma unroll
            for (int l = 0; l < RS_MAX_LEVELS - 1; ++l) {
                ab.x += lw[l] ? lv[l][j].x : 0u; ab.y += lw[l] ? lv[l][j].y : 0u; ab.z += lw[l] ? lv[l][j].z : 0u; ab.w += lw[l] ? lv[l][j].w : 0u;
            }
#pragma unroll
            for (int q = 0; q < RS_TOP_BATCH / RS_WAVES; ++q) {
                at.x += tw[q] ? tv[q][j].x : 0u; at.y += tw[q] ? tv[q][j].y : 0u; at.z += tw[q] ? tv[q][j].z : 0u; at.w += tw[q] ? tv[q][j].w : 0u;
                ab.x += tb[q] ? tv[q][j].x : 0u; ab.y += tb[q] ? tv[q][j].y : 0u; ab.z += tb[q] ? tv[q][j].z : 0u; ab.w += tb[q] ? tv[q][j].w : 0u;
            }
            for (uint32_t r0 = RS_TOP_BATCH; r0 < a.tree.top_rows; r0 += RS_TOP_BATCH)
#pragma unroll
                for (int q = 0; q < RS_TOP_BATCH / RS_WAVES; ++q) {
                    const uint32_t r = r0 + (uint32_t)wv + 4u * q;
                    if (r < a.tree.top_rows) {
                        const uint4 v = top4[(size_t)r * R4 + j * WAVE + lane];
                        at.x += v.x; at.y += v.y; at.z += v.z; at.w += v.w;
                        if (r < top_node) { ab.x += v.x; ab.y += v.y; ab.z += v.z; ab.w += v.w; }
                    }
                }
            part[(wv * 2 + 0) * R4 + j * WAVE + lane] = ab;
            part[(wv * 2 + 1) * R4 + j * WAVE + lane] = at;
        }
    }
    RS_DRAIN();
    RS_STAMP(1);
    if (!BALLOT) {
#pragma unroll
        for (int i = 0; i < ITEMS; ++i) {
            const uint32_t e = (uint32_t)wv * (ITEMS * WAVE) + (uint32_t)i * WAVE + lane;
            const uint32_t d = (rs_xf(key[i], a.sub) >> a.shift) & (RADIX - 1);
            rank[i] = 0;
            if (e < tile_n) rank[i] = __hip_atomic_fetch_add(&wave_hist[wv][d], 1u, __ATOMIC_RELAXED, __HIP_MEMORY_SCOPE_WORKGROUP);
        }
    } else {
        const unsigned long long lt_mask = (1ull << lane) - 1ull;
#pragma unroll
        for (int i = 0; i < ITEMS; ++i) {
            const uint32_t e = (uint32_t)wv * (ITEMS * WAVE) + (uint32_t)i * WAVE + lane;
            const bool valid = e < tile_n;
            const uint32_t d = (rs_xf(key[i], a.sub) >> a.shift) & (RADIX - 1);
            unsigned long long peers = __builtin_amdgcn_ballot_w64(valid);
#pragma unroll
            for (int b = 0; b < DB; ++b) {
                const bool bit = (d >> b) & 1u;
                const unsigned long long bm = __builtin_amdgcn_ballot_w64(valid && bit);
                peers &= bit ? bm : ~bm;
            }
            rank[i] = 0;
            if (valid) {
                const uint32_t prev = wave_hist[wv][d];
                rank[i] = prev + (uint32_t)__popcll(peers & lt_mask);
                if ((peers & lt_mask) == 0ull) wave_hist[wv][d] = prev + (uint32_t)__popcll(peers);
            }
        }
    }
    __syncthreads();
    if (SCANNED) {
#pragma unroll
        for (int j = 0; j < DPT; ++j)
#pragma unroll
            for (int w = 0; w < RS_WAVES; ++w) {
                before[j] += sbuf[(w * 2 + 0) * RADIX + t * DPT + j];
                hcount[j] += sbuf[(w * 2 + 1) * RADIX + t * DPT + j];
            }
    }
    RS_STAMP(2);

    uint32_t total[DPT], tsum = 0;
#pragma unroll
    for (int j = 0; j < DPT; ++j) {
        uint32_t run = 0;
#pragma unroll
        for (int w = 0; w < RS_WAVES; ++w) {
            const uint32_t c = wave_hist[w][t * DPT + j];
            wave_hist[w][t * DPT + j] = run;
            run += c;
        }
        total[j] = run;
        tsum += run;
    }
    const uint32_t incl = wave_incl_scan_dpp(tsum);
    if (lane == 63) wsum[wv] = incl;
    __syncthreads();
    uint32_t wadd = 0;
    for (int w = 0; w < wv; ++w) wadd += wsum[w];
    uint32_t dbase[DPT];
    {
        uint32_t run = wadd + incl - tsum;
#pragma unroll
        for (int j = 0; j < DPT; ++j) { dbase[j] = run; digit_base[t * DPT + j] = run; run += total[j]; }
    }
    uint32_t gdigit_base[DPT];
    if constexpr (SCANNED) {
        rs_digit_bases<DPT>(hcount, gdigit_base, wsum, lane, wv);
#pragma unroll
        for (int j = 0; j < DPT; ++j) gbase[t * DPT + j] = gdigit_base[j] + before[j] - dbase[j];
        __syncthreads();
    } else {
        static_assert(DPT == 1, "the one-sweep path ranks 256 digits");
        constexpr uint32_t G = RS_GROUP;
        const uint32_t live_tiles = (n_live + (uint32_t)TILE_PAIRS - 1) / (uint32_t)TILE_PAIRS;
        const uint32_t grp = tile / G, jin = tile % G;
        const uint32_t members = min(G, live_tiles - grp * G);
        uint64_t* gstat = a.status + (size_t)a.tiles * RADIX;
        rs_digit_bases<DPT>(hcount, gdigit_base, wsum, lane, wv);
        __hip_atomic_store(a.status + (size_t)tile * RADIX + t, RS_FLAG_LOCAL | (uint64_t)total[0], __ATOMIC_RELAXED,
                           __HIP_MEMORY_SCOPE_AGENT);
        uint32_t spins = 0, pre = 0, gpre = 0;
        bool ok = rs_gather(a.status + (size_t)grp * G * RADIX + t, RADIX, jin, pre, spins, a.error + a.pass);
        if (jin == members - 1)
            __hip_atomic_store(gstat + (size_t)grp * RADIX + t, RS_FLAG_GLOBAL | (uint64_t)(pre + total[0]), __ATOMIC_RELAXED,
                               __HIP_MEMORY_SCOPE_AGENT);
        if (ok) ok = rs_gather(gstat + t, RADIX, grp, gpre, spins, a.error + a.pass);
        gbase[t] = gdigit_base[0] + gpre + pre - dbase[0];
        __syncthreads();
    }

    RS_STAMP(3);
#pragma unroll
    for (int i = 0; i < ITEMS; ++i) {
        const uint32_t e = (uint32_t)wv * (ITEMS * WAVE) + (uint32_t)i * WAVE + lane;
        const uint32_t d = (rs_xf(key[i], a.sub) >> a.shift) & (RADIX - 1);
        rank[i] = e < tile_n ? digit_base[d] + wave_hist[wv][d] + rank[i] : 0xFFFFFFFFu;
    }
    rs_exchange<ITEMS>(sbuf, rank, key, t);
    __syncthreads();
    rs_exchange<ITEMS>(sbuf, rank, val, t);
    if constexpr (PAYLOAD) {
        __syncthreads();
        rs_exchange<ITEMS>(sbuf, rank, pay, t);
    }
    RS_STAMP(4);
    uint32_t g[ITEMS];
    bool live[ITEMS];
#pragma unroll
    for (int i = 0; i < ITEMS; ++i) {
        const uint32_t p = (uint32_t)i * RS_THREADS + t;
        live[i] = p < tile_n;
        g[i] = gbase[(rs_xf(key[i], a.sub) >> a.shift) & (RADIX - 1)] + p;
    }
    if (!final_pass) {
#pragma unroll
        for (int i = 0; i < ITEMS; ++i)
            if (live[i]) {
                a.kout[g[i]] = key[i];
                a.vout[g[i]] = val[i];
                if constexpr (PAYLOAD) a.pout[g[i]] = pay[i];
            }
        RS_STAMP(5); RS_DRAIN(); RS_STAMP(6); RS_STAMP(7);
        return;
    }
#pragma unroll
    for (int i = 0; i < ITEMS; ++i)
        if (live[i]) {
            if (a.kfinal) a.kfinal[g[i]] = key[i];
            a.vfinal[g[i]] = val[i];
        }
    if (a.ranges) {
        __shared__ uint32_t s_edge[RS_WAVES * ITEMS];
        if (lane == 63) {
#pragma unroll
            for (int i = 0; i < ITEMS; ++i) s_edge[wv * ITEMS + i] = key[i];
        }
        __syncthreads();
#pragma unroll
        for (int i = 0; i < ITEMS; ++i) {
            const uint32_t p = (uint32_t)i * RS_THREADS + t;
            uint32_t l = (uint32_t)__shfl_up((int)key[i], 1, 64);
            if (lane == 0) l = wv > 0 ? s_edge[(wv - 1) * ITEMS + i] : (i > 0 ? s_edge[(RS_WAVES - 1) * ITEMS + i - 1] : 0xFFFFFFFFu);
            if (p < tile_n && (p == 0 || l != key[i])) {
                atomicMin(&a.ranges[key[i]].x, g[i]);
                if (p > 0)
                    atomicMax(&a.ranges[l].y, gbase[(rs_xf(l, a.sub) >> a.shift) & (RADIX - 1)] + p);
            }
            if (p + 1 == tile_n) atomicMax(&a.ranges[key[i]].y, g[i] + 1u);
        }
    }
    RS_STAMP(5);
    RS_DRAIN();
    RS_STAMP(6);
    if (a.aux_out) {
        uint2* __restrict__ aout = a.aux_out;
        if constexpr (PAYLOAD) {
#pragma unroll
            for (int i = 0; i < ITEMS; ++i)
                if (live[i]) {
                    const uint32_t r = pay[i];
                    aout[g[i]] = key[i] == 0xFFFFFFFFu ? make_uint2(0u, 0u)
                                                       : make_uint2((r & 0xFFu) | ((r & 0xFF00u) << 8), ((r >> 16) & 0xFFu) | ((r >> 24) << 16));
                }
        } else {
            const uint2* __restrict__ ain = a.aux_in;
            uint2 r[ITEMS];
#pragma unroll
            for (int i = 0; i < ITEMS; ++i)
                r[i] = (live[i] && !(a.aux_skip_ones && key[i] == 0xFFFFFFFFu)) ? ain[val[i]] : make_uint2(0u, 0u);
#pragma unroll
            for (int i = 0; i < ITEMS; ++i)
                if (live[i]) aout[g[i]] = r[i];
        }
    }
    RS_DRAIN();
    RS_STAMP(7);
}


bool radix_result_in_b(int bits) { return (rs_plan_plain(bits).npasses & 1) != 0; }

const uint32_t* radix_error_flag(void* temp, uint64_t n, int bits) {
    return rs_carve(temp, n ? n : 1, rs_plan_plain(bits), rs_scanned(n ? n : 1)).error;
}
const uint32_t* radix_depth_error_flag(void* temp, uint64_t n) {
    return rs_carve(temp, n ? n : 1, rs_plan_for_depth(n ? n : 1), rs_scanned(n ? n : 1)).error;
}

void radix_zero_region(void* temp, uint64_t n, int bits, uint32_t** ptr, size_t* words) {
    const RsTemp t = rs_carve(temp, n ? n : 1, rs_plan_plain(bits), rs_scanned(n ? n : 1));
    *ptr = t.hist;
    *words = t.zero_bytes / 4;
}
void radix_depth_zero_region(void* temp, uint64_t n, uint32_t** ptr, size_t* words) {
    const RsTemp t = rs_carve(temp, n ? n : 1, rs_plan_for_depth(n ? n : 1), rs_scanned(n ? n : 1));
    *ptr = t.hist;
    *words = t.zero_bytes / 4;
}

bool radix_wants_hist(uint64_t n) { return n > 0 && !rs_scanned(n); }
bool radix_depth_payload(uint64_t n) { return n > 0 && rs_scanned(n); }

template <int ITEMS, int DB, bool SCANNED, bool PAYLOAD>
static void rs_launch_pass(const RsPassArgs& a, uint32_t tiles, bool ballot, hipStream_t s) {
    if (ballot && DB == 8 && !PAYLOAD && a.vin != nullptr)
        hipLaunchKernelGGL((rs_pass_kernel<ITEMS, 8, SCANNED, false, true, false>), dim3(tiles), dim3(RS_THREADS), 0, s, a);
    else if (a.vin == nullptr && (DB == 9 || !SCANNED))
        hipLaunchKernelGGL((rs_pass_kernel<ITEMS, DB, SCANNED, PAYLOAD, false, (DB == 9 || !SCANNED)>), dim3(tiles), dim3(RS_THREADS), 0, s, a);
    else
        hipLaunchKernelGGL((rs_pass_kernel<ITEMS, DB, SCANNED, PAYLOAD, false, false>), dim3(tiles), dim3(RS_THREADS), 0, s, a);
}
template <int DB, bool PAYLOAD>
static void rs_launch_pass_items(const RsPassArgs& a, int items, bool scanned, uint32_t tiles, bool ballot, hipStream_t s) {
    if (scanned) {
        if (items == RS_ITEMS_WIDE) rs_launch_pass<RS_ITEMS_WIDE, DB, true, PAYLOAD>(a, tiles, ballot, s);
        else if (items == RS_ITEMS_MID) rs_launch_pass<RS_ITEMS_MID, DB, true, PAYLOAD>(a, tiles, ballot, s);
        else rs_launch_pass<RS_ITEMS, DB, true, PAYLOAD>(a, tiles, ballot, s);
    } else if constexpr (!PAYLOAD && DB == 8) {
        if (items == RS_ITEMS_SMALL) rs_launch_pass<RS_ITEMS_SMALL, 8, false, false>(a, tiles, ballot, s);
        else if (items == RS_ITEMS_MID) rs_launch_pass<RS_ITEMS_MID, 8, false, false>(a, tiles, ballot, s);
        else rs_launch_pass<RS_ITEMS, 8, false, false>(a, tiles, ballot, s);
    }
}

struct RsBuffers {
    uint2* ranges;
    uint32_t *ka, *va, *pa;
    bool va_is_index;
    uint32_t *kb, *vb, *pb;
    uint32_t *kfinal, *vfinal;
    const uint2* aux_in;
    uint2* aux_out;
    bool aux_skip_ones;
};
static int rs_run(const RsPlan& pl, const RsBuffers& b, uint64_t n, void* temp, hipStream_t s, const uint32_t* n_dev,
                  bool temp_zeroed, const uint32_t* ext_hist, bool exclusive) {
    if (n == 0) return 0;
    if (n >= (1ull << 32)) { set_error("radix sort: more than 2^32-1 pairs"); return 1; }
    const bool scanned = rs_scanned(n);
    const RsTemp t = rs_carve(temp, n, pl, scanned);
    if (!temp_zeroed) MGS_HIP(zero_fill(t.hist, t.zero_bytes, s));
    const uint32_t tiles = rs_tiles(n, scanned);
    const int items = rs_tile_items(n, scanned);
    const bool payload = b.pa != nullptr;
    if (payload && !scanned) { set_error("radix sort: payloads need the counted-tiles path"); return 1; }
    const RsTree tree = rs_tree(tiles);
    RsTreeArgs ta;
    ta.levels = tree.levels;
    for (int l = 0; l < RS_MAX_LEVELS; ++l) ta.off[l] = l < tree.levels ? tree.off[l] : 0u;
    ta.top_rows = tree.rows[tree.levels - 1];
    if (!scanned && !ext_hist) {
        RsHistArgs h;
        h.npasses = pl.npasses; h.radix = pl.radix; h.sub = pl.sub; h.wide = pl.depth ? t.wide : nullptr;
        for (int p = 0; p < RS_MAX_PASSES; ++p) { h.shift[p] = pl.shift[p]; h.mask[p] = (1 << pl.db[p]) - 1; }
        hipLaunchKernelGGL(rs_hist_kernel, dim3(min(tiles, 1024u)), dim3(RS_THREADS), 0, s, b.ka, (uint32_t)n, n_dev, h, t.hist);
    }
    const uint32_t* ghist = (!scanned && ext_hist) ? ext_hist : t.hist;
    const int hstride = (!scanned && ext_hist) ? 256 : pl.radix;
    const uint32_t *kin = b.ka, *vin = b.va_is_index ? nullptr : b.va, *pin = b.pa;
    uint32_t *kout = b.kb, *vout = b.vb, *pout = b.pb;
    uint32_t *kalt = b.ka, *valt = b.va, *palt = b.pa;
    for (int p = 0; p < pl.npasses; ++p) {
        RsPassArgs a;
        a.kin = kin; a.vin = vin; a.pin = pin; a.kout = kout; a.vout = vout; a.pout = pout;
        a.n = (uint32_t)n; a.n_dev = n_dev; a.shift = pl.shift[p]; a.sub = pl.sub;
        a.hist = ghist + p * hstride;
        a.status = t.status + (size_t)p * rs_status_rows(tiles) * pl.radix;
        a.tiles = tiles;
        a.ticket = (exclusive && tiles <= 256u) ? nullptr : t.tickets + p;
        a.error = t.error;
        a.pass = p;
        a.xcd_band = (scanned && g_opt_radix_xcd_band != 0) ? 1 : 0;
        a.counts = t.counts; a.sums = t.sums + (size_t)p * tree.sum_rows * pl.radix;
        a.tree = ta;
        a.wide = pl.depth ? t.wide : nullptr;
        a.cond = pl.depth ? (p == 2 ? 1 : (p == 3 ? 2 : 0)) : 0;
        a.last = (!pl.depth && p == pl.npasses - 1) ? 1 : 0;
        a.vfinal = b.vfinal ? b.vfinal : vout;
        a.kfinal = b.vfinal ? b.kfinal : kout;
        a.ranges = (!pl.depth && p == pl.npasses - 1) ? b.ranges : nullptr;
        if (a.ranges) a.kfinal = nullptr;
        a.aux_in = b.aux_in; a.aux_out = b.aux_out; a.aux_skip_ones = b.aux_skip_ones ? 1 : 0;
        if (scanned) {
            RsTileHistArgs h;
            h.keys = kin; h.n = (uint32_t)n; h.n_dev = n_dev; h.shift = a.shift; h.sub = pl.sub; h.tiles = tiles; h.tr = ta;
            h.counts = t.counts; h.sums = const_cast<uint32_t*>(a.sums);
            h.wide = t.wide; h.detect = (pl.depth && p == 0) ? 1 : 0; h.only_if_wide = a.cond == 2 ? 1 : 0;
            if (items == RS_ITEMS_WIDE) {
                if (pl.db[p] == 9) rs_launch_tile_hist<RS_ITEMS_WIDE, 9>(h, s); else rs_launch_tile_hist<RS_ITEMS_WIDE, 8>(h, s);
            } else if (items == RS_ITEMS_MID) {
                if (pl.db[p] == 9) rs_launch_tile_hist<RS_ITEMS_MID, 9>(h, s); else rs_launch_tile_hist<RS_ITEMS_MID, 8>(h, s);
            } else {
                if (pl.db[p] == 9) rs_launch_tile_hist<RS_ITEMS, 9>(h, s); else rs_launch_tile_hist<RS_ITEMS, 8>(h, s);
            }
        }
        const bool ballot = g_opt_radix_ballot_rank != 0;
        if (pl.db[p] == 9) {
            if (payload) rs_launch_pass_items<9, true>(a, items, scanned, tiles, ballot, s);
            else rs_launch_pass_items<9, false>(a, items, scanned, tiles, ballot, s);
        } else {
            if (payload) rs_launch_pass_items<8, true>(a, items, scanned, tiles, ballot, s);
            else rs_launch_pass_items<8, false>(a, items, scanned, tiles, ballot, s);
        }
        kin = kout; vin = vout; pin = pout;
        uint32_t* tk = kalt; kalt = kout; kout = tk;
        uint32_t* tv = valt; valt = vout; vout = tv;
        uint32_t* tp = palt; palt = pout; pout = tp;
    }
    MGS_HIP(hipGetLastError());
    return 0;
}

int radix_sort_pairs(uint32_t* ka, uint32_t* va, uint32_t* kb, uint32_t* vb, uint64_t n, int bits, void* temp,
                     hipStream_t s, const uint32_t* n_dev, bool temp_zeroed, const uint2* aux_in, uint2* aux_out,
                     const uint32_t* ext_hist, bool aux_empty_for_ones, bool exclusive, uint2* ranges) {
    const RsPlan pl = rs_plan_plain(bits);
    if (pl.npasses > RS_MAX_PASSES) { set_error("radix sort: more than 32 key bits"); return 1; }
    RsBuffers b;
    b.ranges = ranges;
    b.ka = ka; b.va = va; b.va_is_index = false; b.pa = nullptr; b.kb = kb; b.vb = vb; b.pb = nullptr; b.kfinal = nullptr; b.vfinal = nullptr;
    b.aux_in = aux_in; b.aux_out = aux_out; b.aux_skip_ones = aux_empty_for_ones;
    return rs_run(pl, b, n, temp, s, n_dev, temp_zeroed, ext_hist, exclusive);
}

int radix_sort_depth(uint32_t* keys, uint32_t* key_b, uint32_t* val_a, uint32_t* val_b, void* rect, bool payload,
                     uint32_t* perm, uint2* rect_sorted, uint64_t n, void* temp, hipStream_t s, bool temp_zeroed, bool exclusive) {
    const RsPlan pl = rs_plan_for_depth(n);
    RsBuffers b;
    b.ranges = nullptr;
    b.ka = keys; b.va = val_a; b.va_is_index = true; b.kb = key_b; b.vb = val_b;
    b.pa = payload ? (uint32_t*)rect : nullptr; b.pb = payload ? (uint32_t*)rect + n : nullptr;
    b.kfinal = nullptr; b.vfinal = perm;
    b.aux_in = payload ? nullptr : (const uint2*)rect; b.aux_out = rect_sorted; b.aux_skip_ones = true;
    return rs_run(pl, b, n, temp, s, nullptr, temp_zeroed, nullptr, exclusive);
}

int set_radix_spin_limit(uint32_t limit) {
    const uint32_t v = limit == 0xFFFFFFFFu ? RS_SPIN_LIMIT : limit;
    MGS_HIP(hipMemcpyToSymbol(HIP_SYMBOL(g_rs_spin_limit), &v, sizeof(v)));
    return 0;
}

}
```

### monogs_amd/debug.py

```python
from __future__ import annotations

import ctypes as C

import torch

from . import _lib
from .rasterizer import _camera, _f32, _ptr, _stream, _device_guard


def _au(v, a=256):
    return (v + a - 1) // a * a


def forward_tables(rs, means3D, opacities, colors_precomp=None, shs=None, scales=None, rotations=None,
                   cov3D_precomp=None, between=None):
    lib = _lib.load()
    dev = means3D.device
    P = means3D.shape[0]
    H, W = int(rs.image_height), int(rs.image_width)
    c = lambda t, n: None if t is None else _f32(t.detach(), n)
    means3D, opacities = c(means3D, "means3D"), c(opacities, "opacities")
    colors_precomp, shs, scales = c(colors_precomp, "colors"), c(shs, "shs"), c(scales, "scales")
    rotations, cov3D_precomp = c(rotations, "rotations"), c(cov3D_precomp, "cov3D")
    with _device_guard(dev):
        keep = []
        scale_dim = int(scales.shape[1]) if scales is not None else 3
        if scale_dim not in (1, 3):
            raise Exception("scales must be [P,3] (or [P,1] for an isotropic map)")
        cam = _camera(rs, 0 if shs is None else shs.shape[1], keep, scale_dim)
        u8 = dict(dtype=torch.uint8, device=dev)
        geom = torch.zeros(lib.mgs_geometry_bytes(P), **u8)
        img = torch.zeros(lib.mgs_image_bytes(W, H), **u8)
        radii = torch.empty(P, dtype=torch.int32, device=dev)
        n_touched = torch.empty(P, dtype=torch.int32, device=dev)
        color = torch.empty(3, H, W, dtype=torch.float32, device=dev)
        depth = torch.empty(1, H, W, dtype=torch.float32, device=dev)
        opacity = torch.empty(1, H, W, dtype=torch.float32, device=dev)
        nr = C.c_uint64(0)
        _lib.check(lib.mgs_forward_preprocess(C.byref(cam), P, _ptr(means3D), _ptr(shs), _ptr(colors_precomp),
                                              _ptr(opacities), _ptr(scales), _ptr(rotations), _ptr(cov3D_precomp),
                                              geom.data_ptr(), radii.data_ptr(), None, C.byref(nr), None, None, None, _stream()),
                   "mgs_forward_preprocess")
        R = int(nr.value)
        if between is not None:
            between()
        binning = torch.zeros(lib.mgs_binning_bytes(R, W, H), **u8)
        status = torch.zeros(1, dtype=torch.int32, device=dev)
        _lib.check(lib.mgs_forward_render(C.byref(cam), P, R, geom.data_ptr(), binning.data_ptr(), img.data_ptr(),
                                          color.data_ptr(), depth.data_ptr(), opacity.data_ptr(),
                                          n_touched.data_ptr(), status.data_ptr() if P > 0 else None, None, _stream()),
                   "mgs_forward_render")
        torch.cuda.synchronize()

    def view(buf, off, nbytes, dtype):
        base = _au(buf.data_ptr()) - buf.data_ptr()
        return buf[base + off: base + off + nbytes].view(dtype)

    HW = H * W
    ntiles = ((W + 15) // 16) * ((H + 15) // 16)
    final_T = view(img, 0, HW * 4, torch.float32).reshape(H, W)
    n_contrib = view(img, _au(HW * 4), HW * 4, torch.int32).reshape(H, W)
    ranges = view(img, 2 * _au(HW * 4), ntiles * 8, torch.int32).reshape(ntiles, 2)
    r = max(R, 1)
    tile_bits = max(1, (ntiles - 1).bit_length())
    in_b = ((tile_bits + 7) // 8) % 2 == 1
    rg = ranges.long()
    tile_sorted = torch.repeat_interleave(torch.arange(ntiles, device=ranges.device), (rg[:, 1] - rg[:, 0]).clamp_min(0)).to(torch.int32)
    point_list = view(binning, (3 if in_b else 2) * _au(r * 4), R * 4, torch.int32)
    rec = view(geom, 0, P * 64, torch.float32).reshape(P, 16)
    o = _au(P * 64)
    perm = view(geom, o + 4 * _au(P * 4), P * 4, torch.int32)
    o_rect = o + 6 * _au(P * 4) + _au(((P + 2047) // 2048 + 64) * 4) + _au(P * 4)
    wh_sorted = view(geom, o_rect + _au(P * 8), P * 8, torch.int32).reshape(P, 2)[:, 1]
    tiles_touched = torch.zeros(P, dtype=torch.int32, device=geom.device)
    tiles_touched[perm.long()] = (wh_sorted & 0xFFFF) * ((wh_sorted >> 16) & 0xFFFF)
    depth_key = rec[:, 11].contiguous().view(torch.int32)
    return dict(color=color, depth=depth, opacity=opacity, radii=radii, n_touched=n_touched, num_rendered=R,
                status=int(status.item()),
                final_T=final_T, n_contrib=n_contrib, ranges=ranges, tile_sorted=tile_sorted,
                point_list=point_list, rec=rec, tiles_touched=tiles_touched, depth_key=depth_key, perm=perm)
```

Before: 2572 Mpix/s.

## Replace global depth sort with per-tile depth ordering for large maps

For large Gaussian counts, the global depth radix sort over all Gaussians is skipped. High depth bits are packed into the low bits of the tile key during duplication, so the tile radix sort only sorts on the tile bits, and a new per-tile LDS radix sort kernel then orders entries within each tile by the packed depth bits. Range detection shifts keys to recover tile ids. This removes a full P-sized sort and its scatter, at the cost of an extra per-tile sort pass and more complex key packing that could lose depth precision.

```diff
diff --git a/include/monogs_raster.h b/include/monogs_raster.h
--- a/include/monogs_raster.h
+++ b/include/monogs_raster.h
@@ -8,7 +8,7 @@
 extern "C" {
 #endif
 
-#define MGS_ABI_VERSION 9
+#define MGS_ABI_VERSION 10
 #define MGS_TILE 16
 
 typedef struct mgs_camera {
@@ -80,6 +80,8 @@
 
 int mgs_debug_set_radix_spin_limit(uint32_t limit);
 int mgs_debug_set_option(const char* name, int64_t value);
+
+int mgs_binning_path(int32_t P, int32_t W, int32_t H);
 
 size_t mgs_debug_sort_temp_bytes(uint64_t n, int32_t bits);
 int mgs_debug_sort_pairs(uint32_t* keys, uint32_t* vals, uint32_t* keys_alt, uint32_t* vals_alt, uint64_t n, int32_t bits,
diff --git a/monogs_amd/_lib.py b/monogs_amd/_lib.py
--- a/monogs_amd/_lib.py
+++ b/monogs_amd/_lib.py
@@ -5,7 +5,7 @@
 
 _HERE = os.path.dirname(os.path.abspath(__file__))
 LIB_PATH = os.environ.get("MGS_LIB_PATH") or os.path.join(_HERE, "lib", "libmonogs_raster.so")
-ABI_VERSION = 9
+ABI_VERSION = 10
 
 c_float_p = C.c_void_p
 
@@ -45,6 +45,7 @@
                            + [C.POINTER(MgsTiming), C.c_void_p]),
     "mgs_debug_set_radix_spin_limit": (C.c_int, [C.c_uint32]),
     "mgs_debug_set_option": (C.c_int, [C.c_char_p, C.c_int64]),
+    "mgs_binning_path": (C.c_int, [C.c_int32, C.c_int32, C.c_int32]),
     "mgs_debug_sort_temp_bytes": (C.c_size_t, [C.c_uint64, C.c_int32]),
     "mgs_debug_sort_pairs": (C.c_int, [C.c_void_p] * 4 + [C.c_uint64, C.c_int32, C.c_void_p, C.c_void_p]),
     "mgs_forward_render_capacity": (C.c_int, [C.POINTER(MgsCamera), C.c_int32, C.c_uint64] + [C.c_void_p] * 8
diff --git a/monogs_amd/csrc/api.hip b/monogs_amd/csrc/api.hip
--- a/monogs_amd/csrc/api.hip
+++ b/monogs_amd/csrc/api.hip
@@ -133,6 +133,7 @@
 extern "C" {
 
 int mgs_abi_version(void) { return MGS_ABI_VERSION; }
+int mgs_binning_path(int32_t P, int32_t W, int32_t H) { return binning_path(P, W, H); }
 const char* mgs_last_error(void) { return g_err; }
 
 size_t mgs_geometry_bytes(int32_t P) { return GeometryState::bytes(P < 0 ? 0 : P); }
@@ -183,13 +184,17 @@
                                            prepare_backward ? backward_grad_acc(prepare_backward) : nullptr, s)) return rc;
     tm.mark();
     const bool exclusive = (cam->flags & MGS_FLAG_EXCLUSIVE_DEVICE) != 0;
-    if (depth_chain_is_small(P)) {
+    const bool per_tile = binning_path(P, cam->image_width, cam->image_height) != 0;
+    if (per_tile) {
+        tm.mark();
+        if (int rc = launch_scan(g, P, s, exclusive, g.rect)) return rc;
+    } else if (depth_chain_is_small(P)) {
         if (int rc = launch_depth_chain_small(g, P, s)) return rc;
         tm.mark();
     } else {
         if (int rc = launch_depth_sort(g, P, depth_sort_payload(P, cam->image_width, cam->image_height), s, exclusive)) return rc;
         tm.mark();
-        if (int rc = launch_scan(g, P, s, exclusive)) return rc;
+        if (int rc = launch_scan(g, P, s, exclusive, g.rect_sorted)) return rc;
     }
     tm.mark();
     if (num_rendered) {
@@ -206,7 +211,7 @@
     if (timing) {
         if (!num_rendered) MGS_HIP(hipStreamSynchronize(s));
         timing->preprocess_ms = tm.ms(0);
-        timing->depth_sort_ms = tm.ms(1);
+        timing->depth_sort_ms = per_tile ? 0.f : tm.ms(1);
         timing->scan_ms = tm.ms(2);
     }
     return 0;
@@ -232,11 +237,15 @@
     StageTimer tm(s, timing != nullptr);
     const bool cap = capacity && binning;
     if (cap) n_dev = b.count;
+    const bool per_tile = binning_path(P, W, H) != 0;
     tm.mark();
     if (int rc = launch_duplicate(*cam, P, g, b, capacity ? R : (R > 0 ? 0xFFFFFFFFull : 0ull), n_touched, img, R,
-                                  tile_bits(W, H), cap ? b.count : nullptr, overflow, s)) return rc;
-    tm.mark();
-    if (int rc = launch_sort(g, b, R, tile_bits(W, H), s, n_dev, (cam->flags & MGS_FLAG_EXCLUSIVE_DEVICE) != 0, img.ranges)) return rc;
+                                  tile_bits(W, H), cap ? b.count : nullptr, overflow, s, per_tile)) return rc;
+    tm.mark();
+    if (int rc = launch_sort(g, b, R, tile_bits(W, H), s, n_dev, (cam->flags & MGS_FLAG_EXCLUSIVE_DEVICE) != 0, img.ranges,
+                             per_tile)) return rc;
+    if (per_tile)
+        if (int rc = launch_tile_depth_sort(*cam, P, g, b, img, R, n_dev, s)) return rc;
     tm.mark();
     if (g_dbg_fwd_events[0]) MGS_HIP(hipEventRecord(g_dbg_fwd_events[0], s));
     if (int rc = launch_blend_forward(*cam, g, b, img, out_color, out_depth, out_opacity, n_touched,
diff --git a/monogs_amd/csrc/binning.hip b/monogs_amd/csrc/binning.hip
--- a/monogs_amd/csrc/binning.hip
+++ b/monogs_amd/csrc/binning.hip
@@ -123,17 +123,17 @@
 bool scan_is_small(int P) { return g_opt_scan_small != 0 && scan_nblocks(P) <= SCAN_SMALL_MAX_BLOCKS; }
 
 
-int launch_scan(const GeometryState& g, int P, hipStream_t s, bool exclusive) {
+int launch_scan(const GeometryState& g, int P, hipStream_t s, bool exclusive, const uint2* rects) {
     if (P == 0) return 0;
     const int nb = scan_nblocks(P);
     if (scan_is_small(P)) {
-        hipLaunchKernelGGL(scan_small_kernel, dim3(nb), dim3(SCAN_THREADS), 0, s, g.rect_sorted, g.point_offsets, g.scan_blocks,
+        hipLaunchKernelGGL(scan_small_kernel, dim3(nb), dim3(SCAN_THREADS), 0, s, rects, g.point_offsets, g.scan_blocks,
                            g.scan_status, P, nb, const_cast<uint32_t*>(radix_depth_error_flag(g.sort_temp, (uint64_t)P)),
                            exclusive ? 0 : 1);
         MGS_HIP(hipGetLastError());
         return 0;
     }
-    hipLaunchKernelGGL(scan_local_kernel, dim3(nb), dim3(SCAN_THREADS), 0, s, g.rect_sorted, g.point_offsets,
+    hipLaunchKernelGGL(scan_local_kernel, dim3(nb), dim3(SCAN_THREADS), 0, s, rects, g.point_offsets,
                        g.scan_blocks, P);
     hipLaunchKernelGGL(scan_blocks_kernel, dim3(1), dim3(SCAN_THREADS), 0, s, g.scan_blocks, nb);
     MGS_HIP(hipGetLastError());
@@ -278,8 +278,19 @@
     return 0;
 }
 
+__device__ __forceinline__ void dup_pair(uint32_t gidx, const uint32_t* __restrict__ depth_key, int lo, uint32_t& val,
+                                         uint32_t& kfield) {
+    val = gidx; kfield = 0u;
+    if (depth_key) {
+        const uint32_t k = depth_key[gidx];
+        const uint32_t d = k == 0xFFFFFFFFu ? DEPTH_KEY_NARROW : min(k - DEPTH_KEY_SUB, DEPTH_KEY_NARROW);
+        kfield = d >> lo;
+        if (lo) val |= (d & ((1u << lo) - 1u)) << (32 - lo);
+    }
+}
 __global__ void __launch_bounds__(256) duplicate_kernel(int P, const uint2* __restrict__ rects,
                                                         const uint32_t* __restrict__ perm,
+                                                        const uint32_t* __restrict__ depth_key, int tshift, int lo,
                                                         const uint32_t* __restrict__ offsets ,
                                                         const uint32_t* __restrict__ block_sums ,
                                                         uint32_t* keys,
@@ -303,10 +314,10 @@
         overflow[0] = (count ? count[1] : 0u) | (depth_bad ? (uint32_t)MGS_STATUS_DEPTH_SORT_TIMEOUT : 0u);
     if (i < ntiles) ranges[i] = make_uint2(0xFFFFFFFFu, 0u);
     if (i < P) n_touched[i] = 0;
-    uint32_t idx = 0, nt = 0, off = 0;
+    uint32_t idx = 0, nt = 0, off = 0, kf = 0;
     int x0 = 0, y0 = 0, x1 = 0;
     if (i < P) {
-        idx = perm[i];
+        dup_pair(perm ? perm[i] : (uint32_t)i, depth_key, lo, idx, kf);
         const uint2 r = rects[i];
         const int w = (int)(r.y & 0xFFFFu), h = (int)(r.y >> 16);
         nt = (uint32_t)(w * h);
@@ -315,7 +326,7 @@
     if (depth_bad) nt = 0;
     if (nt) off = i == 0 ? 0u : offsets[i - 1] + (offsets_global ? 0u : block_sums[(i - 1) / SCAN_ITEMS]);
     __shared__ uint32_t s_own[4][WAVE];
-    __shared__ uint32_t s_idx[4][WAVE], s_off[4][WAVE];
+    __shared__ uint32_t s_idx[4][WAVE], s_off[4][WAVE], s_kf[4][WAVE];
     __shared__ int s_x0[4][WAVE], s_y0[4][WAVE], s_w[4][WAVE];
     __shared__ uint32_t s_hist[2][256];
     if (hist) {
@@ -350,7 +361,7 @@
         while (sl < s1 && g < (uint32_t)P) {
             const uint32_t gi = g + (uint32_t)lane;
             const bool valid = gi < (uint32_t)P;
-            uint32_t inc = 0, ntg = 0, idg = 0;
+            uint32_t inc = 0, ntg = 0, idg = 0, kfg = 0;
             int gx0 = 0, gy0 = 0, gw = 1;
             if (valid) {
                 inc = incl(gi);
@@ -358,14 +369,14 @@
                 gw = (int)(r.y & 0xFFFFu);
                 ntg = (uint32_t)(gw * (int)(r.y >> 16));
                 gx0 = (int)(r.x & 0xFFFFu); gy0 = (int)(r.x >> 16);
-                idg = perm[gi];
+                dup_pair(perm ? perm[gi] : gi, depth_key, lo, idg, kfg);
             }
             const uint32_t exc = inc - ntg;
             uint32_t Eg = valid ? inc : 0u;
 #pragma unroll
             for (int o2 = 32; o2 > 0; o2 >>= 1) Eg = max(Eg, (uint32_t)__shfl_xor((int)Eg, o2, 64));
             __builtin_amdgcn_wave_barrier();
-            s_idx[wv][lane] = idg; s_off[wv][lane] = exc; s_x0[wv][lane] = gx0; s_y0[wv][lane] = gy0; s_w[wv][lane] = max(gw, 1);
+            s_idx[wv][lane] = idg; s_kf[wv][lane] = kfg; s_off[wv][lane] = exc; s_x0[wv][lane] = gx0; s_y0[wv][lane] = gy0; s_w[wv][lane] = max(gw, 1);
             const uint32_t e = min(s1, Eg);
             const uint32_t cb0 = sl & ~63u;
             const unsigned long long before = __builtin_amdgcn_ballot_w64(ntg != 0u && exc < cb0);
@@ -389,13 +400,14 @@
                     const uint32_t t = o - s_off[wv][L];
                     const uint32_t w = (uint32_t)s_w[wv][L];
                     const uint32_t yy = t / w, xx = t - yy * w;
-                    const uint32_t key = (uint32_t)((s_y0[wv][L] + (int)yy) * gx + s_x0[wv][L] + (int)xx);
+                    const uint32_t tid = (uint32_t)((s_y0[wv][L] + (int)yy) * gx + s_x0[wv][L] + (int)xx);
+                    const uint32_t key = (tid << tshift) | s_kf[wv][L];
                     keys[o] = key;
                     vals[o] = s_idx[wv][L];
                     if (hist) {
-                        atomicAdd(&s_hist[0][key & 0xFFu], 1u);
+                        atomicAdd(&s_hist[0][(key >> tshift) & 0xFFu], 1u);
                         if (hist_passes > 1) {
-                            const uint32_t d1 = (key >> 8) & 0xFFu;
+                            const uint32_t d1 = (key >> (tshift + 8)) & 0xFFu;
                             const uint32_t lead = (uint32_t)__builtin_amdgcn_readfirstlane((int)d1);
                             const unsigned long long same = __builtin_amdgcn_ballot_w64(d1 == lead);
                             if (d1 != lead) atomicAdd(&s_hist[1][d1], 1u);
@@ -415,7 +427,7 @@
         }
         return;
     }
-    s_idx[wv][lane] = idx; s_off[wv][lane] = off; s_x0[wv][lane] = x0; s_y0[wv][lane] = y0; s_w[wv][lane] = max(x1 - x0, 1);
+    s_idx[wv][lane] = idx; s_kf[wv][lane] = kf; s_off[wv][lane] = off; s_x0[wv][lane] = x0; s_y0[wv][lane] = y0; s_w[wv][lane] = max(x1 - x0, 1);
     const unsigned long long live = __builtin_amdgcn_ballot_w64(nt != 0);
     if (live == 0ull && !hist) return;
     const int first = live ? __builtin_ctzll(live) : 0, lastl = live ? 63 - __builtin_clzll(live) : 0;
@@ -441,13 +453,14 @@
             const uint32_t t = o - s_off[wv][L];
             const uint32_t w = (uint32_t)s_w[wv][L];
             const uint32_t yy = t / w, xx = t - yy * w;
-            const uint32_t key = (uint32_t)((s_y0[wv][L] + (int)yy) * gx + s_x0[wv][L] + (int)xx);
+            const uint32_t tid = (uint32_t)((s_y0[wv][L] + (int)yy) * gx + s_x0[wv][L] + (int)xx);
+            const uint32_t key = (tid << tshift) | s_kf[wv][L];
             keys[o] = key;
             vals[o] = s_idx[wv][L];
             if (hist) {
-                atomicAdd(&s_hist[0][key & 0xFFu], 1u);
+                atomicAdd(&s_hist[0][(key >> tshift) & 0xFFu], 1u);
                 if (hist_passes > 1) {
-                    const uint32_t d1 = (key >> 8) & 0xFFu;
+                    const uint32_t d1 = (key >> (tshift + 8)) & 0xFFu;
                     const uint32_t lead = (uint32_t)__builtin_amdgcn_readfirstlane((int)d1);
                     const unsigned long long same = __builtin_amdgcn_ballot_w64(d1 == lead);
                     if (d1 != lead) atomicAdd(&s_hist[1][d1], 1u);
@@ -469,7 +482,7 @@
 
 int launch_duplicate(const mgs_camera& cam, int P, const GeometryState& g, const BinningState& b, uint64_t r_cap,
                      int32_t* n_touched, const ImageState& img, uint64_t sort_n, int sort_bits, uint32_t* count,
-                     uint32_t* overflow, hipStream_t s) {
+                     uint32_t* overflow, hipStream_t s, bool per_tile) {
     const uint32_t* depth_err = P > 0 ? radix_depth_error_flag(g.sort_temp, (uint64_t)P) : nullptr;
     const int ntiles = tiles_x(cam.image_width) * tiles_y(cam.image_height);
     int n = P > ntiles ? P : ntiles;
@@ -485,10 +498,14 @@
     size_t zero_words = 0;
     if (sort_n > 0) radix_zero_region(b.sort_temp, sort_n, sort_bits, &zero_ptr, &zero_words);
     const bool count_digits = P > 0 && sort_bits <= 16 && radix_wants_hist(sort_n);
-    hipLaunchKernelGGL(duplicate_kernel, dim3(n_threads / 256), dim3(256), 0, s, P, g.rect_sorted, g.perm, g.point_offsets,
+    const int tb = tile_bits(cam.image_width, cam.image_height);
+    hipLaunchKernelGGL(duplicate_kernel, dim3(n_threads / 256), dim3(256), 0, s, P, per_tile ? g.rect : g.rect_sorted,
+                       per_tile ? nullptr : g.perm, per_tile ? g.depth_key : nullptr, per_tile ? 32 - tb : 0,
+                       per_tile ? tile_depth_lo_bits(tb) : 0, g.point_offsets,
                        g.scan_blocks, b.keys_a, b.vals_a, tiles_x(cam.image_width), tiles_y(cam.image_height),
                        (uint32_t)(r_cap > 0xFFFFFFFFull ? 0xFFFFFFFFull : r_cap), n_touched, img.ranges, ntiles, zero_ptr,
-                       zero_words, count, overflow, depth_err, (P > 0 && (scan_is_small(P) || depth_chain_is_small(P))) ? 1 : 0,
+                       zero_words, count, overflow, depth_err,
+                       (P > 0 && (scan_is_small(P) || (!per_tile && depth_chain_is_small(P)))) ? 1 : 0,
                        count_digits ? g.tile_hist : nullptr, (sort_bits + 7) / 8, n_threads, slot_major ? 1 : 0);
     MGS_HIP(hipGetLastError());
     return 0;
@@ -502,12 +519,236 @@
 }
 
 int launch_sort(const GeometryState& g, const BinningState& b, uint64_t R, int bits, hipStream_t s, const uint32_t* n_dev,
-                bool exclusive, uint2* ranges) {
+                bool exclusive, uint2* ranges, bool per_tile) {
     if (R == 0) return 0;
     const bool counted = bits <= 16 && radix_wants_hist(R) && g.tile_hist != nullptr;
     return radix_sort_pairs(b.keys_a, b.vals_a, b.keys_b, b.vals_b, R, bits, b.sort_temp, s, n_dev, true, nullptr, nullptr,
-                            counted ? g.tile_hist : nullptr, false, exclusive, ranges);
-}
-
-
-}
+                            counted ? g.tile_hist : nullptr, false, exclusive, ranges, per_tile ? 32 - bits : 0);
+}
+
+constexpr int TDS_THREADS = 256, TDS_WAVES = TDS_THREADS / WAVE, TDS_ITEMS = 4, TDS_CAP = TDS_THREADS * TDS_ITEMS;
+constexpr int TDS_DB = 9, TDS_RADIX = 1 << TDS_DB, TDS_DPT = TDS_RADIX / TDS_THREADS;
+
+__device__ __forceinline__ void tds_minmax(uint32_t lo, uint32_t hi, uint32_t* s_red , uint32_t& mn,
+                                           uint32_t& mx) {
+    const int lane = threadIdx.x & 63, wv = threadIdx.x >> 6;
+#pragma unroll
+    for (int o = 32; o > 0; o >>= 1) {
+        lo = min(lo, (uint32_t)__shfl_xor((int)lo, o, 64));
+        hi = max(hi, (uint32_t)__shfl_xor((int)hi, o, 64));
+    }
+    if (lane == 0) { s_red[wv] = lo; s_red[TDS_WAVES + wv] = hi; }
+    __syncthreads();
+    mn = s_red[0]; mx = s_red[TDS_WAVES];
+#pragma unroll
+    for (int w = 1; w < TDS_WAVES; ++w) { mn = min(mn, s_red[w]); mx = max(mx, s_red[TDS_WAVES + w]); }
+    __syncthreads();
+}
+
+__device__ __forceinline__ void tds_lds_sort(uint32_t* s_k, uint32_t* s_v, uint32_t (*s_cnt)[TDS_RADIX], uint32_t* s_wsum,
+                                             int base, int m, int bits) {
+    const int t = threadIdx.x, lane = t & 63, wv = t >> 6;
+    for (int sh = 0; sh < bits; sh += TDS_DB) {
+#pragma unroll
+        for (int w = 0; w < TDS_WAVES; ++w)
+#pragma unroll
+            for (int j = 0; j < TDS_DPT; ++j) s_cnt[w][t * TDS_DPT + j] = 0u;
+        __syncthreads();
+        uint32_t k[TDS_ITEMS], v[TDS_ITEMS], r[TDS_ITEMS];
+#pragma unroll
+        for (int i = 0; i < TDS_ITEMS; ++i) {
+            const int e = wv * (TDS_ITEMS * WAVE) + i * WAVE + lane;
+            k[i] = 0u; v[i] = 0u; r[i] = 0u;
+            if (e < m) {
+                k[i] = s_k[base + e]; v[i] = s_v[base + e];
+                r[i] = __hip_atomic_fetch_add(&s_cnt[wv][(k[i] >> sh) & (TDS_RADIX - 1)], 1u, __ATOMIC_RELAXED,
+                                              __HIP_MEMORY_SCOPE_WORKGROUP);
+            }
+        }
+        __syncthreads();
+        uint32_t c[TDS_DPT][TDS_WAVES], tot[TDS_DPT], tsum = 0;
+#pragma unroll
+        for (int j = 0; j < TDS_DPT; ++j) {
+            tot[j] = 0u;
+#pragma unroll
+            for (int w = 0; w < TDS_WAVES; ++w) { c[j][w] = s_cnt[w][t * TDS_DPT + j]; tot[j] += c[j][w]; }
+            tsum += tot[j];
+        }
+        const uint32_t incl = wave_incl_scan_dpp(tsum);
+        if (lane == 63) s_wsum[wv] = incl;
+        __syncthreads();
+        uint32_t run = incl - tsum;
+        for (int w = 0; w < wv; ++w) run += s_wsum[w];
+#pragma unroll
+        for (int j = 0; j < TDS_DPT; ++j)
+#pragma unroll
+            for (int w = 0; w < TDS_WAVES; ++w) { s_cnt[w][t * TDS_DPT + j] = run; run += c[j][w]; }
+        __syncthreads();
+#pragma unroll
+        for (int i = 0; i < TDS_ITEMS; ++i) {
+            const int e = wv * (TDS_ITEMS * WAVE) + i * WAVE + lane;
+            if (e < m) {
+                const uint32_t dst = s_cnt[wv][(k[i] >> sh) & (TDS_RADIX - 1)] + r[i];
+                s_k[base + dst] = k[i]; s_v[base + dst] = v[i];
+            }
+        }
+        __syncthreads();
+    }
+    __syncthreads();
+}
+
+__device__ void tds_global_sort(uint32_t* __restrict__ kx, uint32_t* __restrict__ vx, uint32_t* __restrict__ ky,
+                                uint32_t* __restrict__ vy, uint32_t n, const uint32_t* __restrict__ depth_key, int lo,
+                                uint32_t (*s_cnt)[TDS_RADIX], uint32_t* s_run, uint32_t* s_wsum) {
+    const int t = threadIdx.x, lane = t & 63, wv = t >> 6;
+    const uint32_t imask = lo ? (1u << (32 - lo)) - 1u : 0xFFFFFFFFu;
+    for (uint32_t e = t; e < n; e += TDS_THREADS) {
+        const uint32_t g = vx[e] & imask;
+        kx[e] = depth_key[g] - DEPTH_KEY_SUB;
+        vx[e] = g;
+    }
+    for (int sh = 0; sh < 32; sh += 8) {
+        __threadfence();
+        if (t < 256) s_run[t] = 0u;
+#pragma unroll
+        for (int w = 0; w < TDS_WAVES; ++w) s_cnt[w][t] = 0u;
+        __syncthreads();
+        for (uint32_t e = t; e < n; e += TDS_THREADS) atomicAdd(&s_run[(kx[e] >> sh) & 255u], 1u);
+        __syncthreads();
+        {
+            const uint32_t c = s_run[t], incl = wave_incl_scan_dpp(c);
+            if (lane == 63) s_wsum[wv] = incl;
+            __syncthreads();
+            uint32_t b0 = incl - c;
+            for (int w = 0; w < wv; ++w) b0 += s_wsum[w];
+            s_run[t] = b0;
+        }
+        __syncthreads();
+        for (uint32_t c0 = 0; c0 < n; c0 += TDS_THREADS) {
+            const uint32_t e = c0 + (uint32_t)t;
+            uint32_t k = 0u, v = 0u, r = 0u, d = 0u;
+            if (e < n) {
+                k = kx[e]; v = vx[e]; d = (k >> sh) & 255u;
+                r = __hip_atomic_fetch_add(&s_cnt[wv][d], 1u, __ATOMIC_RELAXED, __HIP_MEMORY_SCOPE_WORKGROUP);
+            }
+            __syncthreads();
+            uint32_t pre[TDS_WAVES];
+            {
+                uint32_t run = s_run[t];
+#pragma unroll
+                for (int w = 0; w < TDS_WAVES; ++w) { const uint32_t c = s_cnt[w][t]; pre[w] = run; run += c; }
+                s_run[t] = run;
+            }
+            __syncthreads();
+#pragma unroll
+            for (int w = 0; w < TDS_WAVES; ++w) s_cnt[w][t] = pre[w];
+            __syncthreads();
+            if (e < n) { const uint32_t dst = s_cnt[wv][d] + r; ky[dst] = k; vy[dst] = v; }
+            __syncthreads();
+#pragma unroll
+            for (int w = 0; w < TDS_WAVES; ++w) s_cnt[w][t] = 0u;
+            __syncthreads();
+        }
+        __threadfence();
+        __syncthreads();
+        uint32_t* tk = kx; kx = ky; ky = tk;
+        uint32_t* tv = vx; vx = vy; vy = tv;
+    }
+}
+
+__global__ void __launch_bounds__(TDS_THREADS) tile_depth_sort_kernel(const uint2* __restrict__ ranges, int ntiles,
+                                                                       uint32_t* __restrict__ keys, uint32_t* __restrict__ vals,
+                                                                       uint32_t* __restrict__ keys_alt, uint32_t* __restrict__ vals_alt,
+                                                                       const uint32_t* __restrict__ depth_key, int tb, uint32_t n_cap,
+                                                                       const uint32_t* __restrict__ n_dev,
+                                                                       const uint32_t* __restrict__ sort_err) {
+    __shared__ uint32_t s_k[TDS_CAP], s_v[TDS_CAP];
+    __shared__ uint32_t s_cnt[TDS_WAVES][TDS_RADIX];
+    __shared__ uint32_t s_wsum[TDS_WAVES], s_red[2 * TDS_WAVES];
+    const int tile = blockIdx.x, t = threadIdx.x, lane = t & 63, wv = t >> 6;
+    if (tile >= ntiles) return;
+    if (sort_err && radix_failed(sort_err) != 0u) return;
+    const uint32_t n_live = n_dev ? min(n_cap, n_dev[0]) : n_cap;
+    const uint2 rg = ranges[tile];
+    const uint32_t start = rg.x, end = min(rg.y, n_live);
+    if (start >= end) return;
+    const uint32_t n = end - start;
+    const int lo = tile_depth_lo_bits(tb);
+    const uint32_t kmask = tb < 32 ? (0xFFFFFFFFu >> tb) : 0u, imask = lo ? (1u << (32 - lo)) - 1u : 0xFFFFFFFFu;
+    if (n > (uint32_t)TDS_CAP) {
+        tds_global_sort(keys + start, vals + start, keys_alt + start, vals_alt + start, n, depth_key, lo, s_cnt, s_k, s_wsum);
+        return;
+    }
+    uint32_t d[TDS_ITEMS], g[TDS_ITEMS];
+    uint32_t dmin = 0xFFFFFFFFu, dmax = 0u;
+#pragma unroll
+    for (int i = 0; i < TDS_ITEMS; ++i) {
+        const uint32_t e = (uint32_t)(wv * (TDS_ITEMS * WAVE) + i * WAVE + lane);
+        d[i] = 0u; g[i] = 0u;
+        if (e < n) {
+            const uint32_t k = keys[start + e], v = vals[start + e];
+            d[i] = ((k & kmask) << lo) | (lo ? v >> (32 - lo) : 0u);
+            g[i] = v & imask;
+            dmin = min(dmin, d[i]); dmax = max(dmax, d[i]);
+        }
+    }
+    uint32_t mn, mx;
+    tds_minmax(dmin, dmax, s_red, mn, mx);
+#pragma unroll
+    for (int i = 0; i < TDS_ITEMS; ++i) {
+        const int e = wv * (TDS_ITEMS * WAVE) + i * WAVE + lane;
+        if (e < (int)n) { s_k[e] = d[i] - mn; s_v[e] = g[i]; }
+    }
+    const uint32_t span = mx - mn;
+    tds_lds_sort(s_k, s_v, s_cnt, s_wsum, 0, (int)n, span ? 32 - __builtin_clz(span) : 0);
+    if (mx == DEPTH_KEY_NARROW) {
+        uint32_t c = 0;
+#pragma unroll
+        for (int i = 0; i < TDS_ITEMS; ++i) {
+            const uint32_t e = (uint32_t)(wv * (TDS_ITEMS * WAVE) + i * WAVE + lane);
+            c += (e < n && d[i] == DEPTH_KEY_NARROW) ? 1u : 0u;
+        }
+#pragma unroll
+        for (int o = 32; o > 0; o >>= 1) c += (uint32_t)__shfl_xor((int)c, o, 64);
+        if (lane == 0) s_red[wv] = c;
+        __syncthreads();
+        uint32_t m = 0;
+#pragma unroll
+        for (int w = 0; w < TDS_WAVES; ++w) m += s_red[w];
+        __syncthreads();
+        const uint32_t f = n - m;
+        uint32_t xmin = 0xFFFFFFFFu, xmax = 0u;
+        for (uint32_t e = f + t; e < n; e += TDS_THREADS) {
+            const uint32_t x = depth_key[s_v[e]] - DEPTH_KEY_SUB;
+            s_k[e] = x;
+            xmin = min(xmin, x); xmax = max(xmax, x);
+        }
+        uint32_t rmn, rmx;
+        tds_minmax(xmin, xmax, s_red, rmn, rmx);
+        for (uint32_t e = f + t; e < n; e += TDS_THREADS) s_k[e] -= rmn;
+        __syncthreads();
+        const uint32_t rspan = rmx - rmn;
+        tds_lds_sort(s_k, s_v, s_cnt, s_wsum, (int)f, (int)m, rspan ? 32 - __builtin_clz(rspan) : 0);
+    }
+#pragma unroll
+    for (int i = 0; i < TDS_ITEMS; ++i) {
+        const int e = wv * (TDS_ITEMS * WAVE) + i * WAVE + lane;
+        if (e < (int)n) vals[start + e] = s_v[e];
+    }
+}
+
+int launch_tile_depth_sort(const mgs_camera& cam, int P, const GeometryState& g, const BinningState& b, const ImageState& img,
+                           uint64_t R, const uint32_t* n_dev, hipStream_t s) {
+    if (R == 0 || P == 0) return 0;
+    const int W = cam.image_width, H = cam.image_height, ntiles = tiles_x(W) * tiles_y(H), tb = tile_bits(W, H);
+    uint32_t* keys_alt = b.keys_sorted == b.keys_a ? b.keys_b : b.keys_a;
+    uint32_t* vals_alt = b.vals_sorted == b.vals_a ? b.vals_b : b.vals_a;
+    hipLaunchKernelGGL(tile_depth_sort_kernel, dim3(ntiles), dim3(TDS_THREADS), 0, s, img.ranges, ntiles, b.keys_sorted,
+                       b.vals_sorted, keys_alt, vals_alt, g.depth_key, tb, (uint32_t)R, n_dev,
+                       radix_error_flag(b.sort_temp, R, tb));
+    MGS_HIP(hipGetLastError());
+    return 0;
+}
+
+
+}
diff --git a/monogs_amd/csrc/common.h b/monogs_amd/csrc/common.h
--- a/monogs_amd/csrc/common.h
+++ b/monogs_amd/csrc/common.h
@@ -144,6 +144,11 @@
     return b == 0 ? 1 : b;
 }
 
+constexpr uint32_t DEPTH_KEY_SUB = 0x3E4CCCCDu;
+constexpr uint32_t DEPTH_KEY_NARROW = (1u << 27) - 1u;
+__host__ __device__ inline int tile_depth_lo_bits(int tb) { return tb > 5 ? tb - 5 : 0; }
+int binning_path(int P, int W, int H);
+
 void set_error(const char* fmt, ...);
 #define MGS_HIP(expr)                                                                     \
     do {                                                                                  \
@@ -164,12 +169,12 @@
 inline float* backward_grad_acc(void* scratch) { return (float*)align_up((size_t)scratch, 256); }
 inline float* backward_tau_part(void* scratch, int P) { return backward_grad_acc(scratch) + (size_t)P * GRAD_FLOATS; }
 inline float* backward_tau_out(void* scratch, int P) { return backward_tau_part(scratch, P) + (size_t)TAU_SLOTS * 16; }
-int launch_scan(const GeometryState& g, int P, hipStream_t s, bool exclusive = false);
+int launch_scan(const GeometryState& g, int P, hipStream_t s, bool exclusive, const uint2* rects);
 bool depth_chain_is_small(int P);
 int launch_depth_chain_small(const GeometryState& g, int P, hipStream_t s);
 int launch_duplicate(const mgs_camera& cam, int P, const GeometryState& g, const BinningState& b, uint64_t r_cap,
                      int32_t* n_touched, const ImageState& img, uint64_t sort_n, int sort_bits, uint32_t* count,
-                     uint32_t* overflow, hipStream_t s);
+                     uint32_t* overflow, hipStream_t s, bool per_tile);
 size_t sort_temp_bytes(uint64_t n, int bits);
 size_t radix_temp_bytes(uint64_t n, int bits);
 size_t radix_depth_temp_bytes(uint64_t n);
@@ -179,14 +184,15 @@
 const uint32_t* radix_depth_error_flag(void* temp, uint64_t n);
 __device__ __forceinline__ uint32_t radix_failed(const uint32_t* __restrict__ e) { return (e[0] | e[1]) | (e[2] | e[3]); }
 void radix_zero_region(void* temp, uint64_t n, int bits, uint32_t** ptr, size_t* words);
-void radix_depth_zero_region(void* temp, uint64_t n, uint32_t** ptr, size_t* words);
+void radix_depth_zero_region(void* temp, uint64_t n, uint32_t** ptr, size_t* words, bool header_only = false);
 int radix_sort_pairs(uint32_t* ka, uint32_t* va, uint32_t* kb, uint32_t* vb, uint64_t n, int bits, void* temp,
                      hipStream_t s, const uint32_t* n_dev = nullptr, bool temp_zeroed = false,
                      const uint2* aux_in = nullptr, uint2* aux_out = nullptr,
                      const uint32_t* ext_hist = nullptr,
                      bool aux_empty_for_ones = false,
                      bool exclusive = false,
-                     uint2* ranges = nullptr);
+                     uint2* ranges = nullptr,
+                     int key_shift = 0);
 bool radix_wants_hist(uint64_t n);
 bool radix_depth_payload(uint64_t n);
 int radix_sort_depth(uint32_t* keys, uint32_t* key_b, uint32_t* val_a, uint32_t* val_b, void* rect, bool payload,
@@ -195,7 +201,9 @@
 inline bool depth_sort_payload(int P, int W, int H) { return radix_depth_payload((uint64_t)P) && tiles_x(W) <= 255 && tiles_y(H) <= 255; }
 int launch_depth_sort(const GeometryState& g, int P, bool payload, hipStream_t s, bool exclusive = false);
 int launch_sort(const GeometryState& g, const BinningState& b, uint64_t R, int bits, hipStream_t s,
-                const uint32_t* n_dev = nullptr, bool exclusive = false, uint2* ranges = nullptr);
+                const uint32_t* n_dev = nullptr, bool exclusive = false, uint2* ranges = nullptr, bool per_tile = false);
+int launch_tile_depth_sort(const mgs_camera& cam, int P, const GeometryState& g, const BinningState& b, const ImageState& img,
+                           uint64_t R, const uint32_t* n_dev, hipStream_t s);
 int set_radix_spin_limit(uint32_t limit);
 extern int g_opt_radix_ballot_rank, g_opt_radix_scanned, g_opt_radix_xcd_band, g_opt_radix_tile_items, g_opt_knn_grid_min, g_opt_scan_small, g_opt_dup_slot_major, g_opt_blend_bwd_transposed, g_opt_blend_lds_pad_fwd, g_opt_blend_lds_pad_bwd, g_opt_depth_small;
 int launch_blend_forward(const mgs_camera& cam, const GeometryState& g, const BinningState& b,
diff --git a/monogs_amd/csrc/preprocess.hip b/monogs_amd/csrc/preprocess.hip
--- a/monogs_amd/csrc/preprocess.hip
+++ b/monogs_amd/csrc/preprocess.hip
@@ -350,8 +350,9 @@
     a.P = P; a.W = cam.image_width; a.H = cam.image_height;
     a.gx = tiles_x(a.W); a.gy = tiles_y(a.H); a.deg = cam.sh_degree; a.M = cam.sh_coeffs;
     if (P == 0) return 0;
-    a.rect_packed = depth_sort_payload(P, cam.image_width, cam.image_height) ? 1 : 0;
-    radix_depth_zero_region(g.sort_temp, (uint64_t)P, &a.zero_ptr, &a.zero_words);
+    const bool per_tile = binning_path(P, cam.image_width, cam.image_height) != 0;
+    a.rect_packed = (!per_tile && depth_sort_payload(P, cam.image_width, cam.image_height)) ? 1 : 0;
+    radix_depth_zero_region(g.sort_temp, (uint64_t)P, &a.zero_ptr, &a.zero_words, per_tile);
     a.zero_words += (size_t)((char*)a.zero_ptr - (char*)g.scan_status) / 4;
     a.zero_ptr = (uint32_t*)g.scan_status;
     const dim3 grid((P + 255) / 256), block(256);
diff --git a/monogs_amd/csrc/radix_sort.hip b/monogs_amd/csrc/radix_sort.hip
--- a/monogs_amd/csrc/radix_sort.hip
+++ b/monogs_amd/csrc/radix_sort.hip
@@ -33,8 +33,8 @@
 __device__ uint32_t g_rs_spin_limit = RS_SPIN_LIMIT;
 constexpr uint32_t RS_GROUP = 16;
 
-constexpr uint32_t RS_DEPTH_SUB = 0x3E4CCCCDu;
-constexpr uint32_t RS_DEPTH_NARROW = (1u << 27) - 1u;
+constexpr uint32_t RS_DEPTH_SUB = DEPTH_KEY_SUB;
+constexpr uint32_t RS_DEPTH_NARROW = DEPTH_KEY_NARROW;
 __device__ __forceinline__ uint32_t rs_xf(uint32_t k, uint32_t sub) { return k == 0xFFFFFFFFu ? k : k - sub; }
 
 int g_opt_radix_scanned = -1;
@@ -44,6 +44,14 @@
 static inline bool rs_scanned(uint64_t n) {
     if (g_opt_radix_scanned >= 0) return g_opt_radix_scanned == 1 && n > RS_SCANNED_MIN;
     return n > RS_ONE_SWEEP_MAX;
+}
+
+int binning_path(int P, int W, int H) {
+    if (P <= 0) return 0;
+    const bool large = g_opt_radix_scanned >= 0 ? g_opt_radix_scanned == 1 : (uint64_t)P > RS_ONE_SWEEP_MAX;
+    const int tb = tile_bits(W, H);
+    if (!large || tb > 16) return 0;
+    return (uint64_t)P <= (1ull << (32 - tile_depth_lo_bits(tb))) ? 1 : 0;
 }
 int g_opt_radix_tile_items = 0;
 static inline int rs_tile_items(uint64_t n, bool scanned) {
@@ -308,6 +316,7 @@
     int pass;
     int xcd_band;
     int last;
+    int range_shift;
     int cond;
     const uint32_t* wide;
     uint2* ranges;
@@ -629,12 +638,13 @@
             const uint32_t p = (uint32_t)i * RS_THREADS + t;
             uint32_t l = (uint32_t)__shfl_up((int)key[i], 1, 64);
             if (lane == 0) l = wv > 0 ? s_edge[(wv - 1) * ITEMS + i] : (i > 0 ? s_edge[(RS_WAVES - 1) * ITEMS + i - 1] : 0xFFFFFFFFu);
-            if (p < tile_n && (p == 0 || l != key[i])) {
-                atomicMin(&a.ranges[key[i]].x, g[i]);
+            const uint32_t kr = key[i] >> a.range_shift, lr = l >> a.range_shift;
+            if (p < tile_n && (p == 0 || lr != kr)) {
+                atomicMin(&a.ranges[kr].x, g[i]);
                 if (p > 0)
-                    atomicMax(&a.ranges[l].y, gbase[(rs_xf(l, a.sub) >> a.shift) & (RADIX - 1)] + p);
-            }
-            if (p + 1 == tile_n) atomicMax(&a.ranges[key[i]].y, g[i] + 1u);
+                    atomicMax(&a.ranges[lr].y, gbase[(rs_xf(l, a.sub) >> a.shift) & (RADIX - 1)] + p);
+            }
+            if (p + 1 == tile_n) atomicMax(&a.ranges[kr].y, g[i] + 1u);
         }
     }
     RS_STAMP(5);
@@ -680,10 +690,10 @@
     *ptr = t.hist;
     *words = t.zero_bytes / 4;
 }
-void radix_depth_zero_region(void* temp, uint64_t n, uint32_t** ptr, size_t* words) {
+void radix_depth_zero_region(void* temp, uint64_t n, uint32_t** ptr, size_t* words, bool header_only) {
     const RsTemp t = rs_carve(temp, n ? n : 1, rs_plan_for_depth(n ? n : 1), rs_scanned(n ? n : 1));
     *ptr = t.hist;
-    *words = t.zero_bytes / 4;
+    *words = header_only ? (size_t)((char*)t.status - (char*)t.hist) / 4 : t.zero_bytes / 4;
 }
 
 bool radix_wants_hist(uint64_t n) { return n > 0 && !rs_scanned(n); }
@@ -722,7 +732,7 @@
     bool aux_skip_ones;
 };
 static int rs_run(const RsPlan& pl, const RsBuffers& b, uint64_t n, void* temp, hipStream_t s, const uint32_t* n_dev,
-                  bool temp_zeroed, const uint32_t* ext_hist, bool exclusive) {
+                  bool temp_zeroed, const uint32_t* ext_hist, bool exclusive, int key_shift = 0) {
     if (n == 0) return 0;
     if (n >= (1ull << 32)) { set_error("radix sort: more than 2^32-1 pairs"); return 1; }
     const bool scanned = rs_scanned(n);
@@ -767,7 +777,8 @@
         a.vfinal = b.vfinal ? b.vfinal : vout;
         a.kfinal = b.vfinal ? b.kfinal : kout;
         a.ranges = (!pl.depth && p == pl.npasses - 1) ? b.ranges : nullptr;
-        if (a.ranges) a.kfinal = nullptr;
+        a.range_shift = key_shift;
+        if (a.ranges && key_shift == 0) a.kfinal = nullptr;
         a.aux_in = b.aux_in; a.aux_out = b.aux_out; a.aux_skip_ones = b.aux_skip_ones ? 1 : 0;
         if (scanned) {
             RsTileHistArgs h;
@@ -801,14 +812,15 @@
 
 int radix_sort_pairs(uint32_t* ka, uint32_t* va, uint32_t* kb, uint32_t* vb, uint64_t n, int bits, void* temp,
                      hipStream_t s, const uint32_t* n_dev, bool temp_zeroed, const uint2* aux_in, uint2* aux_out,
-                     const uint32_t* ext_hist, bool aux_empty_for_ones, bool exclusive, uint2* ranges) {
-    const RsPlan pl = rs_plan_plain(bits);
+                     const uint32_t* ext_hist, bool aux_empty_for_ones, bool exclusive, uint2* ranges, int key_shift) {
+    RsPlan pl = rs_plan_plain(bits);
+    for (int p = 0; p < RS_MAX_PASSES; ++p) pl.shift[p] += key_shift;
     if (pl.npasses > RS_MAX_PASSES) { set_error("radix sort: more than 32 key bits"); return 1; }
     RsBuffers b;
     b.ranges = ranges;
     b.ka = ka; b.va = va; b.va_is_index = false; b.pa = nullptr; b.kb = kb; b.vb = vb; b.pb = nullptr; b.kfinal = nullptr; b.vfinal = nullptr;
     b.aux_in = aux_in; b.aux_out = aux_out; b.aux_skip_ones = aux_empty_for_ones;
-    return rs_run(pl, b, n, temp, s, n_dev, temp_zeroed, ext_hist, exclusive);
+    return rs_run(pl, b, n, temp, s, n_dev, temp_zeroed, ext_hist, exclusive, key_shift);
 }
 
 int radix_sort_depth(uint32_t* keys, uint32_t* key_b, uint32_t* val_a, uint32_t* val_b, void* rect, bool payload,
diff --git a/monogs_amd/debug.py b/monogs_amd/debug.py
--- a/monogs_amd/debug.py
+++ b/monogs_amd/debug.py
@@ -18,6 +18,7 @@
     dev = means3D.device
     P = means3D.shape[0]
     H, W = int(rs.image_height), int(rs.image_width)
+    per_tile = lib.mgs_binning_path(P, W, H) == 1
     c = lambda t, n: None if t is None else _f32(t.detach(), n)
     means3D, opacities = c(means3D, "means3D"), c(opacities, "opacities")
     colors_precomp, shs, scales = c(colors_precomp, "colors"), c(shs, "shs"), c(scales, "scales")
@@ -69,13 +70,20 @@
     point_list = view(binning, (3 if in_b else 2) * _au(r * 4), R * 4, torch.int32)
     rec = view(geom, 0, P * 64, torch.float32).reshape(P, 16)
     o = _au(P * 64)
-    perm = view(geom, o + 4 * _au(P * 4), P * 4, torch.int32)
     o_rect = o + 6 * _au(P * 4) + _au(((P + 2047) // 2048 + 64) * 4) + _au(P * 4)
-    wh_sorted = view(geom, o_rect + _au(P * 8), P * 8, torch.int32).reshape(P, 2)[:, 1]
-    tiles_touched = torch.zeros(P, dtype=torch.int32, device=geom.device)
-    tiles_touched[perm.long()] = (wh_sorted & 0xFFFF) * ((wh_sorted >> 16) & 0xFFFF)
+    if per_tile:
+        keys = view(geom, o, P * 4, torch.int32).long() & 0xFFFFFFFF
+        perm = torch.sort(keys, stable=True).indices.to(torch.int32)
+        wh = view(geom, o_rect, P * 8, torch.int32).reshape(P, 2)[:, 1]
+        tiles_touched = (wh & 0xFFFF) * ((wh >> 16) & 0xFFFF)
+    else:
+        perm = view(geom, o + 4 * _au(P * 4), P * 4, torch.int32)
+        wh_sorted = view(geom, o_rect + _au(P * 8), P * 8, torch.int32).reshape(P, 2)[:, 1]
+        tiles_touched = torch.zeros(P, dtype=torch.int32, device=geom.device)
+        tiles_touched[perm.long()] = (wh_sorted & 0xFFFF) * ((wh_sorted >> 16) & 0xFFFF)
     depth_key = rec[:, 11].contiguous().view(torch.int32)
     return dict(color=color, depth=depth, opacity=opacity, radii=radii, n_touched=n_touched, num_rendered=R,
                 status=int(status.item()),
                 final_T=final_T, n_contrib=n_contrib, ranges=ranges, tile_sorted=tile_sorted,
-                point_list=point_list, rec=rec, tiles_touched=tiles_touched, depth_key=depth_key, perm=perm)
+                point_list=point_list, rec=rec, tiles_touched=tiles_touched, depth_key=depth_key, perm=perm,
+                depth_path="per_tile" if per_tile else "global")
```

Result: faster. 2752 Mpix/s, median of 6 (+7.0%).
